# edavalosanaya/FastPoseCNN

Hardware: AMD Instinct MI355X
Metric: img/s end-to-end 640x480 inference; hough-vote kernel HBM GB/s vs roofline (higher is better)
Workload: dtype f32

## Files before the change

fastposecnn_amd/_native.py:

```python
import ctypes
import os

import torch

_HERE = os.path.dirname(os.path.abspath(__file__))
LIB_PATH = os.path.join(_HERE, "libfpc_hip.so")

_lib = None

_vp = ctypes.c_void_p
_i = ctypes.c_int
_i64 = ctypes.c_int64
_u64 = ctypes.c_uint64
_f = ctypes.c_float
_sz = ctypes.c_size_t

_SIGNATURES = {
    "fpc_abi_version": (ctypes.c_int, []),
    "fpc_error_string": (ctypes.c_char_p, [_i]),
    "fpc_last_hip_error": (ctypes.c_char_p, []),
    "fpc_generate_hypothesis": (_i, [_vp, _vp, _vp, _vp, _i, _i, _i, _vp]),
    "fpc_voting_for_hypothesis": (_i, [_vp, _vp, _vp, _vp, _i, _i, _i, _f, _vp]),
    "fpc_ransac_workspace_bytes": (_sz, [_i, _i, _i, _i]),
    "fpc_ransac_voting_v3": (_i, [_vp, _vp, _i64, _i64, _i64, _i64, _i, _vp, _i, _i, _i, _vp, _vp, _u64, _f, _i, _i,
                                  _vp, _vp, _vp, _vp, _vp, _vp, _vp, _vp, _vp, _sz, _vp]),
    "fpc_ransac_voting_v3_bits": (_i, [_vp, _vp, _vp, _i64, _i64, _i64, _i64, _i, _vp, _i, _i, _i, _vp, _vp, _u64, _f, _i, _i, _vp, _vp, _vp, _vp, _vp, _vp, _vp, _vp, _vp, _sz, _vp]),
    "fpc_ransac_voting_v3_pose": (_i, [_vp, _vp, _vp, _i64, _i64, _i64, _i64, _i, _vp, _i, _i, _i, _vp, _vp, _u64, _f, _i, _i, _vp, _vp, _vp, _vp, _vp, _vp, _vp, _vp,
                                       _vp, _vp, _vp, _vp, _vp, _vp, _vp, _sz, _vp]),
    "fpc_vote_set_prune": (_i, [_i, _i, ctypes.POINTER(ctypes.c_int32)]),
    "fpc_vote_prune_info": (_i, [_vp, _sz, _i, _i, _i, _i, _vp, _vp]),
    "fpc_class_compress": (_i, [_vp, _vp, _vp, _vp, _vp, _vp, _i, _i, _i, _vp, _vp, _vp, _vp, _vp, _vp]),
    "fpc_class_compress_bits": (_i, [_vp, _vp, _vp, _vp, _vp, _vp, _i, _i, _i, _vp, _vp, _vp, _vp, _vp, _vp, _vp]),
    "fpc_cc_workspace_bytes": (_sz, [_i, _i, _i]),
    "fpc_cc_bits_supported": (_i, [_i, _i, _i]),
    "fpc_fg_bits": (_i, [_vp, _i, _i, _i, _vp, _vp]),
    "fpc_cc_label_bits": (_i, [_vp, _i, _i, _i, _vp, _vp, _vp, _i, _vp, _sz, _vp]),
    "fpc_cc_label": (_i, [_vp, _i, _i, _i, _vp, _vp, _vp, _i, _vp, _sz, _vp]),
    "fpc_aggregate_workspace_bytes": (_sz, [_i]),
    "fpc_aggregate": (_i, [_vp, _vp, _vp, _vp, _vp, _vp, _i, _i, _i, _i, _vp, _vp, _vp, _vp, _vp, _vp, _vp, _vp, _vp, _vp, _sz,
                           _vp]),
    "fpc_aggregate_bits": (_i, [_vp, _vp, _vp, _vp, _vp, _vp, _i, _i, _i, _i, _vp, _vp, _vp, _vp, _vp, _vp, _vp, _vp, _vp, _vp, _vp, _vp, _sz, _vp]),
    "fpc_mask_bits_words": (_sz, [_i, _i]),
    "fpc_pose_errors": (_i, [_vp, _vp, _vp, _vp, _i, _vp, _vp, _vp, _vp, _vp, _vp, _i, _vp, _vp, _vp, _vp]),
    "fpc_post_network_backward": (_i, [_vp, _vp, _i, _i, _i, _i, _vp, _vp, _f, _i, _u64, _vp, _vp, _vp, _vp, _vp, _vp]),
    "fpc_vote_refine_backward": (_i, [_vp, _vp, _i64, _i64, _i64, _i64, _i, _i, _i, _vp, _f, _i, _u64, _vp, _vp, _vp]),
    "fpc_class_compress_backward": (_i, [_vp, _vp, _vp, _vp, _vp, _vp, _vp, _i, _i, _i, _vp, _vp, _vp, _vp, _vp]),
    "fpc_mask_losses": (_i, [_vp, _vp, _i, _i, _i, _i64, _i64, _f, _f, _vp, _vp, _vp, _vp]),
    "fpc_grad_sumsq": (_i, [_vp, _sz, _vp, _vp]),
    "fpc_lookahead_radam_step": (_i, [_vp, _vp, _vp, _vp, _vp, _sz, _f, _f, _f, _f, _f, _i64, _i, _f, _vp, _vp]),
    "fpc_pose_rt": (_i, [_vp, _vp, _vp, _vp, _i, _vp, _vp, _vp, _vp]),
    "fpc_pack_pose_records": (_i, [_vp] * 9 + [_i, _i, _i, _vp, _vp]),
    "fpc_mask_iou_workspace_bytes": (_sz, [_i, _i, _i64]),
    "fpc_mask_iou": (_i, [_vp, _i, _vp, _i, _i64, _i, _vp, _vp, _vp, _vp, _sz, _vp]),
    "fpc_preprocess_workspace_bytes": (_sz, [_i]),
    "fpc_preprocess_u8": (_i, [_vp, _i, _i, _i, ctypes.POINTER(ctypes.c_double), ctypes.POINTER(ctypes.c_double), _i, _vp, _vp,
                               _sz, _vp]),
    "fpc_png_info": (_i, [_vp, _sz, ctypes.POINTER(ctypes.c_int32)]),
    "fpc_png_decode": (_i, [_vp, _sz, _vp, _sz, _i]),
    "fpc_png_decode_batch": (_i, [ctypes.POINTER(_vp), ctypes.POINTER(_sz), _i, _vp, _i, _i, _i]),
    "fpc_net_create": (_i, [ctypes.c_char_p, _i, _i, _i, _i, ctypes.POINTER(_vp)]),
    "fpc_net_create_encoder": (_i, [_i, ctypes.POINTER(_i), _i, _i, _i, _i, ctypes.POINTER(_vp)]),
    "fpc_net_destroy": (None, [_vp]),
    "fpc_net_set_graph": (_i, [_vp, _i]),
    "fpc_net_set_split_precision": (_i, [_vp, _i]),
    "fpc_net_param_count": (_i, [_vp]),
    "fpc_net_param_name": (ctypes.c_char_p, [_vp, _i]),
    "fpc_net_param_numel": (_i64, [_vp, _i]),
    "fpc_net_workspace_bytes": (_sz, [_vp]),
    "fpc_net_load_params": (_i, [_vp, _vp, _i, _vp, _sz, _vp]),
    "fpc_net_forward": (_i, [_vp, _vp, _vp, _vp, _vp, _vp, _vp, _vp, _vp, _vp, _vp, _vp, _vp]),
    "fpc_net_forward_bits": (_i, [_vp, _vp, _vp, _vp, _vp, _vp, _vp, _vp, _vp, _vp, _vp, _vp, _vp, _vp]),
    "fpc_net_autotune_next": (_i, [_vp, _i]),
    "fpc_net_conv_count": (_i, [_vp]),
    "fpc_net_conv_plan": (_i, [_vp, _i, ctypes.POINTER(_i)]),
    "fpc_net_copy_plans": (_i, [_vp, _vp]),
    "fpc_net_force_winograd": (_i, [_vp, _i]),
    "fpc_net_force_pointwise": (_i, [_vp, _i]),
    "fpc_net_force_fold": (_i, [_vp, _i]),
    "fpc_net_force_direct_h3": (_i, [_vp, _i]),
    "fpc_net_force_stem_pool": (_i, [_vp, _i]),
    "fpc_stem_pool_tasks": (_i, [_i, _i, ctypes.POINTER(_i64)]),
    "fpc_net_graph_recorded": (_i, [_vp]),
    "fpc_net_flops": (_i, [_vp, ctypes.POINTER(ctypes.c_double)]),
    "fpc_net_tensor": (_i, [_vp, ctypes.c_char_p, ctypes.POINTER(_vp), ctypes.POINTER(_i), ctypes.POINTER(_i),
                            ctypes.POINTER(_i)]),
    "fpc_conv2d_workspace_bytes": (_sz, [_i, _i, _i, _i, _i, _i, _i]),
    "fpc_conv2d_workspace_bytes_for": (_sz, [_i, _i, _i, _i, _i, _i, _i, _i, _i, _i]),
    "fpc_conv2d_plan": (_i, [_i, _i, _i, _i, _i, _i, _i, _i, _i, _i, ctypes.POINTER(_i)]),
    "fpc_conv2d": (_i, [_vp, _i64, _i64, _i64, _i64, _vp, _vp, _vp, _vp, _vp, _vp, _vp, _i, _i, _i, _i, _i, _i, _i, _i,
                        _i, _i, _i, _i, _i, _vp, _sz, _vp]),
    "fpc_conv2d_wgrad_workspace_bytes": (_sz, [_i, _i, _i, _i, _i, _i, _i]),
    "fpc_upsample_bilinear_fwd": (_i, [_vp, _i64, _i64, _i64, _i64, _vp, _i, _i, _i, _i, _i, _i, _vp]),
    "fpc_upsample_bilinear_bwd_scratch_floats": (_sz, [_i, _i, _i, _i, _i]),
    "fpc_upsample_bilinear_bwd": (_i, [_vp, _i64, _i64, _i64, _i64, _vp, _vp, _i, _i, _i, _i, _i, _i, _vp]),
    "fpc_groupnorm4_relu_scratch_floats": (_sz, [_i, _i, _i]),
    "fpc_groupnorm4_relu_fwd": (_i, [_vp, _vp, _vp, _vp, _vp, _vp, _i, _i, _i, _i, ctypes.c_float, _vp]),
    "fpc_groupnorm4_relu_bwd": (_i, [_vp, _vp, _vp, _vp, _vp, _vp, _vp, _i, _i, _i, _i, _vp]),
    "fpc_conv2d_wgrad": (_i, [_vp, _i64, _i64, _i64, _vp, _vp, _i, _i, _i, _i, _i, _i, _i, _i, _i, _vp, _sz, _vp]),
    "fpc_conv2d_wgrad_split": (_i, [_vp, _i64, _i64, _i64, _vp, _vp, _i, _i, _i, _i, _i, _i, _i, _i, _i, _vp, _sz, _vp]),
}

EXPORTED = tuple(_SIGNATURES)


def lib():
    global _lib
    if _lib is None:
        if not os.path.exists(LIB_PATH):
            raise RuntimeError(
                f"fastposecnn_amd: {LIB_PATH} is missing — build it with `python -m fastposecnn_amd.build` "
                "(hipcc --offload-arch=gfx950). There is no CPU fallback for the HIP hot path.")
        L = ctypes.CDLL(LIB_PATH)
        for name, (res, args) in _SIGNATURES.items():
            fn = getattr(L, name)
            fn.restype = res
            fn.argtypes = args
        if L.fpc_abi_version() != 11:
            raise RuntimeError("fastposecnn_amd: libfpc_hip.so ABI version mismatch")
        _lib = L
    return _lib


def check(rc, what):
    if rc != 0:
        L = lib()
        msg = L.fpc_error_string(rc).decode()
        hip = L.fpc_last_hip_error().decode() if rc == -3 else ""
        raise RuntimeError(f"fastposecnn_amd: {what} failed: {msg} (code {rc}){' — HIP: ' + hip if hip else ''}")


def ptr(t):
    return None if t is None else t.data_ptr()


_raw_stream = getattr(torch._C, "_cuda_getCurrentRawStream", None)
_cur_device = getattr(torch._C, "_cuda_getDevice", None)


def stream():
    if _raw_stream is not None and _cur_device is not None:
        return _raw_stream(_cur_device())
    return torch.cuda.current_stream().cuda_stream


def require_gpu(*tensors, what="this op"):
    for t in tensors:
        if t is not None and not t.is_cuda:
            raise RuntimeError(f"fastposecnn_amd: {what} runs only on GPU tensors (HIP kernels, no CPU fallback)")


_workspaces = {}


def workspace(tag, device, nbytes):
    key = (tag, device.index, stream())
    ws = _workspaces.get(key)
    if ws is None or ws.numel() < nbytes:
        ws = torch.empty(max(int(nbytes), 256), dtype=torch.uint8, device=device)
        assert ws.data_ptr() % 256 == 0
        _workspaces[key] = ws
    return ws
```

fastposecnn_amd/csrc/net.hip:

```cpp
#include <math.h>
#include <stdio.h>
#include <stdlib.h>
#include <string.h>

#include <initializer_list>
#include <string>
#include <utility>
#include <vector>

#include "net_kernels.hpp"

namespace fpc {

struct PackedConv {
    int Cin = 0, Cinp = 0, Cout = 0, Kh = 1, Kw = 1, stride = 1, pad = 0;
    int Kwp = 1;
    int K = 0, Kpad = 0, Npad = 0;
    int p_w = -1;
    int p_bn = -1;
    int p_bias = -1;
    size_t w_off = 0, scale_off = 0, shift_off = 0;
    size_t wino_off = 0;
    bool wino_ok = false;
    size_t h3_off = 0;
    bool h3_ok = false;
};

struct Act { size_t off = 0; int H = 0, W = 0, C = 0; };

struct ConvPlan {
    int bm = 64, bn = 64, nsplit = 1, mtiles = 1, ntiles = 1, wino = 0, bf3 = 0, fused = 0;
    int lat = 0;
    int stem = 0;
    int pw = 0;
    int fold = 0;
    int h3 = 0;
    int pool = 0;
};

static bool stem_ok(const ConvArgs& a) {
    return a.lanepx == 1 && a.generic == 0 && a.Kh == 7 && a.stride == 2 && a.pad == 3 && a.Cout == 64 && a.Kpad == 224 &&
           a.Wo % 64 == 0 && !a.p[0].res && !a.p[0].up && !a.p[0].gn_part && a.in_sc == 1 && a.in_sw == 4 &&
           a.in_sh == (long long)4 * a.Wi && a.in_sb == (long long)4 * a.Hi * a.Wi;
}

static bool lateral_ok(const ConvArgs& a, int groups) {
    if (a.Kh != 1 || a.Kw != 1 || a.stride != 1 || a.pad != 0 || a.generic != 0 || (a.Cin != 64 && a.Cin != 128) || a.Kpad != a.Cin ||
        a.Cout % 32 != 0 || a.in_sc != 1 || a.in_sw != a.Cin || a.in_sh != (long long)a.Wi * a.Cin ||
        a.in_sb != (long long)a.Hi * a.Wi * a.Cin || a.lanepx)
        return false;
    for (int g = 0; g < groups; ++g)
        if (a.p[g].in != a.p[0].in || a.p[g].scale || a.p[g].res || a.p[g].gn_part || ((a.p[g].up != nullptr) != (a.p[0].up != nullptr)))
            return false;
    return !(a.p[0].up && ((a.Ho | a.Wo) & 1));
}

static bool pw_ok(const ConvArgs& a, int groups) {
    if (a.Kh != 1 || a.Kw != 1 || a.pad != 0 || (a.stride != 1 && a.stride != 2) || a.generic != 0 || a.lanepx || a.Cin % 64 != 0 ||
        a.Kpad != a.Cin || a.Cout % 64 != 0 || a.in_sc != 1)
        return false;
    for (int g = 0; g < groups; ++g)
        if (a.p[g].in != a.p[0].in || a.p[g].gn_part || (a.p[g].scale != nullptr) != (a.p[0].scale != nullptr) ||
            (a.p[g].shift != nullptr) != (a.p[0].shift != nullptr) || (a.p[g].res != nullptr) != (a.p[0].res != nullptr) ||
            (a.p[g].up != nullptr) != (a.p[0].up != nullptr))
            return false;
    return !(a.p[0].up && ((a.Ho | a.Wo) & 1));
}

static bool can_fuse(const ConvPlan& p, int groups, int B) {
    return p.nsplit > 1 && (long long)groups * B * p.mtiles * p.ntiles <= kConvTickets;
}

static ConvPlan plan_conv(int HoWo, int B, int Cout, int ksteps, int groups, int force_bm = 0, int force_bn = 0,
                          int force_split = 0) {
    ConvPlan best;
    double best_t = 1e300;
    const int bms[2] = {64, 128}, bns[2] = {64, 128};
    for (int bi = 0; bi < 2; ++bi)
        for (int bj = 0; bj < 2; ++bj) {
            int bm = bms[bi], bn = bns[bj];
            if (force_bm && bm != force_bm) continue;
            if (force_bn && bn != force_bn) continue;
            if (!force_bn && bn == 128 && Cout <= 64) continue;
            int mt = cdiv(HoWo, bm), nt = cdiv(Cout, bn);
            for (int ns = 1; ns <= 32; ++ns) {
                if (force_split && ns != force_split) continue;
                int per = cdiv(ksteps, ns);
                if ((ns - 1) * per >= ksteps) continue;
                if (ns > 1 && (Cout % 4 != 0)) continue;
                double nblk = (double)groups * B * mt * nt * ns;
                double work = (double)(bm / 64) * (bn / 64) * per * 16.0 * 64.0 + 4000.0;
                double t = ceil(nblk / 256.0) * work + (ns > 1 ? 10000.0 + 200.0 * ns : 0.0);
                if (t < best_t) { best_t = t; best = ConvPlan{bm, bn, ns, mt, nt, 0}; }
            }
        }
    best.fused = can_fuse(best, groups, B) ? 1 : 0;
    return best;
}

static std::vector<ConvPlan> conv_candidates(int HoWo, int B, int Cout, int ksteps, int groups) {
    std::vector<ConvPlan> out;
    const int splits[] = {1, 2, 3, 4, 6, 8, 12, 16, 24};
    for (int bm = 64; bm <= 128; bm += 64)
        for (int bn = 64; bn <= 128; bn += 64) {
            if (bn == 128 && Cout <= 64) continue;
            int mt = cdiv(HoWo, bm), nt = cdiv(Cout, bn);
            long long base = (long long)groups * B * mt * nt;
            for (int ns : splits) {
                int per = cdiv(ksteps, ns);
                if (ns > 1 && (per < 2 || (ns - 1) * per >= ksteps || Cout % 4 != 0)) continue;
                if (ns > 1 && base * ns > 4096) continue;
                out.push_back(ConvPlan{bm, bn, ns, mt, nt, 0});
                if (can_fuse(out.back(), groups, B)) { ConvPlan f = out.back(); f.fused = 1; out.push_back(f); }
            }
        }
    return out;
}

static size_t splitk_floats_for(const ConvPlan& p, int groups, int B, int Npad) {
    return p.nsplit > 1 ? (size_t)groups * p.nsplit * B * p.mtiles * p.bm * Npad : 0;
}

}

using namespace fpc;

struct fpc_net {
    int layers[4];
    int classes, B, H, W;
    int expansion = 1;
    std::vector<std::string> pnames;
    std::vector<int64_t> pnumel;
    std::vector<const float*> pptr;
    std::vector<PackedConv> convs;
    size_t packed_floats = 0;
    size_t total_floats = 0;
    float* ws = nullptr;
    bool loaded = false;
    bool tuning = false;
    bool tuned = false;
    int tune_mode = 0;

    int c_stem = -1;
    struct Block { int conv1, conv2, ds, conv3 = -1; };
    std::vector<Block> blocks[4];
    struct Dec {
        int lat[4];
        int seg[7];
        int p_gn[7];
        int p_head_w, p_head_b;
        int head_ch, head_chp;
    } dec[4];

    Act a_img4, a_stem, a_pool;
    std::vector<Act> a_blk_t[4], a_blk_y[4], a_blk_d[4];
    std::vector<Act> a_blk_t2[4];
    Act a_p[4][4];
    Act a_seg[4][7];
    Act a_up[4][3];
    size_t gn_part_off[4][7], gn_aff_off[4][7];
    int gn_P[7];
    Act a_low[4];
    Act a_lsum[4];
    int merge_split = -1;
    size_t splitk_off = 0, splitk_floats = 0;
    int use_graph = 0;
    int split_precision = 0;
    hipGraphExec_t graph_exec = nullptr;
    size_t zeros_off = 0;
    size_t tickets_off = 0;

    bool h3_packed = false;
    hipStream_t load_stream = nullptr;
    size_t stem_h3_off = 0;
    bool fold_ok = false;
    size_t fold_wc_off[4] = {}, fold_img1_off[4] = {}, fold_img2_off[4] = {}, fold_tab_off[4] = {};

    std::vector<ConvPlan> cplan;
    std::vector<float> tune_score;
    std::vector<int> c_howo, c_groups;

    size_t bump = 0;
    size_t alloc(size_t n) { size_t o = bump; bump += (n + 63) / 64 * 64; return o; }
    Act alloc_act(int h, int w, int c) { Act a; a.H = h; a.W = w; a.C = c; a.off = alloc((size_t)B * h * w * c); return a; }
    int add_param(const std::string& n, int64_t numel) { pnames.push_back(n); pnumel.push_back(numel); return (int)pnames.size() - 1; }

    int add_conv(const std::string& wname, int Cin, int Cout, int k, int stride, int pad, const char* bn_prefix,
                 const char* bias_name, int Cinp = 0, int Kwp = 0) {
        PackedConv c;
        c.Cin = Cin; c.Cinp = Cinp ? Cinp : Cin; c.Cout = Cout; c.Kh = c.Kw = k; c.stride = stride; c.pad = pad;
        c.Kwp = Kwp ? Kwp : k;
        c.K = c.Cinp * k * c.Kwp; c.Kpad = cdiv(c.K, kConvBK) * kConvBK; c.Npad = cdiv(Cout, kConvNAlign) * kConvNAlign;
        c.p_w = add_param(wname, (int64_t)Cout * Cin * k * k);
        if (bn_prefix) {
            std::string p(bn_prefix);
            c.p_bn = add_param(p + ".weight", Cout);
            add_param(p + ".bias", Cout);
            add_param(p + ".running_mean", Cout);
            add_param(p + ".running_var", Cout);
        }
        if (bias_name) c.p_bias = add_param(bias_name, Cout);
        c.w_off = alloc(conv_packed_floats(c.Npad, c.Kpad));
        if (bn_prefix) { c.scale_off = alloc(Cout); c.shift_off = alloc(Cout); }
        c.wino_ok = (k == 3 && stride == 1 && pad == 1 && c.Cinp == Cin && Cin % 8 == 0 && Cout % 64 == 0);
        if (c.wino_ok) c.wino_off = alloc((size_t)(Cout % 128 == 0 ? 96 : 72) * Cout * Cin + 80);
        convs.push_back(c);
        return (int)convs.size() - 1;
    }
};

static const char* kDecNames[4] = {"mask_decoder", "rotation_decoder", "translation_decoder", "scales_decoder"};
static const char* kHeadNames[4] = {"segmentation_head", "rotation_head", "translation_head", "scales_head"};

static int conv_out(int x, int k, int s, int p) { return (x + 2 * p - k) / s + 1; }

static int net_build(fpc_net* n, int classes, int B, int H, int W, fpc_net_t** out);

extern "C" int fpc_net_create(const char* encoder, int classes, int B, int H, int W, fpc_net_t** out) {
    if (!encoder || !out || classes < 2 || classes > 8 || B < 1 || H < 32 || W < 32 || H % 32 || W % 32) return FPC_EINVAL;
    fpc_net* n = new fpc_net();
    if (!strcmp(encoder, "resnet18")) { int l[4] = {2, 2, 2, 2}; memcpy(n->layers, l, sizeof(l)); }
    else if (!strcmp(encoder, "resnet34")) { int l[4] = {3, 4, 6, 3}; memcpy(n->layers, l, sizeof(l)); }
    else { delete n; return FPC_EINVAL; }
    return net_build(n, classes, B, H, W, out);
}

extern "C" int fpc_net_create_encoder(int block, const int* layers4, int classes, int B, int H, int W, fpc_net_t** out) {
    if (!layers4 || !out || (block != 1 && block != 4) || classes < 2 || classes > 8 || B < 1 || H < 32 || W < 32 || H % 32 ||
        W % 32)
        return FPC_EINVAL;
    for (int L = 0; L < 4; ++L)
        if (layers4[L] < 1 || layers4[L] > 64) return FPC_EINVAL;
    fpc_net* n = new fpc_net();
    memcpy(n->layers, layers4, sizeof(n->layers));
    n->expansion = block;
    return net_build(n, classes, B, H, W, out);
}

static int net_build(fpc_net* n, int classes, int B, int H, int W, fpc_net_t** out) {
    n->classes = classes; n->B = B; n->H = H; n->W = W;
    {
        const char* e = getenv("FPC_MERGE_SPLIT");
        n->merge_split = e ? (atoi(e) != 0) : 1;
    }
    char buf[256];

    n->c_stem = n->add_conv("encoder.conv1.weight", 3, 64, 7, 2, 3, "encoder.bn1", nullptr, 4, 8);
    const int planes[4] = {64, 128, 256, 512};
    const int e = n->expansion;
    int inpl = 64;
    for (int L = 0; L < 4; ++L)
        for (int bi = 0; bi < n->layers[L]; ++bi) {
            int stride = (bi == 0 && L > 0) ? 2 : 1;
            fpc_net::Block blk;
            snprintf(buf, sizeof(buf), "encoder.layer%d.%d", L + 1, bi);
            std::string p(buf);
            if (e == 4) {
                const int C = 4 * planes[L];
                blk.conv1 = n->add_conv(p + ".conv1.weight", inpl, planes[L], 1, 1, 0, (p + ".bn1").c_str(), nullptr);
                blk.conv2 = n->add_conv(p + ".conv2.weight", planes[L], planes[L], 3, stride, 1, (p + ".bn2").c_str(), nullptr);
                blk.conv3 = n->add_conv(p + ".conv3.weight", planes[L], C, 1, 1, 0, (p + ".bn3").c_str(), nullptr);
                blk.ds = -1;
                if (stride != 1 || inpl != C)
                    blk.ds = n->add_conv(p + ".downsample.0.weight", inpl, C, 1, stride, 0, (p + ".downsample.1").c_str(), nullptr);
                inpl = C;
                n->blocks[L].push_back(blk);
                continue;
            }
            blk.conv1 = n->add_conv(p + ".conv1.weight", inpl, planes[L], 3, stride, 1, (p + ".bn1").c_str(), nullptr);
            blk.conv2 = n->add_conv(p + ".conv2.weight", planes[L], planes[L], 3, 1, 1, (p + ".bn2").c_str(), nullptr);
            blk.ds = -1;
            if (stride != 1 || inpl != planes[L])
                blk.ds = n->add_conv(p + ".downsample.0.weight", inpl, planes[L], 1, stride, 0, (p + ".downsample.1").c_str(), nullptr);
            inpl = planes[L];
            n->blocks[L].push_back(blk);
        }
    const int G = classes - 1;
    const int head_ch[4] = {classes, 4 * G, 3 * G, 3 * G};
    for (int d = 0; d < 4; ++d) {
        std::string D(kDecNames[d]);
        fpc_net::Dec& dc = n->dec[d];
        dc.lat[0] = n->add_conv(D + ".p5.weight", 512 * e, 256, 1, 1, 0, nullptr, (D + ".p5.bias").c_str());
        const int skipc[3] = {256 * e, 128 * e, 64 * e};
        for (int i = 0; i < 3; ++i) {
            snprintf(buf, sizeof(buf), "%s.p%d.skip_conv", kDecNames[d], 4 - i);
            std::string p(buf);
            dc.lat[1 + i] = n->add_conv(p + ".weight", skipc[i], 256, 1, 1, 0, nullptr, (p + ".bias").c_str());
        }
        const int nconv[4] = {3, 2, 1, 1};
        int si = 0;
        for (int sb = 0; sb < 4; ++sb)
            for (int j = 0; j < nconv[sb]; ++j) {
                snprintf(buf, sizeof(buf), "%s.seg_blocks.%d.block.%d.block", kDecNames[d], sb, j);
                std::string p(buf);
                dc.seg[si] = n->add_conv(p + ".0.weight", j == 0 ? 256 : 128, 128, 3, 1, 1, nullptr, nullptr);
                dc.p_gn[si] = n->add_param(p + ".1.weight", 128);
                n->add_param(p + ".1.bias", 128);
                ++si;
            }
    }
    for (int d = 0; d < 4; ++d) {
        fpc_net::Dec& dc = n->dec[d];
        dc.head_ch = head_ch[d];
        dc.head_chp = (head_ch[d] + 3) / 4 * 4;
        dc.p_head_w = n->add_param(std::string(kHeadNames[d]) + ".0.weight", (int64_t)head_ch[d] * 128);
        dc.p_head_b = n->add_param(std::string(kHeadNames[d]) + ".0.bias", head_ch[d]);
    }
    n->fold_ok = e == 1;
    if (n->fold_ok)
        for (int d = 0; d < 4; ++d) {
            n->fold_wc_off[d] = n->alloc((size_t)128 * 64 * 9);
            n->fold_img1_off[d] = n->alloc((size_t)16 * 128 * 64 + 2);
            n->fold_img2_off[d] = n->alloc((size_t)16 * 128 * 256 + 2);
            n->fold_tab_off[d] = n->alloc((size_t)16 * 128);
        }
    if (e == 1) {
        std::vector<int> sites;
        for (int L = 1; L < 4; ++L) { sites.push_back(n->blocks[L][0].conv1); if (n->blocks[L][0].ds >= 0) sites.push_back(n->blocks[L][0].ds); }
        for (int d = 0; d < 4; ++d)
            for (int i = 0; i < 3; ++i) sites.push_back(n->dec[d].lat[i]);
        for (int ci : sites) {
            PackedConv& c = n->convs[ci];
            if (c.wino_ok || c.Cin % kConvBK != 0 || c.Cinp != c.Cin || c.Kh * c.Kw > 32) continue;
            c.h3_ok = true;
            c.h3_off = n->alloc(h3_packed_floats(c.Npad, c.Kpad));
        }
    }
    n->stem_h3_off = n->alloc(h3_packed_floats(n->convs[n->c_stem].Npad, n->convs[n->c_stem].Kpad));
    n->zeros_off = n->alloc(64);
    n->tickets_off = n->alloc(kConvTickets);
    n->packed_floats = n->bump;

    int h1 = conv_out(H, 7, 2, 3), w1 = conv_out(W, 7, 2, 3);
    n->a_img4 = n->alloc_act(H, W, 4);
    n->a_stem = n->alloc_act(h1, w1, 64);
    int hp = conv_out(h1, 3, 2, 1), wp = conv_out(w1, 3, 2, 1);
    n->a_pool = n->alloc_act(hp, wp, 64);
    int fh[4], fw[4];
    {
        int h = hp, w = wp;
        for (int L = 0; L < 4; ++L) {
            const int hin = h, win = w;
            if (L > 0) { h = conv_out(h, 3, 2, 1); w = conv_out(w, 3, 2, 1); }
            fh[L] = h; fw[L] = w;
            if (e == 4) {
                const int C = 4 * planes[L];
                const Act t1 = n->alloc_act(hin, win, planes[L]), t2 = n->alloc_act(h, w, planes[L]);
                const Act y[2] = {n->alloc_act(h, w, C), n->alloc_act(h, w, C)};
                const Act dd = n->alloc_act(h, w, C);
                for (int bi = 0; bi < n->layers[L]; ++bi) {
                    Act t = t1;
                    if (bi > 0) { t.H = h; t.W = w; }
                    n->a_blk_t[L].push_back(t);
                    n->a_blk_t2[L].push_back(t2);
                    n->a_blk_y[L].push_back(y[bi & 1]);
                    n->a_blk_d[L].push_back(n->blocks[L][bi].ds >= 0 ? dd : Act());
                }
                continue;
            }
            for (int bi = 0; bi < n->layers[L]; ++bi) {
                n->a_blk_t[L].push_back(n->alloc_act(h, w, planes[L]));
                n->a_blk_y[L].push_back(n->alloc_act(h, w, planes[L]));
                n->a_blk_d[L].push_back(n->blocks[L][bi].ds >= 0 ? n->alloc_act(h, w, planes[L]) : Act());
            }
        }
    }
    for (int L = 1; L < 4; ++L)
        if (fh[L - 1] != 2 * fh[L] || fw[L - 1] != 2 * fw[L]) { delete n; return FPC_EINVAL; }
    const int seg_level[7] = {3, 2, 1, 2, 1, 1, 0};
    for (int d = 0; d < 4; ++d) {
        for (int i = 0; i < 4; ++i) n->a_p[d][i] = n->alloc_act(fh[3 - i], fw[3 - i], 256);
        for (int i = 0; i < 7; ++i) n->a_seg[d][i] = n->alloc_act(fh[seg_level[i]], fw[seg_level[i]], 128);
        n->a_up[d][0] = n->alloc_act(fh[2], fw[2], 128);
        n->a_up[d][1] = n->alloc_act(fh[1], fw[1], 128);
        n->a_up[d][2] = n->alloc_act(fh[1], fw[1], 128);
        n->a_low[d] = n->alloc_act(fh[0], fw[0], n->dec[d].head_chp);
        n->a_lsum[d] = n->alloc_act(fh[1], fw[1], n->dec[d].head_chp);
    }

    n->cplan.resize(n->convs.size());
    n->tune_score.assign(n->convs.size(), 0.f);
    n->c_howo.assign(n->convs.size(), 0);
    n->c_groups.assign(n->convs.size(), 0);
    auto plan = [&](int ci, int HoWo, int groups) {
        const PackedConv& c = n->convs[ci];
        n->c_howo[ci] = HoWo; n->c_groups[ci] = groups;
        n->cplan[ci] = plan_conv(HoWo, B, c.Cout, c.Kpad / kConvBK, groups);
        size_t need = splitk_floats_for(n->cplan[ci], groups, B, c.Npad);
        for (const ConvPlan& q : conv_candidates(HoWo, B, c.Cout, c.Kpad / kConvBK, groups)) {
            size_t f = splitk_floats_for(q, groups, B, c.Npad);
            if (f * sizeof(float) <= ((size_t)256 << 20) && f > need) need = f;
        }
        if (need > n->splitk_floats) n->splitk_floats = need;
    };
    plan(n->c_stem, h1 * w1, 1);
    for (int L = 0; L < 4; ++L)
        for (size_t bi = 0; bi < n->blocks[L].size(); ++bi) {
            const fpc_net::Block& blk = n->blocks[L][bi];
            if (e == 4) {
                plan(blk.conv1, n->a_blk_t[L][bi].H * n->a_blk_t[L][bi].W, 1);
                plan(blk.conv2, fh[L] * fw[L], 1);
                plan(blk.conv3, fh[L] * fw[L], 1);
                if (blk.ds >= 0) plan(blk.ds, fh[L] * fw[L], 1);
                continue;
            }
            plan(blk.conv1, fh[L] * fw[L], 1);
            plan(blk.conv2, fh[L] * fw[L], 1);
            if (blk.ds >= 0) plan(blk.ds, fh[L] * fw[L], 1);
        }
    for (int i = 0; i < 4; ++i) plan(n->dec[0].lat[i], fh[3 - i] * fw[3 - i], 4);
    for (int i = 0; i < 7; ++i) {
        int HoWo = fh[seg_level[i]] * fw[seg_level[i]];
        plan(n->dec[0].seg[i], HoWo, 4);
        n->gn_P[i] = cdiv(HoWo, 128) * 4;
        for (int d = 0; d < 4; ++d) {
            n->gn_part_off[d][i] = n->alloc((size_t)B * n->gn_P[i] * 128 * 2);
            n->gn_aff_off[d][i] = n->alloc((size_t)B * 128 * 2);
        }
    }
    n->splitk_off = n->alloc(n->splitk_floats);
    n->total_floats = n->bump;
    n->pptr.assign(n->pnames.size(), nullptr);
    *out = n;
    return FPC_OK;
}

extern "C" void fpc_net_destroy(fpc_net_t* n) {
    if (!n) return;
    if (n->graph_exec) (void)hipGraphExecDestroy(n->graph_exec);
    delete n;
}

static int pack_h3_images(fpc_net* n, hipStream_t s) {
    for (const PackedConv& c : n->convs)
        if (c.h3_ok) {
            int rc = launch_pack_weight_h3(n->pptr[c.p_w], n->ws + c.h3_off, c.Cout, c.Cin, c.Cinp, c.Kh, c.Kw, c.Kwp, c.Npad, c.Kpad, s);
            if (rc) return rc;
        }
    const PackedConv& st = n->convs[n->c_stem];
    int rc = launch_pack_weight_h3(n->pptr[st.p_w], n->ws + n->stem_h3_off, st.Cout, st.Cin, st.Cinp, st.Kh, st.Kw, st.Kwp, st.Npad, st.Kpad, s);
    if (rc) return rc;
    n->h3_packed = true;
    return FPC_OK;
}

extern "C" int fpc_net_set_split_precision(fpc_net_t* n, int on) {
    if (!n) return FPC_EINVAL;
    n->split_precision = on < 0 ? 0 : (on > 3 ? 3 : on);
    if (n->split_precision >= 3 && n->loaded && !n->h3_packed) return pack_h3_images(n, n->load_stream);
    return FPC_OK;
}

extern "C" int fpc_net_graph_recorded(const fpc_net_t* n) { return n && n->use_graph && n->graph_exec ? 1 : 0; }

extern "C" int fpc_net_set_graph(fpc_net_t* n, int on) {
    if (!n) return FPC_EINVAL;
    n->use_graph = on ? 1 : 0;
    if (!on && n->graph_exec) { (void)hipGraphExecDestroy(n->graph_exec); n->graph_exec = nullptr; }
    return FPC_OK;
}
extern "C" int fpc_net_param_count(const fpc_net_t* n) { return n ? (int)n->pnames.size() : 0; }
extern "C" const char* fpc_net_param_name(const fpc_net_t* n, int i) {
    return (n && i >= 0 && i < (int)n->pnames.size()) ? n->pnames[i].c_str() : nullptr;
}
extern "C" int64_t fpc_net_param_numel(const fpc_net_t* n, int i) {
    return (n && i >= 0 && i < (int)n->pnumel.size()) ? n->pnumel[i] : -1;
}
extern "C" size_t fpc_net_workspace_bytes(const fpc_net_t* n) { return n ? n->total_floats * sizeof(float) : 0; }

extern "C" int fpc_net_load_params(fpc_net_t* n, const float* const* params, int count, void* ws, size_t ws_bytes,
                                   fpc_stream_t stream) {
    if (!n || !params || count != (int)n->pnames.size() || !ws) return FPC_EINVAL;
    if (((uintptr_t)ws & 255) != 0 || ws_bytes < n->total_floats * sizeof(float)) return FPC_EWORKSPACE;
    if (n->graph_exec) { (void)hipGraphExecDestroy(n->graph_exec); n->graph_exec = nullptr; }
    for (int i = 0; i < count; ++i)
        if (!params[i] || ((uintptr_t)params[i] & 15)) return FPC_EINVAL;
    hipStream_t s = (hipStream_t)stream;
    n->ws = (float*)ws;
    n->pptr.assign(params, params + count);
    n->load_stream = s;
    n->h3_packed = false;
    if (n->split_precision >= 3) { int rc = pack_h3_images(n, s); if (rc) return rc; }
    if (hipMemsetAsync(n->ws + n->zeros_off, 0, 64 * sizeof(float), s) != hipSuccess) return FPC_ELAUNCH;
    if (hipMemsetAsync(n->ws + n->tickets_off, 0, kConvTickets * sizeof(int), s) != hipSuccess) return FPC_ELAUNCH;
    for (const PackedConv& c : n->convs) {
        int rc = launch_pack_weight(n->pptr[c.p_w], n->ws + c.w_off, c.Cout, c.Cin, c.Cinp, c.Kh, c.Kw, c.Kwp, c.Npad, c.Kpad, s);
        if (rc) return rc;
        rc = launch_pack_weight_bf3(n->pptr[c.p_w], n->ws + c.w_off, c.Cout, c.Cin, c.Cinp, c.Kh, c.Kw, c.Kwp, c.Npad, c.Kpad, s);
        if (rc) return rc;
        if (c.wino_ok) {
            rc = launch_wino_pack(n->pptr[c.p_w], n->ws + c.wino_off, c.Cout, c.Cin, s);
            if (rc) return rc;
            rc = launch_wino_pack_bf3(n->pptr[c.p_w], n->ws + c.wino_off + (size_t)16 * c.Cout * c.Cin, c.Cout, c.Cin, s);
            if (rc) return rc;
            if (c.Cout % 128 == 0) {
                rc = launch_wino_pack_c128(n->pptr[c.p_w], n->ws + c.wino_off + (size_t)40 * c.Cout * c.Cin, c.Cout, c.Cin, s);
                if (rc) return rc;
            }
            rc = launch_wino_pack_h2(n->pptr[c.p_w], n->ws + c.wino_off + (size_t)(c.Cout % 128 == 0 ? 64 : 40) * c.Cout * c.Cin, c.Cout, c.Cin, s);
            if (rc) return rc;
            if (c.Cin % 16 == 0) {
                rc = launch_wino_pack_h3(n->pptr[c.p_w], n->ws + c.wino_off + (size_t)(c.Cout % 128 == 0 ? 80 : 56) * c.Cout * c.Cin + 8, c.Cout, c.Cin, s);
                if (rc) return rc;
            }
        }
        if (c.p_bn >= 0) {
            rc = launch_fold_bn(n->pptr[c.p_bn], n->pptr[c.p_bn + 1], n->pptr[c.p_bn + 2], n->pptr[c.p_bn + 3], 1e-5f,
                                c.Cout, n->ws + c.scale_off, n->ws + c.shift_off, s);
            if (rc) return rc;
        }
    }
    if (n->fold_ok)
        for (int d = 0; d < 4; ++d) {
            const PackedConv &sc = n->convs[n->dec[d].seg[6]], &lc = n->convs[n->dec[d].lat[3]];
            int rc = launch_fold_compose(n->pptr[sc.p_w], n->pptr[lc.p_w], n->pptr[lc.p_bias], n->ws + n->fold_wc_off[d],
                                         n->ws + n->fold_tab_off[d], sc.Cout, sc.Cin, lc.Cin, s);
            if (!rc) rc = launch_wino_pack_h3_pair(n->ws + n->fold_wc_off[d], n->ws + n->fold_img1_off[d], lc.Cin, n->pptr[sc.p_w],
                                                   n->ws + n->fold_img2_off[d], sc.Cin, sc.Cout, s);
            if (rc) return rc;
        }
    n->loaded = true;
    return FPC_OK;
}

namespace {

struct ConvIO {
    const float* in; long long sb, sh, sw, sc; int Hi, Wi;
    float* out; int Ho, Wo;
    const float* res; const float* up; float* gn_part;
};

void fill_conv_args(const fpc_net* n, ConvArgs& a, const PackedConv& c, const ConvPlan& p, int Hi, int Wi, int Ho,
                    int Wo, long long sb, long long sh, long long sw, long long sc, bool relu, int mode) {
    memset(&a, 0, sizeof(a));
    a.B = n->B; a.Hi = Hi; a.Wi = Wi; a.Cin = c.Cin; a.Ho = Ho; a.Wo = Wo; a.Cout = c.Cout; a.Npad = c.Npad;
    a.Kh = c.Kh; a.Kw = c.Kw; a.stride = c.stride; a.pad = c.pad; a.K = c.K; a.Kpad = c.Kpad;
    a.in_sb = sb; a.in_sh = sh; a.in_sw = sw; a.in_sc = sc;
    a.relu = relu ? 1 : 0; a.nsplit = p.nsplit; a.mtiles = p.mtiles; a.ntiles = p.ntiles; a.ksteps = c.Kpad / kConvBK;
    a.bm = p.bm; a.bn = p.bn; a.generic = mode;
    a.splitk_ws = n->ws + n->splitk_off;
    a.zeros = n->ws + n->zeros_off;
    a.tickets = (int*)(n->ws + n->tickets_off);
    a.fused = p.fused;
}

int launch_conv_plan(ConvArgs& a, const ConvPlan& p, int groups, hipStream_t s) {
    if (p.stem) {
        if (groups != 1 || !stem_ok(a)) return FPC_EINVAL;
        StemArgs t;
        memset(&t, 0, sizeof(t));
        t.in = a.p[0].in;
        t.wpl = reinterpret_cast<const unsigned short*>(a.p[0].w + (size_t)a.Npad * a.Kpad);
        t.out = a.p[0].out; t.scale = a.p[0].scale; t.shift = a.p[0].shift;
        t.B = a.B; t.Hi = a.Hi; t.Wi = a.Wi; t.Ho = a.Ho; t.Wo = a.Wo; t.Cout = a.Cout; t.Npad = a.Npad; t.Kpad = a.Kpad; t.relu = a.relu;
        t.grid = p.stem;
        return launch_stem7x7(t, s);
    }
    if (p.pw) {
        if (!pw_ok(a, groups)) return FPC_EINVAL;
        PwArgs w;
        memset(&w, 0, sizeof(w));
        w.in = a.p[0].in;
        for (int g = 0; g < groups; ++g) {
            w.wpl[g] = reinterpret_cast<const unsigned short*>(a.p[g].w + (size_t)a.Npad * a.Kpad);
            w.out[g] = a.p[g].out; w.scale[g] = a.p[g].scale; w.shift[g] = a.p[g].shift; w.res[g] = a.p[g].res; w.up[g] = a.p[g].up;
        }
        w.in_sb = a.in_sb; w.in_sh = a.in_sh; w.in_sw = a.in_sw;
        w.B = a.B; w.Ho = a.Ho; w.Wo = a.Wo; w.Cin = a.Cin; w.Cout = a.Cout; w.Npad = a.Npad; w.Kpad = a.Kpad; w.stride = a.stride;
        w.groups = groups; w.relu = a.relu;
        w.has_scale = a.p[0].scale != nullptr; w.has_shift = a.p[0].shift != nullptr;
        w.has_res = a.p[0].res != nullptr; w.has_up = a.p[0].up != nullptr;
        w.variant = p.pw - 1;
        return launch_conv1x1(w, s);
    }
    if (p.lat) {
        if (!lateral_ok(a, groups)) return FPC_EINVAL;
        LatArgs l;
        memset(&l, 0, sizeof(l));
        l.in = a.p[0].in;
        for (int g = 0; g < groups; ++g) {
            if (p.h3 && !a.h3_w[g]) return FPC_EINVAL;
            l.wpl[g] = reinterpret_cast<const unsigned short*>(p.h3 ? a.h3_w[g] : a.p[g].w + (size_t)a.Npad * a.Kpad);
            l.out[g] = a.p[g].out; l.shift[g] = a.p[g].shift; l.up[g] = a.p[g].up;
        }
        l.B = a.B; l.Ho = a.Ho; l.Wo = a.Wo; l.Cout = a.Cout; l.Npad = a.Npad; l.Kpad = a.Kpad; l.groups = groups; l.relu = a.relu;
        l.parts = p.lat;
        l.h3 = p.h3;
        return launch_lateral1x1(l, s);
    }
    if (p.wino) {
        WinoArgs w;
        memset(&w, 0, sizeof(w));
        for (int g = 0; g < groups; ++g) {
            if (!a.wino_w[g] || a.p[g].up) return FPC_EINVAL;
            w.p[g] = a.p[g];
            w.p[g].w = a.wino_w[g] + ((p.wino == 5 || p.wino == 7) ? (size_t)16 * a.Cout * a.Cin : p.wino == 6 ? (size_t)40 * a.Cout * a.Cin
                                      : p.wino == 8 ? (size_t)(a.Cout % 128 == 0 ? 64 : 40) * a.Cout * a.Cin
                                      : p.wino == 9 ? (size_t)(a.Cout % 128 == 0 ? 80 : 56) * a.Cout * a.Cin + 8 : 0);
        }
        w.variant = p.wino == 3 ? 1 : (p.wino == 4 ? 2 : (p.wino == 5 ? 3 : 0));
        w.zeros = a.zeros;
        w.dbg = (long long*)a.dbg;
        w.groups = groups;
        w.B = a.B; w.H = a.Ho; w.W = a.Wo; w.Cin = a.Cin; w.Cout = a.Cout; w.relu = a.relu;
        w.waves = (p.wino == 2 || p.wino == 4 || p.wino == 5 || p.wino == 7 || p.wino == 8 || p.wino == 9) ? 8 : 4;
        w.tbx = cdiv(cdiv(a.Wo, 2), 8); w.tby = cdiv(cdiv(a.Ho, 2), w.waves);
        if (p.fold) {
            if (p.wino != 9 || !a.fold_in) return FPC_EINVAL;
            for (int g = 0; g < groups; ++g) {
                w.in2[g] = a.fold_up[g]; w.w2[g] = a.fold_w2[g];
                w.btab[g] = a.fold_tab[g];
                w.p[g].in = a.fold_in; w.p[g].w = a.fold_w[g];
            }
            w.fold = 1; w.Cin2 = a.Cin; w.Cin = a.fold_cin;
        }
        if (p.wino == 6) return a.Cout % 128 == 0 ? launch_conv_wino_c128(w, groups, s) : FPC_EINVAL;
        if (p.wino == 7) return launch_conv_wino_w4(w, groups, s);
        if (p.wino == 9) return launch_conv_wino_h3(w, groups, s);
        if (p.wino == 8) return launch_conv_wino_h2(w, groups, s);
        return launch_conv_wino(w, groups, s);
    }
    a.bm = p.bm; a.bn = p.bn; a.nsplit = p.nsplit; a.mtiles = p.mtiles; a.ntiles = p.ntiles; a.groups = groups;
    a.bf3 = (p.bf3 && a.generic == 0) ? 1 : 0;
    a.fused = (p.fused && p.nsplit > 1) ? 1 : 0;
    a.h3 = 0;
    if (p.h3) {
        if (a.generic != 0) return FPC_EINVAL;
        ConvArgs h = a;
        h.bf3 = 0; h.h3 = 1;
        for (int g = 0; g < groups; ++g) {
            if (!a.h3_w[g]) return FPC_EINVAL;
            h.p[g].w = a.h3_w[g];
        }
        int rc = launch_conv(h, groups, s);
        if (!rc && h.nsplit > 1 && !h.fused) rc = launch_conv_splitk_epilogue(h, groups, s);
        return rc;
    }
    int rc = launch_conv(a, groups, s);
    if (rc) return rc;
    if (a.nsplit > 1 && !a.fused) rc = launch_conv_splitk_epilogue(a, groups, s);
    return rc;
}

int plan_gn_rows(const ConvPlan& p, int Ho, int Wo) {
    return p.wino ? cdiv(cdiv(Wo, 2), 8) * cdiv(cdiv(Ho, 2), (p.wino == 2 || p.wino == 4 || p.wino == 5 || p.wino == 7 || p.wino == 8 || p.wino == 9) ? 8 : 4) : p.mtiles * p.bm / 32;
}

int run_conv(fpc_net* n, ConvArgs& a, int groups, int ci, hipStream_t s) {
    if (n && n->tuning) {
        hipEvent_t e0, e1;
        if (hipEventCreate(&e0) != hipSuccess || hipEventCreate(&e1) != hipSuccess) return FPC_ELAUNCH;
        float best_ms = 1e30f;
        ConvPlan best = n->cplan[ci];
        size_t cap = n->splitk_floats;
        std::vector<ConvPlan> cands = conv_candidates(a.Ho * a.Wo, a.B, a.Cout, a.ksteps, groups);
        const size_t nf = cands.size();
        if (n->split_precision && a.generic == 0) {
            for (size_t i = 0; i < nf; ++i) { ConvPlan q = cands[i]; q.bf3 = 1; cands.push_back(q); }
        }
        if (n->split_precision >= 3 && a.generic == 0 && a.h3_w[0]) {
            for (size_t i = 0; i < nf; ++i) { ConvPlan q = cands[i]; q.h3 = 1; cands.push_back(q); }
        }
        if (n->split_precision && groups == 1 && stem_ok(a)) {
            ConvPlan sq; sq.stem = 256; cands.push_back(sq);
        }
        if (n->split_precision && lateral_ok(a, groups)) {
            const int tiles = groups * (a.Cout / 32);
            for (int parts = 1; parts <= tiles; parts *= 2)
                if (tiles % parts == 0) {
                    ConvPlan lq; lq.lat = parts; cands.push_back(lq);
                    if (n->split_precision >= 3 && a.h3_w[0]) { lq.h3 = 1; cands.push_back(lq); }
                }
        }
        if (n->split_precision && n->expansion == 4 && pw_ok(a, groups)) {
            ConvPlan pq;
            pq.pw = 1; cands.push_back(pq);
            pq.pw = 2; cands.push_back(pq);
        }
        if (a.wino_w[0] && !a.p[0].up) {
            ConvPlan wq;
            wq.wino = 1; cands.push_back(wq);
            wq.wino = 2; cands.push_back(wq);
            wq.wino = 3; cands.push_back(wq);
            if (a.zeros) { wq.wino = 4; cands.push_back(wq); }
            if (n->split_precision && a.zeros) { wq.wino = 5; cands.push_back(wq); }
            if (n->split_precision && a.Cout % 128 == 0) { wq.wino = 6; cands.push_back(wq); }
            if (n->split_precision) { wq.wino = 7; cands.push_back(wq); }
            if (n->split_precision >= 3 && a.Cin % 16 == 0) { wq.wino = 9; cands.push_back(wq); }
            else if (n->split_precision >= 2) { wq.wino = 8; cands.push_back(wq); }
        }
        for (const ConvPlan& q : cands) {
            if (splitk_floats_for(q, groups, a.B, a.Npad) > cap) continue;
            int rc = launch_conv_plan(a, q, groups, s);
            if (rc == FPC_EINVAL) continue;
            if (rc) { (void)hipEventDestroy(e0); (void)hipEventDestroy(e1); return rc; }
            float ms = 1e30f;
            for (int rep = 0; rep < 3; ++rep) {
                float t = 0.f;
                bool timed = hipEventRecord(e0, s) == hipSuccess && launch_conv_plan(a, q, groups, s) == FPC_OK &&
                             hipEventRecord(e1, s) == hipSuccess && hipEventSynchronize(e1) == hipSuccess &&
                             hipEventElapsedTime(&t, e0, e1) == hipSuccess;
                if (timed && t < ms) ms = t;
            }
            float score = ms;
            if (n->tune_mode >= 1) {
                double nblk = q.stem ? 512.0
                              : q.lat ? (double)cdiv(a.Ho * a.Wo, 128) * a.B * q.lat
                              : q.pw ? (double)cdiv(a.B * a.Ho * a.Wo, pw_tile_pixels(q.pw - 1)) * (a.Cout / 64) * groups * q.pw
                              : q.wino ? (double)cdiv(cdiv(a.Wo, 2), 8) * cdiv(cdiv(a.Ho, 2), (q.wino == 2 || q.wino == 4 || q.wino == 5 || q.wino == 7 || q.wino == 8 || q.wino == 9) ? 8 : 4) * a.B * (a.Cout / (q.wino == 6 ? 128 : 64)) * groups
                                     : (double)q.mtiles * q.ntiles * q.nsplit * a.B * groups;
                double slots = 256.0 * ((q.wino == 2 || q.wino == 4 || q.wino == 5 || q.wino == 6 || q.wino == 7 || q.wino == 8 || q.wino == 9) ? 1.0 : 2.0);
                double share = nblk / slots;
                if (share > 1.0) share = 1.0;
                if (share < 0.125) share = 0.125;
                score = ms * (float)(n->tune_mode == 2 ? share : sqrt(share));
            }
            if (score < best_ms) { best_ms = score; best = q; }
        }
        n->tune_score[ci] = best_ms;
        if (n->split_precision >= 3 && a.fold_in && a.fold_lat_ms > 0.f) {
            ConvPlan fq;
            fq.wino = 9; fq.fold = 1;
            int rc = launch_conv_plan(a, fq, groups, s);
            if (rc && rc != FPC_EINVAL) { (void)hipEventDestroy(e0); (void)hipEventDestroy(e1); return rc; }
            float ms = 1e30f;
            for (int rep = 0; rep < 3 && !rc; ++rep) {
                float t = 0.f;
                bool timed = hipEventRecord(e0, s) == hipSuccess && launch_conv_plan(a, fq, groups, s) == FPC_OK &&
                             hipEventRecord(e1, s) == hipSuccess && hipEventSynchronize(e1) == hipSuccess &&
                             hipEventElapsedTime(&t, e0, e1) == hipSuccess;
                if (timed && t < ms) ms = t;
            }
            if (ms < best_ms + a.fold_lat_ms) best = fq;
        }
        (void)hipEventDestroy(e0);
        (void)hipEventDestroy(e1);
        n->cplan[ci] = best;
    }
    ConvPlan p = n ? n->cplan[ci] : ConvPlan{a.bm, a.bn, a.nsplit, a.mtiles, a.ntiles, 0, a.bf3, a.fused};
    return launch_conv_plan(a, p, groups, s);
}

}

#define FPC_TRY(x) do { int rc__ = (x); if (rc__) return rc__; } while (0)

static int launch_stem_pool(const ConvArgs& a, const float* h3_image, float* pool, int Hp, int Wp, hipStream_t s) {
    if (!h3_image || !stem_ok(a)) return FPC_EINVAL;
    StemPoolArgs t;
    memset(&t, 0, sizeof(t));
    t.in = a.p[0].in; t.wpl = reinterpret_cast<const unsigned short*>(h3_image); t.out = pool;
    t.scale = a.p[0].scale; t.shift = a.p[0].shift;
    t.B = a.B; t.Hi = a.Hi; t.Wi = a.Wi; t.Ho = a.Ho; t.Wo = a.Wo; t.Hp = Hp; t.Wp = Wp; t.Npad = a.Npad; t.Kpad = a.Kpad; t.relu = a.relu;
    t.band = kStemPoolBand; t.grid = 256;
    return launch_stem_pool_h3(t, s);
}

static int forward_middle(fpc_net* n, hipStream_t s) {
    float* ws = n->ws;
    const int B = n->B, H = n->H, W = n->W;
    ConvArgs a;
    auto nhwc = [&](const Act& t, long long& sb, long long& sh, long long& sw, long long& sc) {
        sc = 1; sw = t.C; sh = (long long)t.W * t.C; sb = (long long)t.H * sh;
    };
    {
        const PackedConv& c = n->convs[n->c_stem];
        fill_conv_args(n, a, c, n->cplan[n->c_stem], H, W, n->a_stem.H, n->a_stem.W, (long long)4 * H * W, (long long)4 * W, 4,
                       1, true, 0);
        a.Cin = 8 * c.Cinp; a.Kw = 1; a.K = c.K; a.lanepx = 1;
        a.p[0] = ConvPtrs{ws + n->a_img4.off, ws + c.w_off, ws + n->a_stem.off, ws + c.scale_off, ws + c.shift_off, nullptr, nullptr, nullptr};
        const float* h3img = n->h3_packed ? ws + n->stem_h3_off : nullptr;
        auto pool_launch = [&]() {
            return launch_maxpool3x3s2(ws + n->a_stem.off, ws + n->a_pool.off, B, n->a_stem.H, n->a_stem.W, 64, n->a_pool.H, n->a_pool.W, s);
        };
        if (n->cplan[n->c_stem].pool && !n->tuning) {
            FPC_TRY(launch_stem_pool(a, h3img, ws + n->a_pool.off, n->a_pool.H, n->a_pool.W, s));
        } else {
            n->cplan[n->c_stem].pool = 0;
            FPC_TRY(run_conv(n, a, 1, n->c_stem, s));
            FPC_TRY(pool_launch());
            if (n->tuning && n->split_precision >= 3 && launch_stem_pool(a, h3img, ws + n->a_pool.off, n->a_pool.H, n->a_pool.W, s) == FPC_OK) {
                hipEvent_t e0, e1;
                if (hipEventCreate(&e0) != hipSuccess || hipEventCreate(&e1) != hipSuccess) return FPC_ELAUNCH;
                const ConvPlan cur = n->cplan[n->c_stem];
                float ms_pair = 1e30f, ms_fused = 1e30f;
                for (int rep = 0; rep < 6; ++rep) {
                    const bool fused = rep & 1;
                    float t = 0.f;
                    bool timed = hipEventRecord(e0, s) == hipSuccess &&
                                 (fused ? launch_stem_pool(a, h3img, ws + n->a_pool.off, n->a_pool.H, n->a_pool.W, s) == FPC_OK
                                        : (launch_conv_plan(a, cur, 1, s) == FPC_OK && pool_launch() == FPC_OK)) &&
                                 hipEventRecord(e1, s) == hipSuccess && hipEventSynchronize(e1) == hipSuccess &&
                                 hipEventElapsedTime(&t, e0, e1) == hipSuccess;
                    if (timed && fused && t < ms_fused) ms_fused = t;
                    if (timed && !fused && t < ms_pair) ms_pair = t;
                }
                (void)hipEventDestroy(e0);
                (void)hipEventDestroy(e1);
                if (ms_fused < ms_pair) { ConvPlan q; q.stem = 256; q.pool = 1; n->cplan[n->c_stem] = q; }
            }
        }
    }
    Act cur = n->a_pool;
    Act feat[4];
    for (int L = 0; L < 4; ++L) {
        for (size_t bi = 0; bi < n->blocks[L].size(); ++bi) {
            const fpc_net::Block& blk = n->blocks[L][bi];
            const Act& T = n->a_blk_t[L][bi];
            const Act& Y = n->a_blk_y[L][bi];
            long long sb, sh, sw, sc;
            if (n->expansion == 4) {
                const Act& T2 = n->a_blk_t2[L][bi];
                nhwc(cur, sb, sh, sw, sc);
                const PackedConv& c1 = n->convs[blk.conv1];
                fill_conv_args(n, a, c1, n->cplan[blk.conv1], cur.H, cur.W, T.H, T.W, sb, sh, sw, sc, true, 0);
                a.p[0] = ConvPtrs{ws + cur.off, ws + c1.w_off, ws + T.off, ws + c1.scale_off, ws + c1.shift_off, nullptr, nullptr, nullptr};
                FPC_TRY(run_conv(n, a, 1, blk.conv1, s));
                long long tb, th, tw, tc;
                nhwc(T, tb, th, tw, tc);
                const PackedConv& c2 = n->convs[blk.conv2];
                fill_conv_args(n, a, c2, n->cplan[blk.conv2], T.H, T.W, T2.H, T2.W, tb, th, tw, tc, true, 0);
                a.p[0] = ConvPtrs{ws + T.off, ws + c2.w_off, ws + T2.off, ws + c2.scale_off, ws + c2.shift_off, nullptr, nullptr, nullptr};
                if (c2.wino_ok) a.wino_w[0] = ws + c2.wino_off;
                FPC_TRY(run_conv(n, a, 1, blk.conv2, s));
                const float* res = ws + cur.off;
                if (blk.ds >= 0) {
                    const PackedConv& cd = n->convs[blk.ds];
                    const Act& D = n->a_blk_d[L][bi];
                    fill_conv_args(n, a, cd, n->cplan[blk.ds], cur.H, cur.W, D.H, D.W, sb, sh, sw, sc, false, 0);
                    a.p[0] = ConvPtrs{ws + cur.off, ws + cd.w_off, ws + D.off, ws + cd.scale_off, ws + cd.shift_off, nullptr, nullptr, nullptr};
                    FPC_TRY(run_conv(n, a, 1, blk.ds, s));
                    res = ws + D.off;
                }
                nhwc(T2, tb, th, tw, tc);
                const PackedConv& c3 = n->convs[blk.conv3];
                fill_conv_args(n, a, c3, n->cplan[blk.conv3], T2.H, T2.W, Y.H, Y.W, tb, th, tw, tc, true, 0);
                a.p[0] = ConvPtrs{ws + T2.off, ws + c3.w_off, ws + Y.off, ws + c3.scale_off, ws + c3.shift_off, res, nullptr, nullptr};
                FPC_TRY(run_conv(n, a, 1, blk.conv3, s));
                cur = Y;
                continue;
            }
            nhwc(cur, sb, sh, sw, sc);
            const PackedConv& c1 = n->convs[blk.conv1];
            fill_conv_args(n, a, c1, n->cplan[blk.conv1], cur.H, cur.W, T.H, T.W, sb, sh, sw, sc, true, 0);
            a.p[0] = ConvPtrs{ws + cur.off, ws + c1.w_off, ws + T.off, ws + c1.scale_off, ws + c1.shift_off, nullptr, nullptr, nullptr};
            if (c1.wino_ok) a.wino_w[0] = ws + c1.wino_off;
            if (c1.h3_ok && n->h3_packed) a.h3_w[0] = ws + c1.h3_off;
            FPC_TRY(run_conv(n, a, 1, blk.conv1, s));
            const float* res = ws + cur.off;
            if (blk.ds >= 0) {
                const PackedConv& cd = n->convs[blk.ds];
                const Act& D = n->a_blk_d[L][bi];
                fill_conv_args(n, a, cd, n->cplan[blk.ds], cur.H, cur.W, D.H, D.W, sb, sh, sw, sc, false, 0);
                a.p[0] = ConvPtrs{ws + cur.off, ws + cd.w_off, ws + D.off, ws + cd.scale_off, ws + cd.shift_off, nullptr, nullptr, nullptr};
                if (cd.h3_ok && n->h3_packed) a.h3_w[0] = ws + cd.h3_off;
                FPC_TRY(run_conv(n, a, 1, blk.ds, s));
                res = ws + D.off;
            }
            nhwc(T, sb, sh, sw, sc);
            const PackedConv& c2 = n->convs[blk.conv2];
            fill_conv_args(n, a, c2, n->cplan[blk.conv2], T.H, T.W, Y.H, Y.W, sb, sh, sw, sc, true, 0);
            a.p[0] = ConvPtrs{ws + T.off, ws + c2.w_off, ws + Y.off, ws + c2.scale_off, ws + c2.shift_off, res, nullptr, nullptr};
            if (c2.wino_ok) a.wino_w[0] = ws + c2.wino_off;
            FPC_TRY(run_conv(n, a, 1, blk.conv2, s));
            cur = Y;
        }
        feat[L] = cur;
    }

    const bool fold = n->cplan[n->dec[0].seg[6]].fold && !n->tuning;
    for (int i = 0; i < 4; ++i) {
        if (i == 3 && fold) continue;
        const Act& src = feat[3 - i];
        long long sb, sh, sw, sc;
        nhwc(src, sb, sh, sw, sc);
        int ci0 = n->dec[0].lat[i];
        fill_conv_args(n, a, n->convs[ci0], n->cplan[ci0], src.H, src.W, src.H, src.W, sb, sh, sw, sc, false, 0);
        for (int d = 0; d < 4; ++d) {
            const PackedConv& c = n->convs[n->dec[d].lat[i]];
            a.p[d] = ConvPtrs{ws + src.off, ws + c.w_off, ws + n->a_p[d][i].off, nullptr, n->pptr[c.p_bias], nullptr,
                              i > 0 ? ws + n->a_p[d][i - 1].off : nullptr, nullptr};
            if (c.h3_ok && n->h3_packed) a.h3_w[d] = ws + c.h3_off;
        }
        FPC_TRY(run_conv(n, a, 4, ci0, s));
    }
    auto seg_conv = [&](int si, int which) -> int {
        int ci0 = n->dec[0].seg[si];
        const Act& in0 = which < 0 ? n->a_p[0][-which - 1] : n->a_up[0][which];
        long long sb, sh, sw, sc;
        nhwc(in0, sb, sh, sw, sc);
        const Act& o0 = n->a_seg[0][si];
        fill_conv_args(n, a, n->convs[ci0], n->cplan[ci0], in0.H, in0.W, o0.H, o0.W, sb, sh, sw, sc, false, 0);
        for (int d = 0; d < 4; ++d) {
            const PackedConv& c = n->convs[n->dec[d].seg[si]];
            const Act& in = which < 0 ? n->a_p[d][-which - 1] : n->a_up[d][which];
            a.p[d] = ConvPtrs{ws + in.off, ws + c.w_off, ws + n->a_seg[d][si].off, nullptr, nullptr, nullptr, nullptr,
                              ws + n->gn_part_off[d][si]};
            if (c.wino_ok) a.wino_w[d] = ws + c.wino_off;
        }
        if (si == 6 && n->fold_ok) {
            a.fold_in = ws + feat[0].off;
            a.fold_cin = feat[0].C;
            for (int d = 0; d < 4; ++d) {
                a.fold_w[d] = ws + n->fold_img1_off[d];
                a.fold_w2[d] = ws + n->fold_img2_off[d];
                a.fold_up[d] = ws + n->a_p[d][2].off;
                a.fold_tab[d] = ws + n->fold_tab_off[d];
            }
            a.fold_lat_ms = n->tune_score[n->dec[0].lat[3]];
        }
        return run_conv(n, a, 4, ci0, s);
    };
    auto gn_finish = [&](std::initializer_list<int> sites) -> int {
        GnFinArgs g;
        memset(&g, 0, sizeof(g));
        int k = 0;
        for (int si : sites) {
            const Act& o0 = n->a_seg[0][si];
            for (int d = 0; d < 4; ++d) {
                g.gn_part[k * kMaxGroup + d] = ws + n->gn_part_off[d][si];
                g.gamma[k * kMaxGroup + d] = n->pptr[n->dec[d].p_gn[si]];
                g.beta[k * kMaxGroup + d] = n->pptr[n->dec[d].p_gn[si] + 1];
                g.affine[k * kMaxGroup + d] = ws + n->gn_aff_off[d][si];
            }
            g.P[k] = plan_gn_rows(n->cplan[n->dec[0].seg[si]], o0.H, o0.W);
            g.count[k] = (long long)o0.H * o0.W * 4;
            ++k;
        }
        g.B = B; g.C = 128; g.groups = 32; g.sites = k; g.eps = 1e-5f;
        return launch_gn_finalize(g, 4, s);
    };
    auto gn_up = [&](std::initializer_list<std::pair<int, int>> jobs) -> int {
        GnUpArgs u;
        memset(&u, 0, sizeof(u));
        int k = 0;
        for (const auto& job : jobs) {
            const int si = job.first, ui = job.second;
            for (int d = 0; d < 4; ++d) {
                u.in[k * kMaxGroup + d] = ws + n->a_seg[d][si].off;
                u.affine[k * kMaxGroup + d] = ws + n->gn_aff_off[d][si];
                u.out[k * kMaxGroup + d] = ws + n->a_up[d][ui].off;
            }
            u.h[k] = n->a_seg[0][si].H; u.w[k] = n->a_seg[0][si].W;
            ++k;
        }
        u.B = B; u.C = 128; u.jobs = k;
        return launch_gn_relu_up2(u, 4, s);
    };
    FPC_TRY(seg_conv(0, -1));
    FPC_TRY(seg_conv(3, -2));
    FPC_TRY(seg_conv(5, -3));
    FPC_TRY(seg_conv(6, -4));
    FPC_TRY(gn_finish({0, 3, 5, 6}));
    FPC_TRY(gn_up({{0, 0}, {3, 2}}));
    FPC_TRY(seg_conv(1, 0));
    FPC_TRY(seg_conv(4, 2));
    FPC_TRY(gn_finish({1, 4}));
    FPC_TRY(gn_up({{1, 1}}));
    FPC_TRY(seg_conv(2, 1));
    FPC_TRY(gn_finish({2}));

    const int lo[3] = {2, 4, 5};
    const int split = n->merge_split;
    if (split) {
        HeadPartArgs hl, hh;
        memset(&hl, 0, sizeof(hl));
        memset(&hh, 0, sizeof(hh));
        for (int d = 0; d < 4; ++d) {
            for (int k = 0; k < 3; ++k) {
                hl.t[d][k] = ws + n->a_seg[d][lo[k]].off;
                hl.aff[d][k] = ws + n->gn_aff_off[d][lo[k]];
            }
            hh.t[d][0] = ws + n->a_seg[d][6].off;
            hh.aff[d][0] = ws + n->gn_aff_off[d][6];
            hl.hw[d] = hh.hw[d] = n->pptr[n->dec[d].p_head_w];
            hl.hb[d] = hh.hb[d] = n->pptr[n->dec[d].p_head_b];
            hl.out[d] = ws + n->a_lsum[d].off;
            hh.lsum[d] = ws + n->a_lsum[d].off;
            hh.out[d] = ws + n->a_low[d].off;
            hl.ch[d] = hh.ch[d] = n->dec[d].head_ch;
            hl.chp[d] = hh.chp[d] = n->dec[d].head_chp;
        }
        hl.B = hh.B = B; hl.C = hh.C = 128;
        hl.H = n->a_seg[0][2].H; hl.W = n->a_seg[0][2].W; hl.hl = hl.H; hl.wl = hl.W;
        hh.H = n->a_seg[0][6].H; hh.W = n->a_seg[0][6].W; hh.hl = hl.H; hh.wl = hl.W;
        FPC_TRY(launch_head_part(hl, false, 4, s));
        FPC_TRY(launch_head_part(hh, true, 4, s));
    } else {
        MergeHeadArgs m;
        memset(&m, 0, sizeof(m));
        for (int d = 0; d < 4; ++d) {
            for (int k = 0; k < 3; ++k) {
                m.t_lo[d][k] = ws + n->a_seg[d][lo[k]].off;
                m.a_lo[d][k] = ws + n->gn_aff_off[d][lo[k]];
            }
            m.t_hi[d] = ws + n->a_seg[d][6].off;
            m.a_hi[d] = ws + n->gn_aff_off[d][6];
            m.hw[d] = n->pptr[n->dec[d].p_head_w];
            m.hb[d] = n->pptr[n->dec[d].p_head_b];
            m.out[d] = ws + n->a_low[d].off;
            m.ch[d] = n->dec[d].head_ch;
            m.chp[d] = n->dec[d].head_chp;
        }
        m.B = B; m.h = n->a_seg[0][2].H; m.w = n->a_seg[0][2].W; m.C = 128;
        FPC_TRY(launch_merge_head(m, 4, s));
    }
    return FPC_OK;
}

extern "C" int fpc_net_forward(fpc_net_t* n, const float* x, float* logits_mask, float* logits_quat,
                               float* logits_scales, float* logits_xy, float* logits_z, int64_t* cat_mask, float* cq,
                               float* cs, float* cxy, float* cz, fpc_stream_t stream) {
    return fpc_net_forward_bits(n, x, logits_mask, logits_quat, logits_scales, logits_xy, logits_z, cat_mask, cq, cs, cxy, cz, nullptr, stream);
}

extern "C" int fpc_net_forward_bits(fpc_net_t* n, const float* x, float* logits_mask, float* logits_quat,
                                    float* logits_scales, float* logits_xy, float* logits_z, int64_t* cat_mask, float* cq,
                                    float* cs, float* cxy, float* cz, uint64_t* fg_bits, fpc_stream_t stream) {
    if (!n || !n->loaded || !x || !cat_mask || !cq || !cs || !cxy || !cz) return FPC_EINVAL;
    if (fg_bits && (n->W % 64 != 0 || ((uintptr_t)fg_bits & 7))) return FPC_EINVAL;
    bool any = logits_mask || logits_quat || logits_scales || logits_xy || logits_z;
    bool all = logits_mask && logits_quat && logits_scales && logits_xy && logits_z;
    if (any && !all) return FPC_EINVAL;
    hipStream_t s = (hipStream_t)stream;
    float* ws = n->ws;
    const int B = n->B, H = n->H, W = n->W;

    FPC_TRY(launch_nchw3_to_nhwc4(x, ws + n->a_img4.off, B, H * W, s));
    if (n->use_graph && !n->tuning && s != nullptr && !n->graph_exec) {
        hipGraph_t g = nullptr;
        if (hipStreamBeginCapture(s, hipStreamCaptureModeThreadLocal) == hipSuccess) {
            int rc = forward_middle(n, s);
            hipError_t e = hipStreamEndCapture(s, &g);
            if (rc) { if (g) (void)hipGraphDestroy(g); return rc; }
            if (e == hipSuccess && g) e = hipGraphInstantiate(&n->graph_exec, g, nullptr, nullptr, 0);
            if (g) (void)hipGraphDestroy(g);
            if (e != hipSuccess) n->graph_exec = nullptr;
        }
        if (!n->graph_exec) { (void)hipGetLastError(); n->use_graph = 0; }
    }
    if (n->use_graph && !n->tuning && s != nullptr && n->graph_exec) {
        if (hipGraphLaunch(n->graph_exec, s) != hipSuccess) return FPC_ELAUNCH;
    } else {
        FPC_TRY(forward_middle(n, s));
    }
    {
        Up4Args u;
        memset(&u, 0, sizeof(u));
        u.lm = ws + n->a_low[0].off; u.lq = ws + n->a_low[1].off; u.lt = ws + n->a_low[2].off; u.ls = ws + n->a_low[3].off;
        u.pm = n->dec[0].head_chp; u.pq = n->dec[1].head_chp; u.pt = n->dec[2].head_chp; u.ps = n->dec[3].head_chp;
        u.o_mask = logits_mask; u.o_quat = logits_quat; u.o_scales = logits_scales; u.o_xy = logits_xy; u.o_z = logits_z;
        u.cat_mask = (long long*)cat_mask; u.cq = cq; u.cs = cs; u.cxy = cxy; u.cz = cz;
        u.B = B; u.hl = n->a_low[0].H; u.wl = n->a_low[0].W; u.H = H; u.W = W; u.C = n->classes;
        u.fg_bits = reinterpret_cast<unsigned long long*>(fg_bits); u.fg_stride = (size_t)((H * W + 4095) / 4096) * 64;
        if (u.hl * 4 != H || u.wl * 4 != W) return FPC_EINVAL;
        FPC_TRY(launch_up4_compress(u, s));
    }
    if (n->tuning) { n->tuning = false; n->tuned = true; }
    return FPC_OK;
}

extern "C" int fpc_net_autotune_next(fpc_net_t* n, int mode) {
    if (!n || !n->loaded || mode < 0 || mode > 2) return FPC_EINVAL;
    n->tuning = true;
    n->tune_mode = mode;
    if (n->graph_exec) { (void)hipGraphExecDestroy(n->graph_exec); n->graph_exec = nullptr; }
    return FPC_OK;
}

extern "C" int fpc_net_conv_count(const fpc_net_t* n) { return n ? (int)n->convs.size() : 0; }
extern "C" int fpc_net_conv_plan(const fpc_net_t* n, int i, int* out5) {
    if (!n || !out5 || i < 0 || i >= (int)n->convs.size()) return FPC_EINVAL;
    out5[0] = n->cplan[i].bm; out5[1] = n->cplan[i].bn; out5[2] = n->cplan[i].wino ? -n->cplan[i].wino : n->cplan[i].nsplit;
    if (n->cplan[i].lat) { out5[0] = 128; out5[1] = 32; out5[2] = 2000 + n->cplan[i].lat; }
    if (n->cplan[i].stem) { out5[0] = 64; out5[1] = 64; out5[2] = n->cplan[i].pool ? 3100 : 3000; }
    if (n->cplan[i].pw) { out5[0] = pw_tile_pixels(n->cplan[i].pw - 1); out5[1] = 64; out5[2] = 4000 + n->cplan[i].pw - 1; }
    if (n->cplan[i].h3) out5[2] = n->cplan[i].lat ? 7000 + n->cplan[i].lat : 6000 + n->cplan[i].nsplit;
    if (n->fold_ok && i == n->dec[0].lat[3] && n->cplan[n->dec[0].seg[6]].fold) out5[2] = 5000;
    out5[3] = n->convs[i].Cout; out5[4] = n->convs[i].K;
    return FPC_OK;
}

extern "C" int fpc_net_force_winograd(fpc_net_t* n, int form) {
    if (!n || form < 1 || form > 9) return FPC_EINVAL;
    int changed = 0;
    for (size_t i = 0; i < n->convs.size(); ++i) {
        const PackedConv& c = n->convs[i];
        if (!c.wino_ok || !n->c_groups[i] || (form == 6 && c.Cout % 128 != 0) || (form == 9 && c.Cin % 16 != 0)) continue;
        ConvPlan q = n->cplan[i];
        q.wino = form; q.lat = 0; q.stem = 0;
        if (form != 9) q.fold = 0;
        n->cplan[i] = q;
        ++changed;
    }
    if (n->graph_exec) { (void)hipGraphExecDestroy(n->graph_exec); n->graph_exec = nullptr; }
    return changed;
}

extern "C" int fpc_net_force_fold(fpc_net_t* n, int on) {
    if (!n || on < 0 || on > 1 || (on && !n->fold_ok)) return FPC_EINVAL;
    ConvPlan& p = n->cplan[n->dec[0].seg[6]];
    if (p.fold == on) return 0;
    ConvPlan q;
    q.wino = 9; q.fold = on;
    p = q;
    if (n->graph_exec) { (void)hipGraphExecDestroy(n->graph_exec); n->graph_exec = nullptr; }
    return 1;
}

extern "C" int fpc_net_force_pointwise(fpc_net_t* n, int on) {
    if (!n || on < 0 || on > 1) return FPC_EINVAL;
    int changed = 0;
    for (size_t i = 0; i < n->convs.size(); ++i) {
        const PackedConv& c = n->convs[i];
        if (!n->c_groups[i] || c.Kh != 1 || c.pad != 0 || c.Cinp != c.Cin || c.Cin % 64 || c.Kpad != c.Cin || c.Cout % 64) continue;
        if (on) {
            if (n->cplan[i].pw) continue;
            ConvPlan q;
            q.pw = 1;
            n->cplan[i] = q;
        } else {
            if (!n->cplan[i].pw) continue;
            n->cplan[i] = plan_conv(n->c_howo[i], n->B, c.Cout, c.Kpad / kConvBK, n->c_groups[i]);
        }
        ++changed;
    }
    if (n->graph_exec) { (void)hipGraphExecDestroy(n->graph_exec); n->graph_exec = nullptr; }
    return changed;
}

extern "C" int fpc_net_force_direct_h3(fpc_net_t* n, int on) {
    if (!n || on < 0 || on > 1 || (on && !n->h3_packed)) return FPC_EINVAL;
    int changed = 0;
    for (size_t i = 0; i < n->convs.size(); ++i) {
        const PackedConv& c = n->convs[i];
        if (!c.h3_ok || !n->c_groups[i] || on == n->cplan[i].h3) continue;
        const ConvPlan& p = n->cplan[i];
        ConvPlan q = plan_conv(n->c_howo[i], n->B, c.Cout, c.Kpad / kConvBK, n->c_groups[i]);
        if (on && !p.wino && !p.stem && !p.pw) q = p;
        q.bf3 = 0;
        q.h3 = on;
        n->cplan[i] = q;
        ++changed;
    }
    if (n->graph_exec) { (void)hipGraphExecDestroy(n->graph_exec); n->graph_exec = nullptr; }
    return changed;
}

extern "C" int fpc_net_force_stem_pool(fpc_net_t* n, int on) {
    if (!n || on < 0 || on > 1 || (on && !n->h3_packed)) return FPC_EINVAL;
    if (on && ((n->a_stem.H & 1) || (n->a_stem.W & 63) || (long long)n->H * n->W * 16 >= (1LL << 31))) return FPC_EINVAL;
    ConvPlan& p = n->cplan[n->c_stem];
    if (p.pool == on) return 0;
    ConvPlan q;
    q.stem = 256; q.pool = on;
    p = q;
    if (n->graph_exec) { (void)hipGraphExecDestroy(n->graph_exec); n->graph_exec = nullptr; }
    return 1;
}

extern "C" int fpc_net_copy_plans(fpc_net_t* dst, const fpc_net_t* src) {
    if (!dst || !src || dst->convs.size() != src->convs.size() || dst->H != src->H || dst->W != src->W) return FPC_EINVAL;
    for (size_t i = 0; i < dst->convs.size(); ++i) {
        const PackedConv &a = dst->convs[i], &b = src->convs[i];
        if (a.Cin != b.Cin || a.Cout != b.Cout || a.Kh != b.Kh || a.Kw != b.Kw || a.stride != b.stride || a.Npad != b.Npad ||
            a.Kpad != b.Kpad || dst->c_groups[i] != src->c_groups[i])
            return FPC_EINVAL;
    }
    for (size_t i = 0; i < dst->convs.size(); ++i) {
        const ConvPlan& q = src->cplan[i];
        if (splitk_floats_for(q, dst->c_groups[i] ? dst->c_groups[i] : 1, dst->B, dst->convs[i].Npad) > dst->splitk_floats) continue;
        if (q.nsplit > 1 && q.fused && !can_fuse(q, dst->c_groups[i] ? dst->c_groups[i] : 1, dst->B)) continue;
        if ((q.h3 || q.pool) && !dst->h3_packed) continue;
        dst->cplan[i] = q;
    }
    dst->tuned = true;
    if (dst->graph_exec) { (void)hipGraphExecDestroy(dst->graph_exec); dst->graph_exec = nullptr; }
    return FPC_OK;
}

extern "C" int fpc_net_flops(const fpc_net_t* n, double* out3) {
    if (!n || !out3) return FPC_EINVAL;
    double direct = 0.0, executed = 0.0, wino = 0.0;
    for (size_t i = 0; i < n->convs.size(); ++i) {
        if (!n->c_groups[i]) continue;
        const PackedConv& c = n->convs[i];
        const double f = 2.0 * n->B * (double)n->c_howo[i] * c.Cout * c.Cin * c.Kh * c.Kw * n->c_groups[i];
        direct += f;
        if (n->cplan[i].wino) { executed += f / 2.25; wino += f; } else executed += f;
    }
    for (int d = 0; d < 4; ++d)
        direct += 2.0 * n->B * (double)n->a_low[d].H * n->a_low[d].W * 128.0 * n->dec[d].head_ch,
        executed += 2.0 * n->B * (double)n->a_low[d].H * n->a_low[d].W * 128.0 * n->dec[d].head_ch;
    out3[0] = direct; out3[1] = executed; out3[2] = direct > 0.0 ? wino / direct : 0.0;
    return FPC_OK;
}

extern "C" int fpc_net_tensor(const fpc_net_t* n, const char* name, const float** ptr, int* H, int* W, int* C) {
    if (!n || !n->ws || !name || !ptr || !H || !W || !C) return FPC_EINVAL;
    Act t;
    bool ok = false;
    if (!strcmp(name, "stem")) {
        if (n->cplan[n->c_stem].pool) return FPC_EINVAL;
        t = n->a_stem; ok = true;
    }
    else if (!strcmp(name, "pool")) { t = n->a_pool; ok = true; }
    else if (name[0] == 'c' && name[1] >= '2' && name[1] <= '5' && !name[2]) { t = n->a_blk_y[name[1] - '2'].back(); ok = true; }
    else if (name[0] == 'd' && name[1] >= '0' && name[1] <= '3' && name[2] == '.') {
        int d = name[1] - '0';
        const char* r = name + 3;
        if (r[0] == 'p' && r[1] >= '2' && r[1] <= '5' && !r[2]) {
            if (r[1] == '2' && n->cplan[n->dec[0].seg[6]].fold) return FPC_EINVAL;
            t = n->a_p[d]['5' - r[1]]; ok = true;
        }
        else if (!strncmp(r, "seg", 3) && r[3] >= '0' && r[3] <= '6' && !r[4]) { t = n->a_seg[d][r[3] - '0']; ok = true; }
        else if (!strcmp(r, "low")) { t = n->a_low[d]; ok = true; }
    }
    if (!ok) return FPC_EINVAL;
    *ptr = n->ws + t.off; *H = t.H; *W = t.W; *C = t.C;
    return FPC_OK;
}

extern "C" int fpc_stem_pool_tasks(int Ho, int Wo, int64_t* out4) {
    if (!out4 || Ho < 2 || (Ho & 1) || Wo < 64 || (Wo & 63)) return FPC_EINVAL;
    long long o[4];
    stem_pool_tasks(Ho, Wo, kStemPoolBand, o);
    for (int i = 0; i < 4; ++i) out4[i] = o[i];
    return FPC_OK;
}

extern "C" size_t fpc_conv2d_workspace_bytes(int B, int Ho, int Wo, int Cin, int Cout, int Kh, int Kw) {
    int K = Cin * Kh * Kw, Kpad = cdiv(K, kConvBK) * kConvBK, Npad = cdiv(Cout, kConvNAlign) * kConvNAlign;
    size_t packed = conv_packed_floats(Npad, Kpad);
    size_t splitk = (size_t)32 * B * (cdiv(Ho * Wo, 128) * 128) * Npad;
    size_t wino = (size_t)96 * Cout * Cin + 128;
    return (packed + splitk + wino + kConvTickets) * sizeof(float);
}

extern "C" int fpc_conv2d_plan(int B, int Ho, int Wo, int Cin, int Cout, int Kh, int Kw, int bm, int bn, int nsplit,
                               int* out4) {
    if (!out4) return FPC_EINVAL;
    int Kpad = cdiv(Cin * Kh * Kw, kConvBK) * kConvBK;
    if (nsplit >= 6000 && nsplit < 6200) nsplit -= 6000;
    if (nsplit >= 2000) nsplit = 1;
    if (nsplit >= 1000) nsplit -= 1000;
    if (nsplit >= 100) nsplit -= 100;
    ConvPlan p = plan_conv(Ho * Wo, B, Cout, Kpad / kConvBK, 1, bm, bn, nsplit);
    if (nsplit <= -1 && nsplit >= -9) { p.wino = -nsplit; p.nsplit = nsplit; }
    out4[0] = p.bm; out4[1] = p.bn; out4[2] = p.nsplit; out4[3] = plan_gn_rows(p, Ho, Wo);
    return FPC_OK;
}

namespace {
struct Conv2dRequest { int nsplit; bool bf3, two_launch, wino; int lat; bool stem; int pw; bool h3; bool pool; };
Conv2dRequest conv2d_request(int nsplit) {
    Conv2dRequest r{nsplit, false, false, false, 0, false, 0, false, false};
    if (r.nsplit >= 7000 && r.nsplit < 8000) { r.lat = r.nsplit - 7000; r.h3 = true; r.nsplit = 1; return r; }
    if (r.nsplit >= 6000 && r.nsplit < 6200) {
        r.h3 = true; r.nsplit -= 6000;
        if (r.nsplit >= 100) { r.two_launch = true; r.nsplit -= 100; }
        return r;
    }
    if (r.nsplit >= 4000) { r.pw = r.nsplit - 4000 + 1; r.bf3 = true; r.nsplit = 1; return r; }
    if (r.nsplit == 3100) { r.stem = true; r.pool = true; r.h3 = true; r.nsplit = 1; return r; }
    if (r.nsplit == 3000) { r.stem = true; r.bf3 = true; r.nsplit = 1; return r; }
    if (r.nsplit >= 2000) { r.lat = r.nsplit - 2000; r.bf3 = true; r.nsplit = 1; return r; }
    if (r.nsplit >= 1000) { r.bf3 = true; r.nsplit -= 1000; }
    if (r.nsplit >= 100) { r.two_launch = true; r.nsplit -= 100; }
    r.wino = r.nsplit <= -1 && r.nsplit >= -9;
    return r;
}
struct Conv2dLayout { size_t packed, splitk, wino, tickets, total; };
Conv2dLayout conv2d_layout(int B, int Cin, int Cout, int Kh, int Kw, const ConvPlan& p, const Conv2dRequest& r) {
    const int K = Cin * Kh * Kw, Kpad = cdiv(K, kConvBK) * kConvBK, Npad = cdiv(Cout, kConvNAlign) * kConvNAlign;
    Conv2dLayout L;
    L.packed = r.wino ? 0 : conv_packed_floats(Npad, Kpad);
    L.splitk = r.wino ? 0 : (splitk_floats_for(p, 1, B, Npad) + 63) / 64 * 64;
    L.wino = r.wino ? (size_t)(r.nsplit == -9 ? (Cout % 128 == 0 ? 96 : 72) : r.nsplit == -8 ? (Cout % 128 == 0 ? 80 : 56) : r.nsplit == -6 ? 64 : (r.nsplit == -5 || r.nsplit == -7) ? 40 : 16) * Cout * Cin + 128 : 0;
    L.tickets = (!r.wino && p.fused && p.nsplit > 1) ? kConvTickets : 0;
    L.total = L.packed + L.splitk + L.wino + L.tickets;
    return L;
}
ConvPlan conv2d_plan_for(int B, int Ho, int Wo, int Cin, int Cout, int Kh, int Kw, int bm, int bn, const Conv2dRequest& r) {
    const int Kpad = cdiv(Cin * Kh * Kw, kConvBK) * kConvBK;
    ConvPlan p = plan_conv(Ho * Wo, B, Cout, Kpad / kConvBK, 1, r.wino ? 0 : bm, bn, r.wino ? 1 : r.nsplit);
    p.bf3 = r.bf3 ? 1 : 0;
    p.h3 = r.h3 ? 1 : 0;
    if (r.two_launch) p.fused = 0;
    p.lat = r.lat;
    p.stem = r.stem ? 256 : 0;
    p.pool = r.pool ? 1 : 0;
    p.pw = r.pw;
    return p;
}
}

extern "C" size_t fpc_conv2d_workspace_bytes_for(int B, int Ho, int Wo, int Cin, int Cout, int Kh, int Kw, int bm, int bn,
                                                 int nsplit) {
    if (B < 1 || Ho < 1 || Wo < 1 || Cin < 1 || Cout < 1 || Kh < 1 || Kw < 1) return 0;
    const Conv2dRequest r = conv2d_request(nsplit);
    const ConvPlan p = conv2d_plan_for(B, Ho, Wo, Cin, Cout, Kh, Kw, bm, bn, r);
    return std::max<size_t>(conv2d_layout(B, Cin, Cout, Kh, Kw, p, r).total * sizeof(float), 256);
}

extern "C" int fpc_conv2d(const float* in, int64_t sb, int64_t sh, int64_t sw, int64_t sc, const float* w_oihw,
                          const float* scale, const float* shift, const float* res, const float* up, float* out,
                          float* gn_part, int B, int Hi, int Wi, int Cin, int Cout, int Kh, int Kw, int stride, int pad,
                          int relu, int bm, int bn, int nsplit, void* ws, size_t ws_bytes, fpc_stream_t stream) {
    if (!in || !w_oihw || !out || !ws || B < 1 || Kh != Kw) return FPC_EINVAL;
    int Ho = conv_out(Hi, Kh, stride, pad), Wo = conv_out(Wi, Kw, stride, pad);
    if (Ho < 1 || Wo < 1) return FPC_EINVAL;
    const Conv2dRequest rq = conv2d_request(nsplit);
    nsplit = rq.nsplit;
    const bool wino = rq.wino;
    ConvPlan p = conv2d_plan_for(B, Ho, Wo, Cin, Cout, Kh, Kw, bm, bn, rq);
    const Conv2dLayout lay = conv2d_layout(B, Cin, Cout, Kh, Kw, p, rq);
    if (ws_bytes < lay.total * sizeof(float) || ((uintptr_t)ws & 255)) return FPC_EWORKSPACE;
    PackedConv c;
    c.Cin = c.Cinp = Cin; c.Cout = Cout; c.Kh = Kh; c.Kw = Kw; c.stride = stride; c.pad = pad;
    c.K = Cin * Kh * Kw; c.Kpad = cdiv(c.K, kConvBK) * kConvBK; c.Npad = cdiv(Cout, kConvNAlign) * kConvNAlign;
    hipStream_t s = (hipStream_t)stream;
    float* packed = (float*)ws;
    if (rq.stem) {
        if (Cin != 4 || Kh != 7 || stride != 2 || pad != 3 || Cout != 64 || sc != 1 || sw != 4 || sh != (int64_t)4 * Wi ||
            sb != (int64_t)4 * Hi * Wi || res || up || gn_part)
            return FPC_EINVAL;
        c.Kwp = 8; c.K = 4 * 7 * 8; c.Kpad = 224;
        if (rq.pool) {
            FPC_TRY(launch_pack_weight_h3(w_oihw, packed, Cout, Cin, Cin, Kh, Kw, c.Kwp, c.Npad, c.Kpad, s));
            fpc_net tmp1;
            tmp1.B = B; tmp1.ws = packed; tmp1.splitk_off = lay.packed;
            ConvArgs a1;
            fill_conv_args(&tmp1, a1, c, p, Hi, Wi, Ho, Wo, sb, sh, sw, sc, relu != 0, 0);
            a1.Cin = 8 * c.Cinp; a1.Kw = 1; a1.K = c.K; a1.lanepx = 1;
            a1.p[0] = ConvPtrs{in, packed, out, scale, shift, nullptr, nullptr, nullptr};
            return launch_stem_pool(a1, packed, out, Ho / 2, Wo / 2, s);
        }
        FPC_TRY(launch_pack_weight_bf3(w_oihw, packed, Cout, Cin, Cin, Kh, Kw, c.Kwp, c.Npad, c.Kpad, s));
        fpc_net tmp0;
        tmp0.B = B; tmp0.ws = packed; tmp0.splitk_off = lay.packed;
        ConvArgs a0;
        fill_conv_args(&tmp0, a0, c, p, Hi, Wi, Ho, Wo, sb, sh, sw, sc, relu != 0, 0);
        a0.Cin = 8 * c.Cinp; a0.Kw = 1; a0.K = c.K; a0.lanepx = 1;
        a0.p[0] = ConvPtrs{in, packed, out, scale, shift, nullptr, nullptr, nullptr};
        return launch_conv_plan(a0, p, 1, s);
    }
    static_assert(FPC_IGEMM_DMA_B, "the split-precision direct form stages its B rows from the bf16 planes by LDS-DMA; a build that loads "
                                   "them from the f32 image must pack that image here as well");
    if (!wino && !p.bf3 && !p.h3) FPC_TRY(launch_pack_weight(w_oihw, packed, Cout, Cin, Cin, Kh, Kw, Kw, c.Npad, c.Kpad, s));
    if (!wino && p.bf3) FPC_TRY(launch_pack_weight_bf3(w_oihw, packed, Cout, Cin, Cin, Kh, Kw, Kw, c.Npad, c.Kpad, s));
    if (!wino && p.h3) FPC_TRY(launch_pack_weight_h3(w_oihw, packed, Cout, Cin, Cin, Kh, Kw, Kw, c.Npad, c.Kpad, s));
    int mode = (sc == 1 && Cin % kConvBK == 0 && Kh * Kw <= 32 && ((int64_t)Hi + 2 * pad) * sh * 4 < ((int64_t)1 << 31)) ? 0
               : (sc == 1 && Cin % 4 == 0 && sw % 4 == 0 && sh % 4 == 0 && sb % 4 == 0 && ((uintptr_t)in & 15) == 0) ? 2 : 1;
    fpc_net tmp;
    tmp.B = B;
    tmp.ws = packed;
    tmp.splitk_off = lay.packed;
    ConvArgs a;
    fill_conv_args(&tmp, a, c, p, Hi, Wi, Ho, Wo, sb, sh, sw, sc, relu != 0, mode);
    a.p[0] = ConvPtrs{in, packed, out, scale, shift, res, up, gn_part};
    a.zeros = nullptr;
    a.tickets = nullptr;
    if (lay.tickets) {
        float* tk = packed + lay.packed + lay.splitk + lay.wino;
        a.tickets = (int*)tk;
        if (hipMemsetAsync(tk, 0, kConvTickets * sizeof(int), s) != hipSuccess) return FPC_ELAUNCH;
    }
    if (wino && relu == 77) { a.dbg = gn_part; a.p[0].gn_part = nullptr; a.relu = 0; }
#ifdef FPC_STAMP_IGEMM
    if (!wino && relu == 77) { a.dbg = gn_part; a.p[0].gn_part = nullptr; a.relu = 0; }
#endif
    if (wino) {
        if (Kh != 3 || stride != 1 || pad != 1 || Cin % 8 || Cout % 64 || sc != 1 || up || sw != Cin ||
            sh != (int64_t)Wi * Cin || sb != (int64_t)Hi * Wi * Cin)
            return FPC_EINVAL;
        float* wp = packed + lay.packed + lay.splitk;
        if (nsplit == -6 && Cout % 128) return FPC_EINVAL;
        if (nsplit > -5) FPC_TRY(launch_wino_pack(w_oihw, wp, Cout, Cin, s));
        if (nsplit == -5 || nsplit == -7) FPC_TRY(launch_wino_pack_bf3(w_oihw, wp + (size_t)16 * Cout * Cin, Cout, Cin, s));
        if (nsplit == -6) FPC_TRY(launch_wino_pack_c128(w_oihw, wp + (size_t)40 * Cout * Cin, Cout, Cin, s));
        if (nsplit == -9) FPC_TRY(launch_wino_pack_h3(w_oihw, wp + (size_t)(Cout % 128 == 0 ? 80 : 56) * Cout * Cin + 8, Cout, Cin, s));
        if (nsplit == -8) FPC_TRY(launch_wino_pack_h2(w_oihw, wp + (size_t)(Cout % 128 == 0 ? 64 : 40) * Cout * Cin, Cout, Cin, s));
        a.wino_w[0] = wp;
        a.zeros = zero_page();
        if (!a.zeros) {
            float* zp = wp + lay.wino - 64;
            if (hipMemsetAsync(zp, 0, 64 * sizeof(float), s) != hipSuccess) return FPC_ELAUNCH;
            a.zeros = zp;
        }
        p.wino = -nsplit;
        return launch_conv_plan(a, p, 1, s);
    }
    if (p.h3) {
        if (mode != 0) return FPC_EINVAL;
        a.h3_w[0] = packed;
        return launch_conv_plan(a, p, 1, s);
    }
    a.bf3 = (p.bf3 && mode == 0) ? 1 : 0;
    if (p.bf3 && mode != 0) return FPC_EINVAL;
    if (p.lat || p.pw) return launch_conv_plan(a, p, 1, s);
    return run_conv(nullptr, a, 1, 0, s);
}
```

fastposecnn_amd/csrc/net_kernels.hpp:

```cpp
#pragma once
#include "common.hpp"

namespace fpc {

#ifndef FPC_IGEMM_DMA_B
#define FPC_IGEMM_DMA_B 1
#endif

constexpr int kMaxGroup = 4;
constexpr int kConvBK = 32;
constexpr int kConvNAlign = 128;
constexpr int kConvTickets = 16384;

struct ConvPtrs {
    const float* in;
    const float* w;
    float* out;
    const float* scale;
    const float* shift;
    const float* res;
    const float* up;
    float* gn_part;
};

struct ConvArgs {
    ConvPtrs p[kMaxGroup];
    float* splitk_ws;
    int* tickets;
    int fused;
    int B, Hi, Wi, Cin, Ho, Wo, Cout, Npad, Kh, Kw, stride, pad, K, Kpad;
    long long in_sb, in_sh, in_sw, in_sc;
    int relu, nsplit, mtiles, ntiles, ksteps, bm, bn, generic, groups;
    int bf3;
    int h3;
    int lanepx;
    const float* wino_w[kMaxGroup];
    const float* h3_w[kMaxGroup];
    const float* zeros;
    const float* fold_in;
    const float* fold_w[kMaxGroup];
    const float* fold_w2[kMaxGroup];
    const float* fold_up[kMaxGroup];
    const float* fold_tab[kMaxGroup];
    int fold_cin;
    float fold_lat_ms;
    void* dbg;
};

struct LatArgs {
    const float* in;
    const unsigned short* wpl[kMaxGroup];
    float* out[kMaxGroup];
    const float* shift[kMaxGroup];
    const float* up[kMaxGroup];
    int B, Ho, Wo, Cout, Npad, Kpad, groups, relu;
    unsigned bias_mask;
    int parts;
    int h3;
};
int launch_lateral1x1(const LatArgs& a, hipStream_t s);

struct PwArgs {
    const float* in;
    const unsigned short* wpl[kMaxGroup];
    float* out[kMaxGroup];
    const float* scale[kMaxGroup];
    const float* shift[kMaxGroup];
    const float* res[kMaxGroup];
    const float* up[kMaxGroup];
    long long in_sb, in_sh, in_sw;
    int B, Ho, Wo, Cin, Cout, Npad, Kpad, stride, groups, relu;
    int has_scale, has_shift, has_res, has_up;
    int variant;
};
int launch_conv1x1(const PwArgs& a, hipStream_t s);
inline int pw_tile_pixels(int variant) { return variant == 0 ? 64 : 128; }

struct StemArgs {
    const float* in;
    const unsigned short* wpl;
    float* out;
    const float* scale;
    const float* shift;
    int B, Hi, Wi, Ho, Wo, Cout, Npad, Kpad, relu;
    int grid;
};
int launch_stem7x7(const StemArgs& a, hipStream_t s);

struct StemPoolArgs {
    const float* in;
    const unsigned short* wpl;
    float* out;
    const float* scale;
    const float* shift;
    int B, Hi, Wi, Ho, Wo, Hp, Wp, Npad, Kpad, relu;
    int band;
    int grid;
};
constexpr int kStemPoolBand = 10;
int launch_stem_pool_h3(const StemPoolArgs& a, hipStream_t s);
void stem_pool_tasks(int Ho, int Wo, int band, long long out4[4]);

constexpr int kMaxGnSites = 4;
struct GnFinArgs {
    const float* gn_part[kMaxGnSites * kMaxGroup];
    const float* gamma[kMaxGnSites * kMaxGroup];
    const float* beta[kMaxGnSites * kMaxGroup];
    float* affine[kMaxGnSites * kMaxGroup];
    int P[kMaxGnSites];
    long long count[kMaxGnSites];
    int B, C, groups, sites;
    float eps;
};

constexpr int kMaxUpJobs = 2;
struct GnUpArgs {
    const float* in[kMaxUpJobs * kMaxGroup];
    const float* affine[kMaxUpJobs * kMaxGroup];
    float* out[kMaxUpJobs * kMaxGroup];
    int h[kMaxUpJobs], w[kMaxUpJobs];
    int B, C, jobs;
};

struct MergeHeadArgs {
    const float* t_lo[kMaxGroup][3];
    const float* a_lo[kMaxGroup][3];
    const float* t_hi[kMaxGroup];
    const float* a_hi[kMaxGroup];
    const float* hw[kMaxGroup];
    const float* hb[kMaxGroup];
    float* out[kMaxGroup];
    int ch[kMaxGroup];
    int chp[kMaxGroup];
    int B, h, w, C;
};

struct HeadPartArgs {
    const float* t[kMaxGroup][3];
    const float* aff[kMaxGroup][3];
    const float* hw[kMaxGroup];
    const float* hb[kMaxGroup];
    const float* lsum[kMaxGroup];
    float* out[kMaxGroup];
    int ch[kMaxGroup], chp[kMaxGroup];
    int B, H, W, C, hl, wl;
};
int launch_head_part(const HeadPartArgs& a, bool hi, int groups, hipStream_t s);

struct Up4Args {
    const float* lm; const float* lq; const float* lt; const float* ls;
    int pm, pq, pt, ps;
    float* o_mask; float* o_quat; float* o_scales; float* o_xy; float* o_z;
    long long* cat_mask; float* cq; float* cs; float* cxy; float* cz;
    int B, hl, wl, H, W, C;
    unsigned long long* fg_bits; size_t fg_stride;
};

struct WinoArgs {
    ConvPtrs p[kMaxGroup];
    long long* dbg;
    const float* zeros;
    int variant;
    int groups;
    int waves;
    int B, H, W, Cin, Cout, relu, tbx, tby;
    const float* in2[kMaxGroup];
    const float* w2[kMaxGroup];
    const float* btab[kMaxGroup];
    int fold, Cin2;
};
int launch_conv_wino(const WinoArgs& a, int groups, hipStream_t s);
const float* zero_page();
int launch_wino_pack(const float* w_oihw, float* packed, int Cout, int Cin, hipStream_t s);
int launch_wino_pack_bf3(const float* w_oihw, float* packed, int Cout, int Cin, hipStream_t s);
int launch_conv_wino_c128(const WinoArgs& a, int groups, hipStream_t s);
int launch_wino_pack_c128(const float* w_oihw, float* packed, int Cout, int Cin, hipStream_t s);
int launch_conv_wino_w4(const WinoArgs& a, int groups, hipStream_t s);
int launch_conv_wino_h2(const WinoArgs& a, int groups, hipStream_t s);
int launch_wino_pack_h2(const float* w_oihw, float* packed, int Cout, int Cin, hipStream_t s);
int launch_absmax_bits(const float* w, long long n, unsigned* out_bits, hipStream_t s);
int launch_conv_wino_h3(const WinoArgs& a, int groups, hipStream_t s);
int launch_wino_pack_h3(const float* w_oihw, float* packed, int Cout, int Cin, hipStream_t s);
int launch_wino_pack_h3_pair(const float* w1, float* packed1, int Cin1, const float* w2, float* packed2, int Cin2, int Cout, hipStream_t s);
int launch_fold_compose(const float* W, const float* L, const float* bias, float* wc, float* btab, int Cout, int Cmid, int Cin,
                        hipStream_t s);
int launch_conv(const ConvArgs& a, int groups, hipStream_t s);
int launch_conv_splitk_epilogue(const ConvArgs& a, int groups, hipStream_t s);
int launch_maxpool3x3s2(const float* in, float* out, int B, int Hi, int Wi, int C, int Ho, int Wo, hipStream_t s);
int launch_gn_finalize(const GnFinArgs& a, int groups, hipStream_t s);
int launch_gn_relu_up2(const GnUpArgs& a, int groups, hipStream_t s);
int launch_merge_head(const MergeHeadArgs& a, int groups, hipStream_t s);
int launch_up4_compress(const Up4Args& a, hipStream_t s);
void launch_up4_compress7x4(const Up4Args& a, hipStream_t s);

struct Lerp { int i0, i1; float l0, l1; };
__device__ __forceinline__ Lerp lerp_coord(int dst, int in, int out) {
    float scale = out > 1 ? (float)(in - 1) / (float)(out - 1) : 0.f;
    float src = scale * (float)dst;
    Lerp L;
    L.i0 = (int)src;
    L.i1 = L.i0 + (L.i0 < in - 1 ? 1 : 0);
    L.l1 = src - (float)L.i0;
    L.l0 = 1.f - L.l1;
    return L;
}

__device__ __forceinline__ Lerp lerp_scaled(int dst, int in, float scale) {
    float src = scale * (float)dst;
    Lerp L;
    L.i0 = (int)src;
    L.i1 = L.i0 + (L.i0 < in - 1 ? 1 : 0);
    L.l1 = src - (float)L.i0;
    L.l0 = 1.f - L.l1;
    return L;
}

int launch_pack_weight(const float* w_oihw, float* packed, int Cout, int Cin, int Cinp, int Kh, int Kw, int Kwp, int Npad,
                       int Kpad, hipStream_t s);
int launch_pack_weight_bf3(const float* w_oihw, float* packed, int Cout, int Cin, int Cinp, int Kh, int Kw, int Kwp, int Npad,
                           int Kpad, hipStream_t s);
inline size_t conv_packed_floats(int Npad, int Kpad) { return ((size_t)Npad * Kpad * 5 / 2 + 63) / 64 * 64; }
int launch_pack_weight_h3(const float* w_oihw, float* packed, int Cout, int Cin, int Cinp, int Kh, int Kw, int Kwp, int Npad,
                          int Kpad, hipStream_t s);
inline size_t h3_packed_floats(int Npad, int Kpad) { return ((size_t)Npad * Kpad + 2 + 63) / 64 * 64; }
int launch_nchw3_to_nhwc4(const float* x, float* out, int B, int HW, hipStream_t s);
int launch_fold_bn(const float* gamma, const float* beta, const float* mean, const float* var, float eps, int C,
                   float* scale, float* shift, hipStream_t s);

}
```

fastposecnn_amd/csrc/wino_h3.hip:

```cpp
#include <algorithm>
#include <cstdlib>
#include <type_traits>
#include "net_kernels.hpp"

namespace fpc {

typedef float f32x16 __attribute__((ext_vector_type(16)));
typedef unsigned u32x4 __attribute__((ext_vector_type(4)));
typedef _Float16 f16x8 __attribute__((ext_vector_type(8)));
typedef __fp16 fp16x2 __attribute__((ext_vector_type(2)));

namespace {

constexpr int kTX = 8, kTY = 8;
constexpr int kRW = 2 * kTX + 2, kRH = 2 * kTY + 2;
constexpr int kBN = 64;
constexpr int kNT = kTX * kTY;
constexpr int kInPieces = 18;
constexpr int kInFloats = kInPieces * 256;
constexpr int kRing = 4;
constexpr int kPairBytes = 16 * 2 * 2 * 64 * 16;
constexpr int kLdsFloats = 4 * 2 * kNT * kBN;
static_assert(kLdsFloats >= kRing * kInFloats, "the K loop's input ring lives in the output image's space");

__device__ __forceinline__ __amdgpu_buffer_rsrc_t make_rsrc(const void* base) {
    return __builtin_amdgcn_make_buffer_rsrc(const_cast<void*>(base), 0, 0x7FFFFFFF, 0x00020000);
}
__device__ __forceinline__ f32x4 fma_s4(float s, f32x4 b, f32x4 a) {
    return f32x4{__builtin_fmaf(s, b[0], a[0]), __builtin_fmaf(s, b[1], a[1]), __builtin_fmaf(s, b[2], a[2]), __builtin_fmaf(s, b[3], a[3])};
}
__device__ __forceinline__ const float* sgpr_ptr(const float* p) {
    const unsigned long long v = reinterpret_cast<unsigned long long>(p);
    const unsigned lo = __builtin_amdgcn_readfirstlane((unsigned)v), hi = __builtin_amdgcn_readfirstlane((unsigned)(v >> 32));
    return reinterpret_cast<const float*>(((unsigned long long)hi << 32) | lo);
}
__device__ __forceinline__ f32x4 sub_s4(f32x4 a, f32x4 b) { return f32x4{a[0] - b[0], a[1] - b[1], a[2] - b[2], a[3] - b[3]}; }
__device__ __forceinline__ f32x4 add_s4(f32x4 a, f32x4 b) { return f32x4{a[0] + b[0], a[1] + b[1], a[2] + b[2], a[3] + b[3]}; }

}

template <int VAR, bool FOLD>
__global__ __launch_bounds__(256, 1) void k_conv_wino_h3(const WinoArgs a) {
    __shared__ __attribute__((aligned(16))) float lds[kLdsFloats];
    const long long t_entry = a.dbg ? clock64() : 0;
    const int t = threadIdx.x, lane = t & 63;
    const int wi = __builtin_amdgcn_readfirstlane(t >> 6);
    const int li = lane & 31, lh = lane >> 5;
    const int H = a.H, W = a.W, Cout = a.Cout, HW = H * W;
    int bid = blockIdx.x;
    const int nnb = Cout / kBN;
    const int nb = bid % nnb; bid /= nnb;
    const int grp = bid % a.groups; bid /= a.groups;
    const int bx = bid % a.tbx; bid /= a.tbx;
    const int by = bid % a.tby;
    const int b = bid / a.tby;
    ConvPtrs P = a.p[0];
    if (grp == 1) P = a.p[1];
    if (grp == 2) P = a.p[2];
    if (grp == 3) P = a.p[3];
    const int ty0 = by * kTY, tx0 = bx * kTX;
    const int y_in0 = 2 * ty0 - 1, x_in0 = 2 * tx0 - 1;

    f32x16 acc[4][2][2];
    float inv_s = 1.f;
    long long t_issued = 0, t_landed = 0, t_synced = 0, c_begin = 0, r_begin = 0;
    const bool stamp = a.dbg != nullptr;

    auto kloop = [&](auto ph, const float* src, const float* wimg, const int Cs, const int up) __attribute__((always_inline)) {
    constexpr int PH = decltype(ph)::value;
    constexpr bool SKIPC = PH == 1;
    const int nkb = Cs >> 3;
    const int npair = nkb >> 1;
    const __amdgpu_buffer_rsrc_t rs_w = make_rsrc(reinterpret_cast<const char*>(wimg) + (size_t)nb * npair * kPairBytes);
    inv_s = wimg[(size_t)nnb * npair * (kPairBytes / 4)];
    const int vo_u = lane * 16;
    int so_u = wi * 4 * 4096;
    u32x4 U1[4][2], U2[4][2];
#define FPC_H3_XI_LIVE(J) (!(SKIPC && (J) == 2))
#define FPC_H3_LOAD_U1_AT(SO, J, NT) do { if (FPC_H3_XI_LIVE(J)) U1[J][NT] = __builtin_bit_cast(u32x4, __builtin_amdgcn_raw_buffer_load_b128(rs_w, vo_u, (SO) + (J) * 4096 + (NT) * 2048, 0)); } while (0)
#define FPC_H3_LOAD_U2_AT(SO, J, NT) do { if (FPC_H3_XI_LIVE(J)) U2[J][NT] = __builtin_bit_cast(u32x4, __builtin_amdgcn_raw_buffer_load_b128(rs_w, vo_u, (SO) + (J) * 4096 + (NT) * 2048 + 1024, 0)); } while (0)
#define FPC_H3_LOAD_U1(J, NT) FPC_H3_LOAD_U1_AT(so_u, J, NT)
#define FPC_H3_LOAD_U2(J, NT) FPC_H3_LOAD_U2_AT(so_u, J, NT)
#pragma unroll
    for (int j = 0; j < 4; ++j)
#pragma unroll
        for (int nt = 0; nt < 2; ++nt) { FPC_H3_LOAD_U1(j, nt); FPC_H3_LOAD_U2(j, nt); }
    if (npair > 1) so_u += kPairBytes;

    const int Hs = H >> up, Ws = W >> up;
    const float* isb = sgpr_ptr(src + (size_t)b * Hs * Ws * Cs);
    unsigned ivo[5];
    bool iok[5];
#pragma unroll
    for (int i = 0; i < 5; ++i) {
        const int slot = (wi + 4 * i) * 64 + lane;
        const int blk = slot >> 4, res = slot & 15, cell = blk >> 3;
        const int ah = (cell / 3) * 4 + (res & 3), qh = (cell % 3) * 4 + (res >> 2);
        const int hf = blk & 1;
        const int ry = 2 * ah + ((blk >> 2) & 1), rx = 2 * qh + ((blk >> 1) & 1);
        const int y = y_in0 + ry, x = x_in0 + rx;
        iok[i] = wi + 4 * i < kInPieces && ah <= kTY && qh <= kTX && y >= 0 && y < H && x >= 0 && x < W;
        ivo[i] = iok[i] ? (unsigned)((((size_t)(y >> up) * Ws + (x >> up)) * Cs + 4 * hf) * sizeof(float)) : 0u;
    }
#pragma clang diagnostic push
#pragma clang diagnostic ignored "-Winline-asm"
#define FPC_LDS_ADDR(PTR) ((unsigned)(size_t)(__attribute__((address_space(3))) void*)(PTR))
    unsigned long long imask[5];
#pragma unroll
    for (int i = 0; i < 5; ++i) imask[i] = __ballot(iok[i]);
#define FPC_H3_ISSUE_IN(BUF, PTR)                                                                             \
    do {                                                                                                      \
        unsigned long long sv_;                                                                               \
        const unsigned l0_ = FPC_LDS_ADDR(lds + (BUF) * kInFloats + wi * 256);                                \
        asm volatile("s_mov_b64 %0, exec\n"                                                                   \
                     "s_mov_b64 exec, %1\n s_mov_b32 m0, %6\n s_nop 0\n global_load_lds_dwordx4 %11, %16\n"   \
                     "s_mov_b64 exec, %2\n s_mov_b32 m0, %7\n s_nop 0\n global_load_lds_dwordx4 %12, %16\n"   \
                     "s_mov_b64 exec, %3\n s_mov_b32 m0, %8\n s_nop 0\n global_load_lds_dwordx4 %13, %16\n"   \
                     "s_mov_b64 exec, %4\n s_mov_b32 m0, %9\n s_nop 0\n global_load_lds_dwordx4 %14, %16\n"   \
                     "s_mov_b64 exec, %5\n s_mov_b32 m0, %10\n s_nop 0\n global_load_lds_dwordx4 %15, %16\n"  \
                     "s_mov_b64 exec, %0\n"                                                                   \
                     : "=&s"(sv_)                                                                             \
                     : "s"(imask[0]), "s"(imask[1]), "s"(imask[2]), "s"(imask[3]), "s"(imask[4]),             \
                       "s"(l0_), "s"(l0_ + 4096), "s"(l0_ + 8192), "s"(l0_ + 12288), "s"(l0_ + 16384),        \
                       "v"(ivo[0]), "v"(ivo[1]), "v"(ivo[2]), "v"(ivo[3]), "v"(ivo[4]), "s"(PTR)              \
                     : "memory", "m0");                                                                       \
    } while (0)

    const int tyl = li >> 3, txl = li & 7;
    const int ra = (wi == 0) ? 0 : (wi == 2 ? 2 : 1);
    const int rb = (wi == 0) ? 2 : (wi == 1 ? 2 : (wi == 2 ? 1 : 3));
    const float sgn = (wi == 1) ? 1.f : -1.f;
    auto unit = [&](int r, int ch) {
        const int ah = tyl + (r >> 1), qh = txl + ch;
        return ((((ah >> 2) * 3 + (qh >> 2)) * 8 + (r & 1) * 4 + lh) * 16 + 4 * (qh & 3) + (ah & 3)) * 4;
    };
    constexpr int in_cs = 2 * 16 * 4;
    constexpr int in_ms = 3 * 8 * 16 * 4;
    const int in_a[2] = {unit(ra, 0), unit(ra, 1)}, in_b[2] = {unit(rb, 0), unit(rb, 1)};

    if (y_in0 < 0 || x_in0 < 0 || y_in0 + kRH > H || x_in0 + kRW > W) {
        for (int i = t; i < kRing * kInFloats / 4; i += 256) reinterpret_cast<f32x4*>(lds)[i] = f32x4{0.f, 0.f, 0.f, 0.f};
        asm volatile("s_waitcnt lgkmcnt(0)" ::: "memory");
        __syncthreads();
    }
    FPC_H3_ISSUE_IN(0, isb);
    isb += 8;
    FPC_H3_ISSUE_IN(1, isb);
    isb += 8;
    FPC_H3_ISSUE_IN(2, nkb > 2 ? isb : isb - 8);
    isb += 8;
    int sn = 3;
#pragma unroll
    for (int j = 0; j < 4; ++j)
#pragma unroll
        for (int mt = 0; mt < 2; ++mt)
#pragma unroll
            for (int nt = 0; nt < 2; ++nt)
#pragma unroll
                for (int r = 0; r < 16; ++r)
                    if (PH == 0) acc[j][mt][nt][r] = 0.f;

    t_issued = stamp ? clock64() : 0;
    asm volatile("s_waitcnt vmcnt(10)" ::: "memory");
    t_landed = stamp ? clock64() : 0;
    __syncthreads();
    t_synced = stamp ? clock64() : 0;

    u32x4 TA1[4][2], TA2[4][2];
    f32x4 vn[2][4];
    float m1;
    asm volatile("s_mov_b32 %0, 0xbf800000" : "=s"(m1));
#define FPC_H3_SPLIT_PAIR(J, MT, PAIR, HALF) FPC_H3_SPLIT_PAIR_V(vn, J, MT, PAIR, HALF)
#define FPC_H3_SPLIT_PAIR_V(V, J, MT, PAIR, HALF)                                                             \
    if (FPC_H3_XI_LIVE(J)) do {                                                                               \
        const float x0_ = V[MT][J][2 * (PAIR)], x1_ = V[MT][J][2 * (PAIR) + 1];                               \
        const fp16x2 h_ = __builtin_amdgcn_cvt_pkrtz(x0_, x1_);                                               \
                                                          \
        const float r0_ = VAR == 1 ? x0_ - (float)h_[0] : __builtin_fmaf((float)h_[0], m1, x0_);              \
        const float r1_ = VAR == 1 ? x1_ - (float)h_[1] : __builtin_fmaf((float)h_[1], m1, x1_);              \
        const unsigned k1_ = __builtin_bit_cast(unsigned, h_);                                                \
        const unsigned k2_ = __builtin_bit_cast(unsigned, __builtin_amdgcn_cvt_pkrtz(r0_, r1_));              \
        asm volatile("" :: "v"(k1_), "v"(k2_));                                                               \
        TA1[J][MT][2 * (HALF) + (PAIR)] = k1_; TA2[J][MT][2 * (HALF) + (PAIR)] = k2_;                         \
    } while (0)
#pragma unroll
    for (int j = 0; j < 4; ++j)
#pragma unroll
        for (int mt = 0; mt < 2; ++mt) { TA1[j][mt] = u32x4{0u, 0u, 0u, 0u}; TA2[j][mt] = u32x4{0u, 0u, 0u, 0u}; }
    {
#pragma unroll
        for (int mt = 0; mt < 2; ++mt) {
            f32x4 e[4];
#pragma unroll
            for (int c = 0; c < 4; ++c)
                e[c] = fma_s4(sgn, *reinterpret_cast<const f32x4*>(lds + in_b[c >> 1] + (c & 1) * in_cs + mt * in_ms),
                              *reinterpret_cast<const f32x4*>(lds + in_a[c >> 1] + (c & 1) * in_cs + mt * in_ms));
            vn[mt][0] = sub_s4(e[0], e[2]); vn[mt][1] = add_s4(e[1], e[2]); vn[mt][2] = sub_s4(e[2], e[1]); vn[mt][3] = sub_s4(e[1], e[3]);
#pragma unroll
            for (int j = 0; j < 3; ++j) { FPC_H3_SPLIT_PAIR(j, mt, 0, 0); FPC_H3_SPLIT_PAIR(j, mt, 1, 0); }
        }
    }
    asm volatile("s_waitcnt vmcnt(0)" ::: "memory");
    __syncthreads();

#define FPC_H3_MFMA(J, MT, NT, A, B) do { if (FPC_H3_XI_LIVE(J)) acc[J][MT][NT] = __builtin_amdgcn_mfma_f32_32x32x16_f16(__builtin_bit_cast(f16x8, A), __builtin_bit_cast(f16x8, B), acc[J][MT][NT], 0, 0, 0); } while (0)
#define FPC_H3_PIN4(V) asm volatile("" :: "v"(V))
#define FPC_H3_SPLIT_Q(J, Q, HALF) do { if ((Q) == 0) FPC_H3_SPLIT_PAIR(J, 0, 0, HALF); if ((Q) == 1) FPC_H3_SPLIT_PAIR(J, 0, 1, HALF); if ((Q) == 2) FPC_H3_SPLIT_PAIR(J, 1, 0, HALF); if ((Q) == 3) FPC_H3_SPLIT_PAIR(J, 1, 1, HALF); } while (0)
    c_begin = stamp ? clock64() : 0; r_begin = stamp ? wall_clock64() : 0;
#pragma unroll 1
    for (int p = 0; p < npair; ++p) {
        {
            const float* InE = lds + ((2 * p + 1) & 3) * kInFloats;
            f32x4 ea[2][4], eb[2][4];
#pragma unroll
            for (int mt = 0; mt < 2; ++mt)
#pragma unroll
                for (int c = 0; c < 4; ++c) {
                    ea[mt][c] = *reinterpret_cast<const f32x4*>(InE + in_a[c >> 1] + (c & 1) * in_cs + mt * in_ms);
                    eb[mt][c] = *reinterpret_cast<const f32x4*>(InE + in_b[c >> 1] + (c & 1) * in_cs + mt * in_ms);
                }
            __builtin_amdgcn_sched_barrier(0);
            if (sn < nkb) { FPC_H3_ISSUE_IN((sn & 3), isb); isb += 8; }
            if (sn + 1 < nkb) { FPC_H3_ISSUE_IN(((sn + 1) & 3), isb); isb += 8; }
            sn += 2;
#pragma unroll
            for (int q = 0; q < 4; ++q) FPC_H3_SPLIT_Q(3, q, 0);
            __builtin_amdgcn_sched_barrier(0);
#pragma unroll
            for (int mt = 0; mt < 2; ++mt) {
                f32x4 e[4];
#pragma unroll
                for (int c = 0; c < 4; ++c) e[c] = fma_s4(sgn, eb[mt][c], ea[mt][c]);
                vn[mt][0] = sub_s4(e[0], e[2]); vn[mt][1] = add_s4(e[1], e[2]); vn[mt][2] = sub_s4(e[2], e[1]); vn[mt][3] = sub_s4(e[1], e[3]);
                FPC_H3_SPLIT_PAIR(0, mt, 0, 1); FPC_H3_SPLIT_PAIR(0, mt, 1, 1);
            }
        }
        __builtin_amdgcn_sched_barrier(0);
        const float* In = lds + ((2 * p + 2) & 3) * kInFloats;
        f32x4 da[2][4], db[2][4], e[2][4];
        __builtin_amdgcn_s_setprio(1);
#pragma unroll
        for (int j = 0; j < 4; ++j)
#pragma unroll
            for (int g = 0; g < 3; ++g)
#pragma unroll
                for (int mt = 0; mt < 2; ++mt)
#pragma unroll
                    for (int nt = 0; nt < 2; ++nt) {
                        const int sl = 12 * j + 4 * g + 2 * mt + nt;
                        if (g == 0) FPC_H3_MFMA(j, mt, nt, TA1[j][mt], U1[j][nt]);
                        if (g == 1) {
                            FPC_H3_MFMA(j, mt, nt, TA2[j][mt], U1[j][nt]);
                            if (mt == 1) FPC_H3_LOAD_U1(j, nt);
                        }
                        if (g == 2) {
                            FPC_H3_MFMA(j, mt, nt, TA1[j][mt], U2[j][nt]);
                            if (mt == 1) FPC_H3_LOAD_U2(j, nt);
                        }
                        if (sl < 4) {
#pragma unroll
                            for (int c = 2 * (sl & 1); c < 2 * (sl & 1) + 2; ++c) {
                                da[sl >> 1][c] = *reinterpret_cast<const f32x4*>(In + in_a[c >> 1] + (c & 1) * in_cs + (sl >> 1) * in_ms);
                                db[sl >> 1][c] = *reinterpret_cast<const f32x4*>(In + in_b[c >> 1] + (c & 1) * in_cs + (sl >> 1) * in_ms);
                            }
                        }
                        if (sl >= 4 && sl < 12) {
                            const int m_ = (sl - 4) >> 2, c = (sl - 4) & 3;
                            e[m_][c] = fma_s4(sgn, db[m_][c], da[m_][c]);
                            FPC_H3_PIN4(e[m_][c]);
                        }
                        if (sl < 4) FPC_H3_SPLIT_Q(1, sl, 1);
                        if (sl >= 4 && sl < 8) FPC_H3_SPLIT_Q(2, sl - 4, 1);
                        if (sl >= 8 && sl < 12) FPC_H3_SPLIT_Q(3, sl - 8, 1);
                        if (sl >= 12 && sl < 20 && !(SKIPC && ((sl - 12) & 3) == 2)) {
                            const int m_ = (sl - 12) >> 2, jx = (sl - 12) & 3;
                            if (jx == 0) vn[m_][0] = sub_s4(e[m_][0], e[m_][2]);
                            if (jx == 1) vn[m_][1] = add_s4(e[m_][1], e[m_][2]);
                            if (jx == 2) vn[m_][2] = sub_s4(e[m_][2], e[m_][1]);
                            if (jx == 3) vn[m_][3] = sub_s4(e[m_][1], e[m_][3]);
                            FPC_H3_PIN4(vn[m_][jx]);
                        }
                        if (sl >= 20 && sl < 24) FPC_H3_SPLIT_Q(0, sl - 20, 0);
                        if (sl >= 24 && sl < 28) FPC_H3_SPLIT_Q(1, sl - 24, 0);
                        if (sl >= 36 && sl < 40) FPC_H3_SPLIT_Q(2, sl - 36, 0);
                        __builtin_amdgcn_sched_barrier(0);
                    }
        __builtin_amdgcn_s_setprio(0);
        so_u += p + 2 < npair ? kPairBytes : 0;
        if (PH == 0) asm volatile("s_waitcnt vmcnt(16)" ::: "memory");
        if (PH == 1) asm volatile("s_waitcnt vmcnt(12)" ::: "memory");
        __syncthreads();
    }
#undef FPC_H3_MFMA
#undef FPC_H3_SPLIT_PAIR
#undef FPC_H3_SPLIT_PAIR_V
#undef FPC_H3_SPLIT_Q
#undef FPC_H3_PIN4
#undef FPC_H3_ISSUE_IN
#undef FPC_H3_LOAD_U1
#undef FPC_H3_LOAD_U2
#undef FPC_H3_LOAD_U1_AT
#undef FPC_H3_LOAD_U2_AT
#undef FPC_H3_XI_LIVE
#undef FPC_LDS_ADDR
#pragma clang diagnostic pop
    };

    if (!FOLD) {
        kloop(std::integral_constant<int, 0>(), P.in, P.w, a.Cin, 0);
    } else {
        kloop(std::integral_constant<int, 0>(), P.in, P.w, a.Cin, 0);
        const float* w2 = a.w2[0];
        const float* in2 = a.in2[0];
        if (grp == 1) { w2 = a.w2[1]; in2 = a.in2[1]; }
        if (grp == 2) { w2 = a.w2[2]; in2 = a.in2[2]; }
        if (grp == 3) { w2 = a.w2[3]; in2 = a.in2[3]; }
        kloop(std::integral_constant<int, 1>(), in2, w2, a.Cin2, 1);
    }
    const long long t_kend = a.dbg ? clock64() : 0;
    if (a.dbg && lane == 0) {
        long long* o = a.dbg + ((size_t)blockIdx.x * 4 + wi) * 8;
        o[0] = t_issued - t_entry; o[1] = t_landed - t_issued; o[2] = t_synced - t_landed;
        o[3] = t_kend - c_begin; o[4] = wall_clock64() - r_begin; o[5] = a.Cin >> 3; o[6] = c_begin - t_entry;
    }

    const int oq = t & 15, otl = t >> 4;
    const int n = nb * kBN + oq * 4;
    const f32x4 e_sc = P.scale ? *reinterpret_cast<const f32x4*>(P.scale + n) : f32x4{1.f, 1.f, 1.f, 1.f};
    const f32x4 e_sh = P.shift ? *reinterpret_cast<const f32x4*>(P.shift + n) : f32x4{0.f, 0.f, 0.f, 0.f};
    const float* btab = a.btab[0];
    if (grp == 1) btab = a.btab[1];
    if (grp == 2) btab = a.btab[2];
    if (grp == 3) btab = a.btab[3];
    f32x4 e_res[4][4];
#pragma unroll
    for (int tp = 0; tp < 4; ++tp)
#pragma unroll
        for (int q = 0; q < 4; ++q) {
            const int ot = otl + 16 * tp;
            const int y = 2 * (ty0 + (ot >> 3)) + (q >> 1), x = 2 * (tx0 + (ot & 7)) + (q & 1);
            e_res[tp][q] = (P.res && y < H && x < W) ? *reinterpret_cast<const f32x4*>(P.res + ((size_t)b * HW + (size_t)y * W + x) * Cout + n)
                                                     : f32x4{0.f, 0.f, 0.f, 0.f};
        }
    __syncthreads();
    float* const zb = lds + ((wi * 2) * kNT + 4 * lh) * kBN + li;
#pragma unroll
    for (int mt = 0; mt < 2; ++mt)
#pragma unroll
        for (int nt = 0; nt < 2; ++nt)
#pragma unroll
            for (int r = 0; r < 16; ++r) {
                const int mc = mt * 32 + (r & 3) + 8 * (r >> 2);
                const float m0 = acc[0][mt][nt][r], m1 = acc[1][mt][nt][r], m2 = acc[2][mt][nt][r], m3 = acc[3][mt][nt][r];
                zb[(0 * kNT + mc) * kBN + nt * 32] = m0 + m1 + m2;
                zb[(1 * kNT + mc) * kBN + nt * 32] = m1 - m2 - m3;
            }
    __syncthreads();
    f32x4 s1 = {0.f, 0.f, 0.f, 0.f}, s2 = {0.f, 0.f, 0.f, 0.f};
#pragma unroll
    for (int tp = 0; tp < 4; ++tp) {
        const int ot = otl + 16 * tp;
        const int oty = ty0 + (ot >> 3), otx = tx0 + (ot & 7);
        f32x4 z[4][2];
#pragma unroll
        for (int i = 0; i < 4; ++i)
#pragma unroll
            for (int cc = 0; cc < 2; ++cc) z[i][cc] = *reinterpret_cast<const f32x4*>(lds + ((i * 2 + cc) * kNT + ot) * kBN + oq * 4);
#pragma unroll
        for (int rr = 0; rr < 2; ++rr)
#pragma unroll
            for (int cc = 0; cc < 2; ++cc) {
                const int y = 2 * oty + rr, x = 2 * otx + cc;
                if (y >= H || x >= W) continue;
                f32x4 val = (rr == 0 ? z[0][cc] + z[1][cc] + z[2][cc] : z[1][cc] - z[2][cc] - z[3][cc]) * inv_s;
                if (FOLD) {
                    const int cls = (((y == 0) | ((y == H - 1) << 1)) << 2) | (x == 0) | ((x == W - 1) << 1);
                    val += *reinterpret_cast<const f32x4*>(btab + (size_t)cls * Cout + n);
                }
                if (P.scale) val = val * e_sc;
                val = val + e_sh;
                const size_t o = ((size_t)b * HW + (size_t)y * W + x) * Cout + n;
                if (P.res) val += e_res[tp][2 * rr + cc];
                if (a.relu) { val[0] = fmaxf(val[0], 0.f); val[1] = fmaxf(val[1], 0.f); val[2] = fmaxf(val[2], 0.f); val[3] = fmaxf(val[3], 0.f); }
                *reinterpret_cast<f32x4*>(P.out + o) = val;
                s1 += val;
                s2 += val * val;
            }
    }
    if (P.gn_part) {
#pragma unroll
        for (int o = 16; o < 64; o <<= 1)
#pragma unroll
            for (int k = 0; k < 4; ++k) { s1[k] += __shfl_xor(s1[k], o, 64); s2[k] += __shfl_xor(s2[k], o, 64); }
        __syncthreads();
        float* red = lds;
        if (lane < 16) {
#pragma unroll
            for (int k = 0; k < 4; ++k) { red[(wi * kBN + oq * 4 + k) * 2] = s1[k]; red[(wi * kBN + oq * 4 + k) * 2 + 1] = s2[k]; }
        }
        __syncthreads();
        if (t < kBN) {
            float u1 = 0.f, u2 = 0.f;
#pragma unroll
            for (int w = 0; w < 4; ++w) { u1 += red[(w * kBN + t) * 2]; u2 += red[(w * kBN + t) * 2 + 1]; }
            const int Pn = a.tbx * a.tby;
            float* g = P.gn_part + (((size_t)b * Pn + by * a.tbx + bx) * Cout + nb * kBN + t) * 2;
            g[0] = u1; g[1] = u2;
        }
    }
    if (a.dbg && lane == 0) {
        asm volatile("s_waitcnt vmcnt(0)" ::: "memory");
        a.dbg[((size_t)blockIdx.x * 4 + wi) * 8 + 7] = clock64() - t_kend;
    }
}

__global__ __launch_bounds__(256) void k_wino_pack_h3(const float* __restrict__ w, unsigned short* __restrict__ out, float* __restrict__ tail,
                                                      int Cout, int Cin) {
    const float wmax = __builtin_bit_cast(float, reinterpret_cast<const unsigned*>(tail)[1]);
    int ex = 0;
    if (wmax > 0.f && wmax < 3.0e38f) { (void)frexpf(2.25f * wmax, &ex); ex = 13 - ex; }
    ex = max(-100, min(100, ex));
    const float sc = ldexpf(1.0f, ex);
    if (blockIdx.x == 0 && threadIdx.x == 0) tail[0] = ldexpf(1.0f, -ex);
    const long long total = (long long)Cout * Cin;
    for (long long g = (long long)blockIdx.x * blockDim.x + threadIdx.x; g < total; g += (long long)gridDim.x * blockDim.x) {
        const int ci = (int)(g % Cin), co = (int)(g / Cin);
        const float* k = w + ((size_t)co * Cin + ci) * 9;
        float gg[4][3];
#pragma unroll
        for (int c = 0; c < 3; ++c) {
            const float g0 = k[c] * sc, g1 = k[3 + c] * sc, g2 = k[6 + c] * sc;
            gg[0][c] = g0;
            gg[1][c] = 0.5f * (g0 + g1 + g2);
            gg[2][c] = 0.5f * (g0 - g1 + g2);
            gg[3][c] = g2;
        }
        const int nb = co >> 6, col = co & 63, nt = col >> 5, kb = ci >> 3, cil = ci & 7, e = cil & 3;
        const int ln = (cil >> 2) * 32 + (col & 31);
        unsigned short* img = out + ((size_t)nb * (Cin >> 4) + (kb >> 1)) * (kPairBytes / 2);
#pragma unroll
        for (int i = 0; i < 4; ++i) {
            const float r0 = gg[i][0], r1 = gg[i][1], r2 = gg[i][2];
            const float u[4] = {r0, 0.5f * (r0 + r1 + r2), 0.5f * (r0 - r1 + r2), r2};
#pragma unroll
            for (int jx = 0; jx < 4; ++jx) {
                const float x = u[jx];
                const fp16x2 h = __builtin_amdgcn_cvt_pkrtz(x, 0.f);
                const float r = x - (float)h[0];
                const fp16x2 h2 = __builtin_amdgcn_cvt_pkrtz(r, 0.f);
                unsigned short* frag = img + ((4 * i + jx) * 4096 + nt * 2048 + ln * 16) / 2;
                frag[(kb & 1) * 4 + e] = (unsigned short)(__builtin_bit_cast(unsigned, h) & 0xFFFFu);
                frag[512 + (kb & 1) * 4 + e] = (unsigned short)(__builtin_bit_cast(unsigned, h2) & 0xFFFFu);
            }
        }
    }
}

int launch_conv_wino_h3(const WinoArgs& a, int groups, hipStream_t s) {
    if (groups < 1 || groups > kMaxGroup || a.Cin % 16 != 0 || a.Cout % kBN != 0) return FPC_EINVAL;
    if ((long long)a.H * a.W * a.Cin * (long long)sizeof(float) >= (1LL << 32)) return FPC_EINVAL;
    if ((long long)(a.Cin >> 4) * kPairBytes >= (1LL << 31)) return FPC_EINVAL;
    if (a.tbx != cdiv(cdiv(a.W, 2), kTX) || a.tby != cdiv(cdiv(a.H, 2), kTY)) return FPC_EINVAL;
    const long long nblk = (long long)a.tbx * a.tby * a.B * (a.Cout / kBN) * groups;
    if (nblk < 1 || nblk >= (1LL << 31)) return FPC_EINVAL;
    if (a.fold) {
        if (a.Cin2 % 16 != 0 || (a.H | a.W) & 1 || (long long)(a.H / 2) * (a.W / 2) * a.Cin2 * (long long)sizeof(float) >= (1LL << 32) ||
            (long long)(a.Cin2 >> 4) * kPairBytes >= (1LL << 31) || a.relu || a.dbg)
            return FPC_EINVAL;
        for (int g = 0; g < groups; ++g)
            if (!a.in2[g] || !a.w2[g] || !a.btab[g] || a.p[g].scale || a.p[g].shift || a.p[g].res || a.p[g].up) return FPC_EINVAL;
        hipLaunchKernelGGL((k_conv_wino_h3<0, true>), dim3((unsigned)nblk), dim3(256), 0, s, a);
        return check_launch();
    }
    static const int var = getenv("FPC_H3_VAR") ? atoi(getenv("FPC_H3_VAR")) : 0;
    if (var == 1) hipLaunchKernelGGL((k_conv_wino_h3<1, false>), dim3((unsigned)nblk), dim3(256), 0, s, a);
    else hipLaunchKernelGGL((k_conv_wino_h3<0, false>), dim3((unsigned)nblk), dim3(256), 0, s, a);
    return check_launch();
}

__global__ __launch_bounds__(256) void k_fold_compose(const float* __restrict__ w, const float* __restrict__ l, const float* __restrict__ bias,
                                                      float* __restrict__ wc, float* __restrict__ btab, int Cout, int Cmid, int Cin) {
    const int g = blockIdx.x * blockDim.x + threadIdx.x;
    const int nw = Cout * Cin * 9;
    if (g < nw) {
        const int tap = g % 9, k = (g / 9) % Cin, o = g / (9 * Cin);
        double acc = 0.0;
        for (int c = 0; c < Cmid; ++c) acc += (double)w[((size_t)o * Cmid + c) * 9 + tap] * (double)l[(size_t)c * Cin + k];
        wc[g] = (float)acc;
    } else if (g < nw + 16 * Cout) {
        const int o = (g - nw) % Cout, cls = (g - nw) / Cout, rc = cls >> 2, cc = cls & 3;
        double acc = 0.0;
        for (int ky = (rc & 1); ky < 3 - ((rc >> 1) & 1); ++ky)
            for (int kx = (cc & 1); kx < 3 - ((cc >> 1) & 1); ++kx)
                for (int c = 0; c < Cmid; ++c) acc += (double)w[((size_t)o * Cmid + c) * 9 + ky * 3 + kx] * (double)bias[c];
        btab[(size_t)cls * Cout + o] = (float)acc;
    }
}

int launch_fold_compose(const float* W, const float* L, const float* bias, float* wc, float* btab, int Cout, int Cmid, int Cin,
                        hipStream_t s) {
    if (!W || !L || !bias || !wc || !btab || Cout < 1 || Cmid < 1 || Cin < 1) return FPC_EINVAL;
    const long long work = (long long)Cout * Cin * 9 + 16LL * Cout;
    hipLaunchKernelGGL(k_fold_compose, dim3((unsigned)((work + 255) / 256)), dim3(256), 0, s, W, L, bias, wc, btab, Cout, Cmid, Cin);
    return check_launch();
}

int launch_wino_pack_h3_pair(const float* w1, float* packed1, int Cin1, const float* w2, float* packed2, int Cin2, int Cout, hipStream_t s) {
    if (Cin1 % 16 != 0 || Cin2 % 16 != 0 || Cout % kBN != 0 || ((uintptr_t)w1 & 15) || ((uintptr_t)w2 & 15)) return FPC_EINVAL;
    float* tail1 = packed1 + (size_t)16 * Cout * Cin1;
    float* tail2 = packed2 + (size_t)16 * Cout * Cin2;
    if (hipMemsetAsync(tail1, 0, 2 * sizeof(float), s) != hipSuccess || hipMemsetAsync(tail2, 0, 2 * sizeof(float), s) != hipSuccess)
        return FPC_ELAUNCH;
    for (float* tail : {tail1, tail2}) {
        int rc = launch_absmax_bits(w1, (long long)Cout * Cin1 * 9, reinterpret_cast<unsigned*>(tail) + 1, s);
        if (!rc) rc = launch_absmax_bits(w2, (long long)Cout * Cin2 * 9, reinterpret_cast<unsigned*>(tail) + 1, s);
        if (rc) return rc;
    }
    hipLaunchKernelGGL(k_wino_pack_h3, dim3((unsigned)std::min<long long>(((long long)Cout * Cin1 + 255) / 256, 4096)), dim3(256), 0, s, w1,
                       reinterpret_cast<unsigned short*>(packed1), tail1, Cout, Cin1);
    int rc = check_launch();
    if (rc) return rc;
    hipLaunchKernelGGL(k_wino_pack_h3, dim3((unsigned)std::min<long long>(((long long)Cout * Cin2 + 255) / 256, 4096)), dim3(256), 0, s, w2,
                       reinterpret_cast<unsigned short*>(packed2), tail2, Cout, Cin2);
    return check_launch();
}

int launch_wino_pack_h3(const float* w_oihw, float* packed, int Cout, int Cin, hipStream_t s) {
    if (Cin % 16 != 0 || Cout % kBN != 0) return FPC_EINVAL;
    float* tail = packed + (size_t)16 * Cout * Cin;
    if (hipMemsetAsync(tail, 0, 2 * sizeof(float), s) != hipSuccess) return FPC_ELAUNCH;
    if ((uintptr_t)w_oihw & 15) return FPC_EINVAL;
    const int rc = launch_absmax_bits(w_oihw, (long long)Cout * Cin * 9, reinterpret_cast<unsigned*>(tail) + 1, s);
    if (rc) return rc;
    const long long work = (long long)Cout * Cin;
    hipLaunchKernelGGL(k_wino_pack_h3, dim3((unsigned)std::min<long long>((work + 255) / 256, 4096)), dim3(256), 0, s, w_oihw,
                       reinterpret_cast<unsigned short*>(packed), tail, Cout, Cin);
    return check_launch();
}

}
```

fastposecnn_amd/engine.py:

```python
import ctypes
import operator

import torch

from fastposecnn_amd import _native as nat


_DATA_PTR = torch.Tensor.data_ptr
_VERSION = operator.attrgetter('_version')

class NetEngine:

    def __init__(self, model, B, H, W, device, autotune=True, tune_mode=0, graph=False, split_precision=False):
        L = nat.lib()
        self._lib = L
        self.B, self.H, self.W, self.device = B, H, W, device
        self.classes = model.classes
        h = ctypes.c_void_p()
        from fastposecnn_amd.lib import backbone
        block, layers = backbone.encoder_layout(model.encoder.name)
        if block == 1:
            nat.check(L.fpc_net_create(model.encoder.name.encode(), self.classes, B, H, W, ctypes.byref(h)), "fpc_net_create")
        else:
            nat.check(L.fpc_net_create_encoder(block, (ctypes.c_int * 4)(*layers), self.classes, B, H, W, ctypes.byref(h)),
                      "fpc_net_create_encoder")
        self._h = h
        self._names = [L.fpc_net_param_name(h, i).decode() for i in range(L.fpc_net_param_count(h))]
        nbytes = L.fpc_net_workspace_bytes(h)
        with torch.cuda.device(device):
            self._ws = torch.empty(nbytes, dtype=torch.uint8, device=device)
            assert self._ws.data_ptr() % 256 == 0
        self.reloads = 0
        self.generation = 0
        self.bind(model)
        if split_precision:
            nat.check(L.fpc_net_set_split_precision(h, int(split_precision)), "fpc_net_set_split_precision")
        if autotune:
            nat.check(L.fpc_net_autotune_next(h, int(tune_mode)), "fpc_net_autotune_next")
            self.forward(torch.zeros((B, 3, H, W), dtype=torch.float32, device=device), want_logits=False)
        if graph:
            nat.check(L.fpc_net_set_graph(h, 1), "fpc_net_set_graph")

    def bind(self, model):
        L, h, device = self._lib, self._h, self.device
        tensors = dict(model.named_parameters())
        tensors.update(dict(model.named_buffers()))
        params = []
        for i, name in enumerate(self._names):
            if name not in tensors:
                raise RuntimeError(f"fastposecnn_amd: the model has no parameter {name!r} (smp naming expected)")
            t = tensors[name]
            if t.device != device or t.dtype != torch.float32 or not t.is_contiguous():
                raise RuntimeError(f"fastposecnn_amd: parameter {name!r} must be a contiguous f32 tensor on {device}")
            if t.numel() != L.fpc_net_param_numel(h, i):
                raise RuntimeError(f"fastposecnn_amd: parameter {name!r} has {t.numel()} elements, expected "
                                   f"{L.fpc_net_param_numel(h, i)}")
            params.append(t)
        self._params = params
        n = len(params)
        ptrs = (ctypes.c_void_p * n)(*[t.data_ptr() for t in params])
        with torch.cuda.device(device):
            nat.check(L.fpc_net_load_params(h, ptrs, n, self._ws.data_ptr(), self._ws.numel(), nat.stream()),
                      "fpc_net_load_params")
        self._stamp = self._fingerprint()
        self.reloads += 1

    def _fingerprint(self):
        return (tuple(map(_DATA_PTR, self._params)), tuple(map(_VERSION, self._params)))

    def stale(self):
        return self._fingerprint() != self._stamp

    def conv_plans(self):
        out = []
        buf = (ctypes.c_int * 5)()
        for i in range(self._lib.fpc_net_conv_count(self._h)):
            self._lib.fpc_net_conv_plan(self._h, i, buf)
            out.append(tuple(buf))
        return out

    def copy_plans_from(self, other):
        nat.check(self._lib.fpc_net_copy_plans(self._h, other._h), "fpc_net_copy_plans")

    def force_winograd(self, form):
        rc = self._lib.fpc_net_force_winograd(self._h, int(form))
        if rc < 0:
            nat.check(rc, "fpc_net_force_winograd")
        return rc

    def force_fold(self, on):
        rc = self._lib.fpc_net_force_fold(self._h, int(on))
        if rc < 0:
            nat.check(rc, "fpc_net_force_fold")
        return rc

    def force_direct_h3(self, on):
        rc = self._lib.fpc_net_force_direct_h3(self._h, int(on))
        if rc < 0:
            nat.check(rc, "fpc_net_force_direct_h3")
        return rc

    def force_stem_pool(self, on):
        rc = self._lib.fpc_net_force_stem_pool(self._h, int(on))
        if rc < 0:
            nat.check(rc, "fpc_net_force_stem_pool")
        return rc

    def force_pointwise(self, on):
        rc = self._lib.fpc_net_force_pointwise(self._h, int(on))
        if rc < 0:
            nat.check(rc, "fpc_net_force_pointwise")
        return rc

    def flops(self):
        buf = (ctypes.c_double * 3)()
        nat.check(self._lib.fpc_net_flops(self._h, buf), "fpc_net_flops")
        return tuple(buf)

    def __del__(self):
        h = getattr(self, "_h", None)
        if h:
            self._lib.fpc_net_destroy(h)
            self._h = None

    def forward(self, x, want_logits=True):
        B, H, W, C, dev = self.B, self.H, self.W, self.classes, self.device
        G = C - 1
        if tuple(x.shape) != (B, 3, H, W) or x.device != dev:
            raise RuntimeError("NetEngine.forward: input shape / device does not match the plan")
        if x.dtype != torch.float32 or not x.is_contiguous():
            x = x.float().contiguous()
        f32 = dict(dtype=torch.float32, device=dev)
        logits = None
        lp = [None] * 5
        if want_logits:
            logits = {'mask': torch.empty((B, C, H, W), **f32), 'quaternion': torch.empty((B, 4 * G, H, W), **f32),
                      'scales': torch.empty((B, 3 * G, H, W), **f32), 'xy': torch.empty((B, 2 * G, H, W), **f32),
                      'z': torch.empty((B, G, H, W), **f32)}
            lp = [logits[k].data_ptr() for k in ('mask', 'quaternion', 'scales', 'xy', 'z')]
        cat = {'mask': torch.empty((B, H, W), dtype=torch.int64, device=dev),
               'quaternion': torch.empty((B, 4, H, W), **f32), 'scales': torch.empty((B, 3, H, W), **f32),
               'xy': torch.empty((B, 2, H, W), **f32), 'z': torch.empty((B, H, W), **f32)}
        bits = None
        if W % 64 == 0 and self._lib.fpc_cc_bits_supported(B, H, W):
            bits = torch.empty((B, self._lib.fpc_mask_bits_words(H, W)), dtype=torch.int64, device=dev)
        with torch.cuda.device(dev):
            nat.check(self._lib.fpc_net_forward_bits(self._h, x.data_ptr(), *lp, cat['mask'].data_ptr(),
                                                     cat['quaternion'].data_ptr(), cat['scales'].data_ptr(),
                                                     cat['xy'].data_ptr(), cat['z'].data_ptr(), nat.ptr(bits), nat.stream()),
                      "fpc_net_forward_bits")
        if bits is not None:
            cat['mask']._fpc_fg_bits = (bits, cat['mask']._version)
        return logits, cat

    def tensor(self, name):
        p = ctypes.c_void_p()
        H, W, C = ctypes.c_int(), ctypes.c_int(), ctypes.c_int()
        nat.check(self._lib.fpc_net_tensor(self._h, name.encode(), ctypes.byref(p), ctypes.byref(H), ctypes.byref(W),
                                           ctypes.byref(C)), "fpc_net_tensor")
        off = p.value - self._ws.data_ptr()
        n = self.B * H.value * W.value * C.value
        return self._ws[off:off + 4 * n].view(torch.float32).view(self.B, H.value, W.value, C.value)
```

include/fpc.h:

```cpp
#ifndef FPC_H_
#define FPC_H_

#include <stddef.h>
#include <stdint.h>

#ifdef __cplusplus
extern "C" {
#endif

#define FPC_ABI_VERSION 11

#define FPC_OK 0
#define FPC_EINVAL (-1)
#define FPC_EWORKSPACE (-2)
#define FPC_ELAUNCH (-3)
#define FPC_EDEVICE (-4)
#define FPC_EFORMAT (-5)

typedef void* fpc_stream_t;

int fpc_abi_version(void);
const char* fpc_error_string(int code);
const char* fpc_last_hip_error(void);

int fpc_generate_hypothesis(const float* direct, const float* coords, const int32_t* idxs,
                            float* hyp, int tn, int vn, int hn, fpc_stream_t stream);

int fpc_voting_for_hypothesis(const float* direct, const float* coords, const float* hyp,
                              uint8_t* inliers, int tn, int vn, int hn, float inlier_thresh,
                              fpc_stream_t stream);

size_t fpc_ransac_workspace_bytes(int n, int H, int W, int hn);
int fpc_ransac_voting_v3(const float* mask, const float* vertex,
                         int64_t vs_n, int64_t vs_h, int64_t vs_w, int64_t vs_c,
                         int n, const int32_t* n_dev, int H, int W, int hn,
                         const int32_t* idxs, const uint8_t* keep, uint64_t seed,
                         float inlier_thresh, int min_num, int max_num,
                         float* out_xy, int32_t* out_tn, int32_t* out_win_idx,
                         int32_t* out_win_count, int32_t* out_inl_count,
                         float* out_hyp, int32_t* out_counts, double* out_refine,
                         void* ws, size_t ws_bytes, fpc_stream_t stream);
int fpc_ransac_voting_v3_bits(const float* mask, const uint64_t* mask_bits, const float* vertex,
                              int64_t vs_n, int64_t vs_h, int64_t vs_w, int64_t vs_c,
                              int n, const int32_t* n_dev, int H, int W, int hn,
                              const int32_t* idxs, const uint8_t* keep, uint64_t seed,
                              float inlier_thresh, int min_num, int max_num,
                              float* out_xy, int32_t* out_tn, int32_t* out_win_idx,
                              int32_t* out_win_count, int32_t* out_inl_count,
                              float* out_hyp, int32_t* out_counts, double* out_refine,
                              void* ws, size_t ws_bytes, fpc_stream_t stream);

int fpc_ransac_voting_v3_pose(const float* mask, const uint64_t* mask_bits, const float* vertex,
                              int64_t vs_n, int64_t vs_h, int64_t vs_w, int64_t vs_c,
                              int n, const int32_t* n_dev, int H, int W, int hn,
                              const int32_t* idxs, const uint8_t* keep, uint64_t seed,
                              float inlier_thresh, int min_num, int max_num,
                              float* out_xy, int32_t* out_tn, int32_t* out_win_idx,
                              int32_t* out_win_count, int32_t* out_inl_count,
                              float* out_hyp, int32_t* out_counts, double* out_refine,
                              const float* pose_q, const float* pose_z, const float* pose_kinv,
                              float* pose_R, float* pose_T, float* pose_RT,
                              void* ws, size_t ws_bytes, fpc_stream_t stream);

int fpc_vote_set_prune(int mode, int npass, const int32_t* cum16);
int fpc_vote_prune_info(const void* ws, size_t ws_bytes, int n, int H, int W, int hn, int32_t* out, fpc_stream_t stream);

int fpc_class_compress(const float* mask_logits, const float* quat, const float* scales,
                       const float* xy, const float* z, const int64_t* cat_mask_in,
                       int B, int C, int HW,
                       int64_t* cat_mask, float* oq, float* os, float* oxy, float* oz,
                       fpc_stream_t stream);
int fpc_class_compress_bits(const float* mask_logits, const float* quat, const float* scales,
                            const float* xy, const float* z, const int64_t* cat_mask_in,
                            int B, int C, int HW,
                            int64_t* cat_mask, float* oq, float* os, float* oxy, float* oz,
                            uint64_t* fg_bits, fpc_stream_t stream);


size_t fpc_cc_workspace_bytes(int B, int H, int W);
int fpc_cc_label(const int64_t* cat_mask, int B, int H, int W,
                 int32_t* labels, int32_t* n_out, int32_t* root_pix, int cap,
                 void* ws, size_t ws_bytes, fpc_stream_t stream);
int fpc_cc_bits_supported(int B, int H, int W);
int fpc_fg_bits(const int64_t* cat_mask, int B, int H, int W, uint64_t* fg_bits, fpc_stream_t stream);
int fpc_cc_label_bits(const uint64_t* fg_bits, int B, int H, int W, int32_t* labels, int32_t* n_out,
                      int32_t* root_pix, int cap, void* ws, size_t ws_bytes, fpc_stream_t stream);


size_t fpc_aggregate_workspace_bytes(int N);
int fpc_aggregate(const int32_t* labels, const int64_t* cat_mask,
                  const float* quat, const float* scales, const float* xy, const float* z,
                  int B, int H, int W, int N, const int32_t* n_dev,
                  int64_t* class_ids, int64_t* sample_ids, float* inst_masks,
                  float* oq, float* os, float* oz, float* oxy, float* out_stats,
                  void* ws, size_t ws_bytes, fpc_stream_t stream);
size_t fpc_mask_bits_words(int H, int W);
int fpc_aggregate_bits(const int32_t* labels, const int64_t* cat_mask,
                       const float* quat, const float* scales, const float* xy, const float* z,
                       int B, int H, int W, int N, const int32_t* n_dev,
                       int64_t* class_ids, int64_t* sample_ids, float* inst_masks,
                       float* oq, float* os, float* oz, float* oxy, float* out_stats, uint64_t* inst_bits,
                       const int32_t* root_pix, void* ws, size_t ws_bytes, fpc_stream_t stream);

int fpc_pose_rt(const float* q, const float* xy, const float* z, const float* kinv, int n,
                float* R, float* T, float* RT, fpc_stream_t stream);

int fpc_pack_pose_records(const int64_t* sample_ids, const int64_t* class_ids, const float* q, const float* scales,
                          const float* xy, const float* z, const float* R, const float* T, const float* RT, int n,
                          int sample_offset, int capacity, float* out, fpc_stream_t stream);

size_t fpc_mask_iou_workspace_bytes(int n1, int n2, int64_t hw);
int fpc_mask_iou(const void* masks1, int n1, const void* masks2, int n2, int64_t hw, int elem_size,
                 float* iou, int32_t* inter, int32_t* uni, void* ws, size_t ws_bytes, fpc_stream_t stream);

size_t fpc_preprocess_workspace_bytes(int B);
int fpc_preprocess_u8(const uint8_t* img_hwc, int B, int H, int W, const double* mean3, const double* std3,
                      int input_range_01, float* out_nchw, void* ws, size_t ws_bytes, fpc_stream_t stream);

int fpc_png_info(const uint8_t* data, size_t nbytes, int32_t* out5);
int fpc_png_decode(const uint8_t* data, size_t nbytes, void* out, size_t out_bytes, int mode);
int fpc_png_decode_batch(const uint8_t* const* datas, const size_t* sizes, int n, uint8_t* out, int H, int W, int threads);

int fpc_pose_errors(const float* q0, const float* q1, const int64_t* symmetric_ids, const float* rot, int nrot,
                    const float* RT1, const float* RT2, const float* scales1, const float* scales2,
                    const float* T1, const float* T2, int n, double* out_degree, float* out_iou3d, float* out_offset,
                    fpc_stream_t stream);

int fpc_post_network_backward(const int32_t* labels, const float* cat_xy, int B, int H, int W, int N,
                              const int32_t* n_dev, const double* table, float inlier_thresh, int max_num,
                              uint64_t seed, const uint8_t* keep, float* g_q, float* g_s, float* g_xy, float* g_z,
                              fpc_stream_t stream);
int fpc_vote_refine_backward(const float* mask, const float* vertex, int64_t vs_n, int64_t vs_h, int64_t vs_w,
                             int64_t vs_c, int n, int H, int W, const double* table, float inlier_thresh, int max_num,
                             uint64_t seed, const uint8_t* keep, float* g_vertex, fpc_stream_t stream);
int fpc_class_compress_backward(const int64_t* cat_mask, const float* quat, const float* xy, const float* go_q,
                                const float* go_s, const float* go_xy, const float* go_z, int B, int C, int HW,
                                float* g_q, float* g_s, float* g_xy, float* g_z, fpc_stream_t stream);
int fpc_mask_losses(const float* logits, const int64_t* target, int B, int C, int HW, int64_t ignore_ce,
                    int64_t ignore_cce, float alpha, float gamma, double* sums6, const float* w3, float* grad,
                    fpc_stream_t stream);
int fpc_grad_sumsq(const float* g, size_t n, double* out2, fpc_stream_t stream);
int fpc_lookahead_radam_step(float* p, const float* g, float* m, float* v, float* slow, size_t n, float lr, float beta1,
                             float beta2, float eps, float weight_decay, int64_t step, int la_k, float la_alpha,
                             const float* ctl, fpc_stream_t stream);

typedef struct fpc_net fpc_net_t;
int fpc_net_create(const char* encoder, int classes, int B, int H, int W, fpc_net_t** out);
int fpc_net_create_encoder(int block, const int* layers4, int classes, int B, int H, int W, fpc_net_t** out);
void fpc_net_destroy(fpc_net_t* net);
int fpc_net_param_count(const fpc_net_t* net);
const char* fpc_net_param_name(const fpc_net_t* net, int i);
int64_t fpc_net_param_numel(const fpc_net_t* net, int i);
size_t fpc_net_workspace_bytes(const fpc_net_t* net);
int fpc_net_load_params(fpc_net_t* net, const float* const* params, int count, void* ws, size_t ws_bytes,
                        fpc_stream_t stream);
int fpc_net_forward(fpc_net_t* net, const float* x, float* logits_mask, float* logits_quat,
                    float* logits_scales, float* logits_xy, float* logits_z, int64_t* cat_mask,
                    float* cq, float* cs, float* cxy, float* cz, fpc_stream_t stream);
int fpc_net_forward_bits(fpc_net_t* net, const float* x, float* logits_mask, float* logits_quat,
                         float* logits_scales, float* logits_xy, float* logits_z, int64_t* cat_mask,
                         float* cq, float* cs, float* cxy, float* cz, uint64_t* fg_bits, fpc_stream_t stream);

int fpc_net_autotune_next(fpc_net_t* net, int mode );
int fpc_net_set_split_precision(fpc_net_t* net, int on);
int fpc_net_set_graph(fpc_net_t* net, int on);
int fpc_net_graph_recorded(const fpc_net_t* net);
int fpc_net_conv_count(const fpc_net_t* net);
int fpc_net_conv_plan(const fpc_net_t* net, int i, int* out5);
int fpc_net_copy_plans(fpc_net_t* dst, const fpc_net_t* src);
int fpc_net_force_winograd(fpc_net_t* net, int form);
int fpc_net_force_pointwise(fpc_net_t* net, int on);
int fpc_net_force_fold(fpc_net_t* net, int on);
int fpc_net_force_direct_h3(fpc_net_t* net, int on);
int fpc_net_force_stem_pool(fpc_net_t* net, int on);
int fpc_stem_pool_tasks(int Ho, int Wo, int64_t* out4);
int fpc_net_flops(const fpc_net_t* net, double* out3);
int fpc_net_tensor(const fpc_net_t* net, const char* name, const float** ptr, int* H, int* W, int* C);

size_t fpc_conv2d_workspace_bytes(int B, int Ho, int Wo, int Cin, int Cout, int Kh, int Kw);
size_t fpc_conv2d_workspace_bytes_for(int B, int Ho, int Wo, int Cin, int Cout, int Kh, int Kw, int bm, int bn, int nsplit);
int fpc_conv2d_plan(int B, int Ho, int Wo, int Cin, int Cout, int Kh, int Kw, int bm, int bn, int nsplit,
                    int* out4 );
int fpc_conv2d(const float* in, int64_t sb, int64_t sh, int64_t sw, int64_t sc, const float* w_oihw,
               const float* scale, const float* shift, const float* res, const float* up, float* out,
               float* gn_part, int B, int Hi, int Wi, int Cin, int Cout, int Kh, int Kw, int stride, int pad,
               int relu, int bm, int bn, int nsplit, void* ws, size_t ws_bytes, fpc_stream_t stream);

size_t fpc_conv2d_wgrad_workspace_bytes(int B, int Ho, int Wo, int Cin, int Cout, int Kh, int Kw);
int fpc_conv2d_wgrad(const float* x, int64_t sb, int64_t sh, int64_t sw, const float* dy, float* dw, int B, int Hi,
                     int Wi, int Cin, int Cout, int Kh, int Kw, int stride, int pad, void* ws, size_t ws_bytes,
                     fpc_stream_t stream);
int fpc_conv2d_wgrad_split(const float* x, int64_t sb, int64_t sh, int64_t sw, const float* dy, float* dw, int B, int Hi,
                           int Wi, int Cin, int Cout, int Kh, int Kw, int stride, int pad, void* ws, size_t ws_bytes,
                           fpc_stream_t stream);

int fpc_upsample_bilinear_fwd(const float* in, int64_t sb, int64_t sc, int64_t sh, int64_t sw, float* out, int B, int C, int h,
                              int w, int scale, int out_nhwc, fpc_stream_t stream);
size_t fpc_upsample_bilinear_bwd_scratch_floats(int B, int C, int h, int w, int scale);
int fpc_upsample_bilinear_bwd(const float* dout, int64_t sb, int64_t sc, int64_t sh, int64_t sw, float* din, float* scratch,
                              int B, int C, int h, int w, int scale, int din_nhwc, fpc_stream_t stream);

size_t fpc_groupnorm4_relu_scratch_floats(int B, int HW, int C);
int fpc_groupnorm4_relu_fwd(const float* x, const float* gamma, const float* beta, float* y, float* stats, float* part, int B,
                            int HW, int C, int groups, float eps, fpc_stream_t stream);
int fpc_groupnorm4_relu_bwd(const float* x, const float* dy, const float* gamma, const float* beta, const float* stats, float* dx,
                            float* part, int B, int HW, int C, int groups, fpc_stream_t stream);

#ifdef __cplusplus
}
#endif
#endif
```

Baseline: 2593.

## Pack multiple batch images into shared Winograd h3 column tiles

Adds a packed mode to the Winograd h3 conv kernel that lays several batch images side by side along the tile-column axis. A block whose tile straddles an image boundary takes its halo and outputs from the next image. This removes partially empty edge tiles when the tile-column count is not a multiple of the tile width, cutting launched blocks and wasted work. It adds boundary handling, a different GroupNorm partial-sum layout with extra zeroed slots, and on-by-default behaviour, so correctness and register pressure are risks.

```diff
diff --git a/fastposecnn_amd/_native.py b/fastposecnn_amd/_native.py
--- a/fastposecnn_amd/_native.py
+++ b/fastposecnn_amd/_native.py
@@ -80,6 +80,9 @@
     "fpc_net_force_direct_h3": (_i, [_vp, _i]),
     "fpc_net_force_stem_pool": (_i, [_vp, _i]),
     "fpc_stem_pool_tasks": (_i, [_i, _i, ctypes.POINTER(_i64)]),
+    "fpc_wino_pack_geometry": (_i, [_i, _i, _i, _i, _i, ctypes.POINTER(_i64)]),
+    "fpc_net_set_wino_pack": (_i, [_vp, _i]),
+    "fpc_net_wino_blocks": (_i64, [_vp]),
     "fpc_net_graph_recorded": (_i, [_vp]),
     "fpc_net_flops": (_i, [_vp, ctypes.POINTER(ctypes.c_double)]),
     "fpc_net_tensor": (_i, [_vp, ctypes.c_char_p, ctypes.POINTER(_vp), ctypes.POINTER(_i), ctypes.POINTER(_i),
diff --git a/fastposecnn_amd/csrc/net.hip b/fastposecnn_amd/csrc/net.hip
--- a/fastposecnn_amd/csrc/net.hip
+++ b/fastposecnn_amd/csrc/net.hip
@@ -165,6 +165,8 @@
     int merge_split = -1;
     size_t splitk_off = 0, splitk_floats = 0;
     int use_graph = 0;
+    long long wino_blocks = 0;
+    int wino_pack = 1;
     int split_precision = 0;
     hipGraphExec_t graph_exec = nullptr;
     size_t zeros_off = 0;
@@ -413,6 +415,7 @@
         int HoWo = fh[seg_level[i]] * fw[seg_level[i]];
         plan(n->dec[0].seg[i], HoWo, 4);
         n->gn_P[i] = cdiv(HoWo, 128) * 4;
+        n->gn_P[i] = std::max(n->gn_P[i], wino_pack_geometry(fh[seg_level[i]], fw[seg_level[i]], B, n->convs[n->dec[0].seg[i]].Cin, true).gn_rows);
         for (int d = 0; d < 4; ++d) {
             n->gn_part_off[d][i] = n->alloc((size_t)B * n->gn_P[i] * 128 * 2);
             n->gn_aff_off[d][i] = n->alloc((size_t)B * 128 * 2);
@@ -452,6 +455,15 @@
 }
 
 extern "C" int fpc_net_graph_recorded(const fpc_net_t* n) { return n && n->use_graph && n->graph_exec ? 1 : 0; }
+
+extern "C" int fpc_net_set_wino_pack(fpc_net_t* n, int on) {
+    if (!n || on < 0 || on > 1) return FPC_EINVAL;
+    if (n->wino_pack != on && n->graph_exec) { (void)hipGraphExecDestroy(n->graph_exec); n->graph_exec = nullptr; }
+    n->wino_pack = on;
+    return FPC_OK;
+}
+
+extern "C" int64_t fpc_net_wino_blocks(const fpc_net_t* n) { return n ? (int64_t)n->wino_blocks : -1; }
 
 extern "C" int fpc_net_set_graph(fpc_net_t* n, int on) {
     if (!n) return FPC_EINVAL;
@@ -543,6 +555,7 @@
     a.zeros = n->ws + n->zeros_off;
     a.tickets = (int*)(n->ws + n->tickets_off);
     a.fused = p.fused;
+    a.wino_pack = n->wino_pack;
 }
 
 int launch_conv_plan(ConvArgs& a, const ConvPlan& p, int groups, hipStream_t s) {
@@ -606,6 +619,11 @@
         w.B = a.B; w.H = a.Ho; w.W = a.Wo; w.Cin = a.Cin; w.Cout = a.Cout; w.relu = a.relu;
         w.waves = (p.wino == 2 || p.wino == 4 || p.wino == 5 || p.wino == 7 || p.wino == 8 || p.wino == 9) ? 8 : 4;
         w.tbx = cdiv(cdiv(a.Wo, 2), 8); w.tby = cdiv(cdiv(a.Ho, 2), w.waves);
+        if (p.wino == 9) {
+            const WinoPackGeom q = wino_pack_geometry(a.Ho, a.Wo, a.B, a.Cin, a.wino_pack && !p.fold);
+            if (q.G > 1) { w.pack = q.G; w.tbx = q.tbx; w.pack_rx = q.rx; }
+            a.wino_blocks = q.patches * (a.Cout / 64) * groups;
+        }
         if (p.fold) {
             if (p.wino != 9 || !a.fold_in) return FPC_EINVAL;
             for (int g = 0; g < groups; ++g) {
@@ -643,7 +661,8 @@
     return rc;
 }
 
-int plan_gn_rows(const ConvPlan& p, int Ho, int Wo) {
+int plan_gn_rows(const ConvPlan& p, int Ho, int Wo, int B, int Cin, int pack) {
+    if (p.wino == 9) return wino_pack_geometry(Ho, Wo, B, Cin, pack && !p.fold).gn_rows;
     return p.wino ? cdiv(cdiv(Wo, 2), 8) * cdiv(cdiv(Ho, 2), (p.wino == 2 || p.wino == 4 || p.wino == 5 || p.wino == 7 || p.wino == 8 || p.wino == 9) ? 8 : 4) : p.mtiles * p.bm / 32;
 }
 
@@ -708,6 +727,7 @@
                 double nblk = q.stem ? 512.0
                               : q.lat ? (double)cdiv(a.Ho * a.Wo, 128) * a.B * q.lat
                               : q.pw ? (double)cdiv(a.B * a.Ho * a.Wo, pw_tile_pixels(q.pw - 1)) * (a.Cout / 64) * groups * q.pw
+                              : q.wino == 9 ? (double)wino_pack_geometry(a.Ho, a.Wo, a.B, a.Cin, a.wino_pack && !q.fold).patches * (a.Cout / 64) * groups
                               : q.wino ? (double)cdiv(cdiv(a.Wo, 2), 8) * cdiv(cdiv(a.Ho, 2), (q.wino == 2 || q.wino == 4 || q.wino == 5 || q.wino == 7 || q.wino == 8 || q.wino == 9) ? 8 : 4) * a.B * (a.Cout / (q.wino == 6 ? 128 : 64)) * groups
                                      : (double)q.mtiles * q.ntiles * q.nsplit * a.B * groups;
                 double slots = 256.0 * ((q.wino == 2 || q.wino == 4 || q.wino == 5 || q.wino == 6 || q.wino == 7 || q.wino == 8 || q.wino == 9) ? 1.0 : 2.0);
@@ -739,7 +759,9 @@
         n->cplan[ci] = best;
     }
     ConvPlan p = n ? n->cplan[ci] : ConvPlan{a.bm, a.bn, a.nsplit, a.mtiles, a.ntiles, 0, a.bf3, a.fused};
-    return launch_conv_plan(a, p, groups, s);
+    const int rc = launch_conv_plan(a, p, groups, s);
+    if (n && !rc && p.wino == 9) n->wino_blocks += a.wino_blocks;
+    return rc;
 }
 
 }
@@ -759,6 +781,7 @@
 
 static int forward_middle(fpc_net* n, hipStream_t s) {
     float* ws = n->ws;
+    n->wino_blocks = 0;
     const int B = n->B, H = n->H, W = n->W;
     ConvArgs a;
     auto nhwc = [&](const Act& t, long long& sb, long long& sh, long long& sw, long long& sc) {
@@ -924,7 +947,7 @@
                 g.beta[k * kMaxGroup + d] = n->pptr[n->dec[d].p_gn[si] + 1];
                 g.affine[k * kMaxGroup + d] = ws + n->gn_aff_off[d][si];
             }
-            g.P[k] = plan_gn_rows(n->cplan[n->dec[0].seg[si]], o0.H, o0.W);
+            g.P[k] = plan_gn_rows(n->cplan[n->dec[0].seg[si]], o0.H, o0.W, B, n->convs[n->dec[0].seg[si]].Cin, n->wino_pack);
             g.count[k] = (long long)o0.H * o0.W * 4;
             ++k;
         }
@@ -1230,6 +1253,14 @@
     return FPC_OK;
 }
 
+extern "C" int fpc_wino_pack_geometry(int H, int W, int B, int Cin, int fold, int64_t* out8) {
+    if (!out8 || H < 1 || W < 1 || B < 1 || Cin < 1) return FPC_EINVAL;
+    const WinoPackGeom q = wino_pack_geometry(H, W, B, Cin, !fold);
+    out8[0] = q.G; out8[1] = q.tbx; out8[2] = q.tby; out8[3] = q.patches; out8[4] = q.slots; out8[5] = q.tiles; out8[6] = q.gn_rows;
+    out8[7] = q.rx;
+    return FPC_OK;
+}
+
 extern "C" size_t fpc_conv2d_workspace_bytes(int B, int Ho, int Wo, int Cin, int Cout, int Kh, int Kw) {
     int K = Cin * Kh * Kw, Kpad = cdiv(K, kConvBK) * kConvBK, Npad = cdiv(Cout, kConvNAlign) * kConvNAlign;
     size_t packed = conv_packed_floats(Npad, Kpad);
@@ -1246,16 +1277,19 @@
     if (nsplit >= 2000) nsplit = 1;
     if (nsplit >= 1000) nsplit -= 1000;
     if (nsplit >= 100) nsplit -= 100;
+    const int pack = nsplit == -10;
+    if (pack) nsplit = -9;
     ConvPlan p = plan_conv(Ho * Wo, B, Cout, Kpad / kConvBK, 1, bm, bn, nsplit);
-    if (nsplit <= -1 && nsplit >= -9) { p.wino = -nsplit; p.nsplit = nsplit; }
-    out4[0] = p.bm; out4[1] = p.bn; out4[2] = p.nsplit; out4[3] = plan_gn_rows(p, Ho, Wo);
+    if (nsplit <= -1 && nsplit >= -9) { p.wino = -nsplit; p.nsplit = pack ? -10 : nsplit; }
+    out4[0] = p.bm; out4[1] = p.bn; out4[2] = p.nsplit; out4[3] = plan_gn_rows(p, Ho, Wo, B, Cin, pack);
     return FPC_OK;
 }
 
 namespace {
-struct Conv2dRequest { int nsplit; bool bf3, two_launch, wino; int lat; bool stem; int pw; bool h3; bool pool; };
+struct Conv2dRequest { int nsplit; bool bf3, two_launch, wino; int lat; bool stem; int pw; bool h3; bool pool; bool pack; };
 Conv2dRequest conv2d_request(int nsplit) {
-    Conv2dRequest r{nsplit, false, false, false, 0, false, 0, false, false};
+    Conv2dRequest r{nsplit, false, false, false, 0, false, 0, false, false, false};
+    if (r.nsplit == -10) { r.pack = true; r.nsplit = -9; }
     if (r.nsplit >= 7000 && r.nsplit < 8000) { r.lat = r.nsplit - 7000; r.h3 = true; r.nsplit = 1; return r; }
     if (r.nsplit >= 6000 && r.nsplit < 6200) {
         r.h3 = true; r.nsplit -= 6000;
@@ -1355,6 +1389,7 @@
                : (sc == 1 && Cin % 4 == 0 && sw % 4 == 0 && sh % 4 == 0 && sb % 4 == 0 && ((uintptr_t)in & 15) == 0) ? 2 : 1;
     fpc_net tmp;
     tmp.B = B;
+    tmp.wino_pack = rq.pack ? 1 : 0;
     tmp.ws = packed;
     tmp.splitk_off = lay.packed;
     ConvArgs a;
diff --git a/fastposecnn_amd/csrc/net_kernels.hpp b/fastposecnn_amd/csrc/net_kernels.hpp
--- a/fastposecnn_amd/csrc/net_kernels.hpp
+++ b/fastposecnn_amd/csrc/net_kernels.hpp
@@ -45,6 +45,8 @@
     int fold_cin;
     float fold_lat_ms;
     void* dbg;
+    long long wino_blocks;
+    int wino_pack;
 };
 
 struct LatArgs {
@@ -168,6 +170,7 @@
     const float* w2[kMaxGroup];
     const float* btab[kMaxGroup];
     int fold, Cin2;
+    int pack, pack_rx;
 };
 int launch_conv_wino(const WinoArgs& a, int groups, hipStream_t s);
 const float* zero_page();
@@ -180,6 +183,8 @@
 int launch_wino_pack_h2(const float* w_oihw, float* packed, int Cout, int Cin, hipStream_t s);
 int launch_absmax_bits(const float* w, long long n, unsigned* out_bits, hipStream_t s);
 int launch_conv_wino_h3(const WinoArgs& a, int groups, hipStream_t s);
+struct WinoPackGeom { int G, tbx, tby, rx; long long patches, slots, tiles; int gn_rows; };
+WinoPackGeom wino_pack_geometry(int H, int W, int B, int Cin, bool allow);
 int launch_wino_pack_h3(const float* w_oihw, float* packed, int Cout, int Cin, hipStream_t s);
 int launch_wino_pack_h3_pair(const float* w1, float* packed1, int Cin1, const float* w2, float* packed2, int Cin2, int Cout, hipStream_t s);
 int launch_fold_compose(const float* W, const float* L, const float* bias, float* wc, float* btab, int Cout, int Cmid, int Cin,
diff --git a/fastposecnn_amd/csrc/wino_h3.hip b/fastposecnn_amd/csrc/wino_h3.hip
--- a/fastposecnn_amd/csrc/wino_h3.hip
+++ b/fastposecnn_amd/csrc/wino_h3.hip
@@ -39,7 +39,7 @@
 
 }
 
-template <int VAR, bool FOLD>
+template <int VAR, bool FOLD, bool PACK>
 __global__ __launch_bounds__(256, 1) void k_conv_wino_h3(const WinoArgs a) {
     __shared__ __attribute__((aligned(16))) float lds[kLdsFloats];
     const long long t_entry = a.dbg ? clock64() : 0;
@@ -51,14 +51,33 @@
     const int nnb = Cout / kBN;
     const int nb = bid % nnb; bid /= nnb;
     const int grp = bid % a.groups; bid /= a.groups;
-    const int bx = bid % a.tbx; bid /= a.tbx;
-    const int by = bid % a.tby;
-    const int b = bid / a.tby;
+    int bx, by, b, tx0;
+    int pk_ks = 99, pk_raw = 99, pk_slot = 0;
+    bool pk_two = false;
+    if constexpr (!PACK) {
+        bx = bid % a.tbx; bid /= a.tbx;
+        by = bid % a.tby;
+        b = bid / a.tby;
+        tx0 = bx * kTX;
+    } else {
+        const int G = a.pack, tcw = (a.W + 1) >> 1, per = a.tbx * a.tby;
+        const int g = bid / per, rem = bid - g * per;
+        const int nf = min(G, a.B - g * G);
+        const int tbxg = min(a.tbx, (nf * tcw + kTX - 1) / kTX);
+        bx = rem % tbxg; by = rem / tbxg;
+        const int f = (kTX * bx) / tcw;
+        tx0 = kTX * bx - f * tcw;
+        b = g * G + f;
+        pk_raw = tcw - tx0;
+        pk_ks = pk_raw < kTX ? pk_raw : 99;
+        pk_two = pk_ks < kTX && f + 1 < nf;
+        pk_slot = bx - (f * tcw) / kTX;
+    }
     ConvPtrs P = a.p[0];
     if (grp == 1) P = a.p[1];
     if (grp == 2) P = a.p[2];
     if (grp == 3) P = a.p[3];
-    const int ty0 = by * kTY, tx0 = bx * kTX;
+    const int ty0 = by * kTY;
     const int y_in0 = 2 * ty0 - 1, x_in0 = 2 * tx0 - 1;
 
     f32x16 acc[4][2][2];
@@ -98,9 +117,13 @@
         const int ah = (cell / 3) * 4 + (res & 3), qh = (cell % 3) * 4 + (res >> 2);
         const int hf = blk & 1;
         const int ry = 2 * ah + ((blk >> 2) & 1), rx = 2 * qh + ((blk >> 1) & 1);
-        const int y = y_in0 + ry, x = x_in0 + rx;
-        iok[i] = wi + 4 * i < kInPieces && ah <= kTY && qh <= kTX && y >= 0 && y < H && x >= 0 && x < W;
-        ivo[i] = iok[i] ? (unsigned)((((size_t)(y >> up) * Ws + (x >> up)) * Cs + 4 * hf) * sizeof(float)) : 0u;
+        const bool far = PACK && qh > pk_ks;
+        const int y = y_in0 + ry, x = far ? rx - 2 * pk_ks - 3 : x_in0 + rx;
+        const int qmax = (PACK && pk_ks < kTX) ? kTX + 1 : kTX;
+        iok[i] = wi + 4 * i < kInPieces && ah <= kTY && qh <= qmax && y >= 0 && y < H && x >= 0 && x < W && (!far || pk_two);
+        ivo[i] = iok[i] ? (unsigned)((((size_t)(y >> up) * Ws + (x >> up)) * Cs + 4 * hf) * sizeof(float)) +
+                              (far ? (unsigned)((size_t)Hs * Ws * Cs * sizeof(float)) : 0u)
+                        : 0u;
     }
 #pragma clang diagnostic push
 #pragma clang diagnostic ignored "-Winline-asm"
@@ -126,7 +149,7 @@
                      : "memory", "m0");                                                                       \
     } while (0)
 
-    const int tyl = li >> 3, txl = li & 7;
+    const int tyl = li >> 3, txl = (li & 7) + ((PACK && (li & 7) >= pk_ks) ? 1 : 0);
     const int ra = (wi == 0) ? 0 : (wi == 2 ? 2 : 1);
     const int rb = (wi == 0) ? 2 : (wi == 1 ? 2 : (wi == 2 ? 1 : 3));
     const float sgn = (wi == 1) ? 1.f : -1.f;
@@ -138,7 +161,7 @@
     constexpr int in_ms = 3 * 8 * 16 * 4;
     const int in_a[2] = {unit(ra, 0), unit(ra, 1)}, in_b[2] = {unit(rb, 0), unit(rb, 1)};
 
-    if (y_in0 < 0 || x_in0 < 0 || y_in0 + kRH > H || x_in0 + kRW > W) {
+    if (y_in0 < 0 || x_in0 < 0 || y_in0 + kRH > H || x_in0 + kRW > W || (PACK && pk_ks < kTX)) {
         for (int i = t; i < kRing * kInFloats / 4; i += 256) reinterpret_cast<f32x4*>(lds)[i] = f32x4{0.f, 0.f, 0.f, 0.f};
         asm volatile("s_waitcnt lgkmcnt(0)" ::: "memory");
         __syncthreads();
@@ -324,7 +347,12 @@
         o[3] = t_kend - c_begin; o[4] = wall_clock64() - r_begin; o[5] = a.Cin >> 3; o[6] = c_begin - t_entry;
     }
 
-    const int oq = t & 15, otl = t >> 4;
+    const int lane_e = PACK ? (int)__builtin_amdgcn_mbcnt_hi(~0u, __builtin_amdgcn_mbcnt_lo(~0u, 0u)) : lane;
+    const int t_e = PACK ? wi * 64 + lane_e : t;
+    const int oq = t_e & 15, otl = t_e >> 4;
+    const bool o_far = PACK && (otl & 7) >= pk_ks;
+    const int ob = o_far ? b + 1 : b, otx = o_far ? (otl & 7) - pk_ks : tx0 + (otl & 7);
+    const bool o_ok = !o_far || pk_two;
     const int n = nb * kBN + oq * 4;
     const f32x4 e_sc = P.scale ? *reinterpret_cast<const f32x4*>(P.scale + n) : f32x4{1.f, 1.f, 1.f, 1.f};
     const f32x4 e_sh = P.shift ? *reinterpret_cast<const f32x4*>(P.shift + n) : f32x4{0.f, 0.f, 0.f, 0.f};
@@ -338,12 +366,12 @@
 #pragma unroll
         for (int q = 0; q < 4; ++q) {
             const int ot = otl + 16 * tp;
-            const int y = 2 * (ty0 + (ot >> 3)) + (q >> 1), x = 2 * (tx0 + (ot & 7)) + (q & 1);
-            e_res[tp][q] = (P.res && y < H && x < W) ? *reinterpret_cast<const f32x4*>(P.res + ((size_t)b * HW + (size_t)y * W + x) * Cout + n)
+            const int y = 2 * (ty0 + (ot >> 3)) + (q >> 1), x = 2 * otx + (q & 1);
+            e_res[tp][q] = (P.res && o_ok && y < H && x < W) ? *reinterpret_cast<const f32x4*>(P.res + ((size_t)ob * HW + (size_t)y * W + x) * Cout + n)
                                                      : f32x4{0.f, 0.f, 0.f, 0.f};
         }
     __syncthreads();
-    float* const zb = lds + ((wi * 2) * kNT + 4 * lh) * kBN + li;
+    float* const zb = lds + ((wi * 2) * kNT + 4 * (PACK ? lane_e >> 5 : lh)) * kBN + (PACK ? lane_e & 31 : li);
 #pragma unroll
     for (int mt = 0; mt < 2; ++mt)
 #pragma unroll
@@ -360,7 +388,7 @@
 #pragma unroll
     for (int tp = 0; tp < 4; ++tp) {
         const int ot = otl + 16 * tp;
-        const int oty = ty0 + (ot >> 3), otx = tx0 + (ot & 7);
+        const int oty = ty0 + (ot >> 3);
         f32x4 z[4][2];
 #pragma unroll
         for (int i = 0; i < 4; ++i)
@@ -371,7 +399,7 @@
 #pragma unroll
             for (int cc = 0; cc < 2; ++cc) {
                 const int y = 2 * oty + rr, x = 2 * otx + cc;
-                if (y >= H || x >= W) continue;
+                if (y >= H || x >= W || !o_ok) continue;
                 f32x4 val = (rr == 0 ? z[0][cc] + z[1][cc] + z[2][cc] : z[1][cc] - z[2][cc] - z[3][cc]) * inv_s;
                 if (FOLD) {
                     const int cls = (((y == 0) | ((y == H - 1) << 1)) << 2) | (x == 0) | ((x == W - 1) << 1);
@@ -379,7 +407,7 @@
                 }
                 if (P.scale) val = val * e_sc;
                 val = val + e_sh;
-                const size_t o = ((size_t)b * HW + (size_t)y * W + x) * Cout + n;
+                const size_t o = ((size_t)ob * HW + (size_t)y * W + x) * Cout + n;
                 if (P.res) val += e_res[tp][2 * rr + cc];
                 if (a.relu) { val[0] = fmaxf(val[0], 0.f); val[1] = fmaxf(val[1], 0.f); val[2] = fmaxf(val[2], 0.f); val[3] = fmaxf(val[3], 0.f); }
                 *reinterpret_cast<f32x4*>(P.out + o) = val;
@@ -387,7 +415,39 @@
                 s2 += val * val;
             }
     }
-    if (P.gn_part) {
+    if (PACK && P.gn_part) {
+        f32x4 q1[2] = {o_far ? f32x4{0.f, 0.f, 0.f, 0.f} : s1, o_far ? s1 : f32x4{0.f, 0.f, 0.f, 0.f}};
+        f32x4 q2[2] = {o_far ? f32x4{0.f, 0.f, 0.f, 0.f} : s2, o_far ? s2 : f32x4{0.f, 0.f, 0.f, 0.f}};
+#pragma unroll
+        for (int sd = 0; sd < 2; ++sd)
+#pragma unroll
+            for (int o = 16; o < 64; o <<= 1)
+#pragma unroll
+                for (int k = 0; k < 4; ++k) { q1[sd][k] += __shfl_xor(q1[sd][k], o, 64); q2[sd][k] += __shfl_xor(q2[sd][k], o, 64); }
+        __syncthreads();
+        float* red = lds;
+        if (lane_e < 16) {
+#pragma unroll
+            for (int sd = 0; sd < 2; ++sd)
+#pragma unroll
+                for (int k = 0; k < 4; ++k) {
+                    red[((sd * 4 + wi) * kBN + oq * 4 + k) * 2] = q1[sd][k];
+                    red[((sd * 4 + wi) * kBN + oq * 4 + k) * 2 + 1] = q2[sd][k];
+                }
+        }
+        __syncthreads();
+        if (t_e < 2 * kBN && (t_e < kBN || pk_two)) {
+            const int sd = t_e >> 6, ch = t_e & (kBN - 1);
+            float u1 = 0.f, u2 = 0.f;
+#pragma unroll
+            for (int w = 0; w < 4; ++w) { u1 += red[((sd * 4 + w) * kBN + ch) * 2]; u2 += red[((sd * 4 + w) * kBN + ch) * 2 + 1]; }
+            const int rx = a.pack_rx, Pn = a.tby * rx, slot = sd ? 0 : pk_slot;
+            float* g = P.gn_part + (((size_t)(b + sd) * Pn + by * rx + slot) * Cout + nb * kBN + ch) * 2;
+            g[0] = u1; g[1] = u2;
+            if (sd == 0 && pk_raw <= kTX)
+                for (int z = slot + 1; z < rx; ++z) { g += (size_t)Cout * 2; g[0] = 0.f; g[1] = 0.f; }
+        }
+    } else if (P.gn_part) {
 #pragma unroll
         for (int o = 16; o < 64; o <<= 1)
 #pragma unroll
@@ -456,10 +516,38 @@
     }
 }
 
+WinoPackGeom wino_pack_geometry(int H, int W, int B, int Cin, bool allow) {
+    WinoPackGeom q;
+    const int tcw = cdiv(W, 2), tch = cdiv(H, 2);
+    q.G = 1;
+    q.tby = cdiv(tch, kTY);
+    if (allow && tcw >= kTX && 2LL * H * W * Cin * (long long)sizeof(float) < (1LL << 32)) {
+        int best = cdiv(tcw, kTX);
+        for (int g = 2; g <= std::min(B, 8); ++g)
+            if ((long long)cdiv(g * tcw, kTX) * q.G < (long long)best * g) { best = cdiv(g * tcw, kTX); q.G = g; }
+    }
+    q.tbx = cdiv(q.G * tcw, kTX);
+    q.rx = 1;
+    for (int f = 0; f < q.G; ++f) q.rx = std::max(q.rx, (f * tcw + tcw - 1) / kTX - (f * tcw) / kTX + 1);
+    q.patches = (long long)q.tby * ((long long)(B / q.G) * q.tbx + cdiv((B % q.G) * tcw, kTX));
+    q.slots = q.patches * kNT;
+    q.tiles = (long long)B * tch * tcw;
+    q.gn_rows = q.tby * q.rx;
+    return q;
+}
+
 int launch_conv_wino_h3(const WinoArgs& a, int groups, hipStream_t s) {
     if (groups < 1 || groups > kMaxGroup || a.Cin % 16 != 0 || a.Cout % kBN != 0) return FPC_EINVAL;
     if ((long long)a.H * a.W * a.Cin * (long long)sizeof(float) >= (1LL << 32)) return FPC_EINVAL;
     if ((long long)(a.Cin >> 4) * kPairBytes >= (1LL << 31)) return FPC_EINVAL;
+    if (a.pack > 1) {
+        const WinoPackGeom q = wino_pack_geometry(a.H, a.W, a.B, a.Cin, !a.fold);
+        if (q.G != a.pack || q.tbx != a.tbx || q.tby != a.tby || q.rx != a.pack_rx) return FPC_EINVAL;
+        const long long nblk = q.patches * (a.Cout / kBN) * groups;
+        if (nblk < 1 || nblk >= (1LL << 31)) return FPC_EINVAL;
+        hipLaunchKernelGGL((k_conv_wino_h3<0, false, true>), dim3((unsigned)nblk), dim3(256), 0, s, a);
+        return check_launch();
+    }
     if (a.tbx != cdiv(cdiv(a.W, 2), kTX) || a.tby != cdiv(cdiv(a.H, 2), kTY)) return FPC_EINVAL;
     const long long nblk = (long long)a.tbx * a.tby * a.B * (a.Cout / kBN) * groups;
     if (nblk < 1 || nblk >= (1LL << 31)) return FPC_EINVAL;
@@ -469,12 +557,12 @@
             return FPC_EINVAL;
         for (int g = 0; g < groups; ++g)
             if (!a.in2[g] || !a.w2[g] || !a.btab[g] || a.p[g].scale || a.p[g].shift || a.p[g].res || a.p[g].up) return FPC_EINVAL;
-        hipLaunchKernelGGL((k_conv_wino_h3<0, true>), dim3((unsigned)nblk), dim3(256), 0, s, a);
+        hipLaunchKernelGGL((k_conv_wino_h3<0, true, false>), dim3((unsigned)nblk), dim3(256), 0, s, a);
         return check_launch();
     }
     static const int var = getenv("FPC_H3_VAR") ? atoi(getenv("FPC_H3_VAR")) : 0;
-    if (var == 1) hipLaunchKernelGGL((k_conv_wino_h3<1, false>), dim3((unsigned)nblk), dim3(256), 0, s, a);
-    else hipLaunchKernelGGL((k_conv_wino_h3<0, false>), dim3((unsigned)nblk), dim3(256), 0, s, a);
+    if (var == 1) hipLaunchKernelGGL((k_conv_wino_h3<1, false, false>), dim3((unsigned)nblk), dim3(256), 0, s, a);
+    else hipLaunchKernelGGL((k_conv_wino_h3<0, false, false>), dim3((unsigned)nblk), dim3(256), 0, s, a);
     return check_launch();
 }
 
diff --git a/fastposecnn_amd/engine.py b/fastposecnn_amd/engine.py
--- a/fastposecnn_amd/engine.py
+++ b/fastposecnn_amd/engine.py
@@ -106,6 +106,12 @@
             nat.check(rc, "fpc_net_force_stem_pool")
         return rc
 
+    def set_wino_pack(self, on):
+        nat.check(self._lib.fpc_net_set_wino_pack(self._h, int(on)), "fpc_net_set_wino_pack")
+
+    def wino_blocks(self):
+        return int(self._lib.fpc_net_wino_blocks(self._h))
+
     def force_pointwise(self, on):
         rc = self._lib.fpc_net_force_pointwise(self._h, int(on))
         if rc < 0:
diff --git a/include/fpc.h b/include/fpc.h
--- a/include/fpc.h
+++ b/include/fpc.h
@@ -174,6 +174,9 @@
 int fpc_net_force_direct_h3(fpc_net_t* net, int on);
 int fpc_net_force_stem_pool(fpc_net_t* net, int on);
 int fpc_stem_pool_tasks(int Ho, int Wo, int64_t* out4);
+int fpc_wino_pack_geometry(int H, int W, int B, int Cin, int fold, int64_t* out8);
+int fpc_net_set_wino_pack(fpc_net_t* net, int on);
+int64_t fpc_net_wino_blocks(const fpc_net_t* net);
 int fpc_net_flops(const fpc_net_t* net, double* out3);
 int fpc_net_tensor(const fpc_net_t* net, const char* name, const float** ptr, int* H, int* W, int* C);
 
diff --git a/tools_dev/frame_window_stats.py b/tools_dev/frame_window_stats.py
--- /dev/null
+++ b/tools_dev/frame_window_stats.py
@@ -0,0 +1,39 @@
+import collections
+import csv
+import sys
+
+rows = list(csv.DictReader(open(sys.argv[1])))
+rows.sort(key=lambda r: int(r["Start_Timestamp"]))
+marks = [i for i, r in enumerate(rows) if "nchw3_to_nhwc4" in r["Kernel_Name"]]
+if "--frame" in sys.argv:
+    s = marks[-5]
+    key = "Stream_Id" if "Stream_Id" in rows[s] else "Queue_Id"
+    q = rows[s][key]
+    mine = [r for r in rows[s:] if r[key] == q]
+    end = next(i for i, r in enumerate(mine[1:], 1) if "nchw3_to_nhwc4" in r["Kernel_Name"])
+    t0, tot = int(mine[0]["Start_Timestamp"]), 0.0
+    for r in mine[:end]:
+        d = (int(r["End_Timestamp"]) - int(r["Start_Timestamp"])) / 1e3
+        tot += d
+        print("%9.1f %8.2f grid=(%d,%s,%s) %s" % ((int(r["Start_Timestamp"]) - t0) / 1e3, d, int(r["Grid_Size_X"]) // int(r["Workgroup_Size_X"]),
+                                                 r["Grid_Size_Y"], r["Grid_Size_Z"], r["Kernel_Name"][:80]))
+    print("sum of kernels %.1f us, span %.1f us, %d dispatches on stream / queue %s" % (tot, (int(mine[end]["Start_Timestamp"]) - t0) / 1e3, end, q))
+    sys.exit(0)
+N = int(sys.argv[2]) if len(sys.argv) > 2 else 200
+assert len(marks) > N, "fewer frames in the trace than asked for"
+s, e = marks[-N - 1], marks[-1]
+span = (int(rows[e]["Start_Timestamp"]) - int(rows[s]["Start_Timestamp"])) / 1e3
+tot = collections.OrderedDict()
+for r in rows[s:e]:
+    nm = r["Kernel_Name"].split("(")[0].replace("void ", "").replace("fpc::", "")
+    if "k_conv_wino_h3" in nm:
+        nm += " grid=%d" % (int(r["Grid_Size_X"]) // int(r["Workgroup_Size_X"]))
+    d = (int(r["End_Timestamp"]) - int(r["Start_Timestamp"])) / 1e3
+    c = tot.setdefault(nm[:80], [0, 0.0])
+    c[0] += 1; c[1] += d
+allk = sum(v[1] for v in tot.values())
+wino = sum(v[1] for k, v in tot.items() if "k_conv_wino_h3" in k)
+print("%d frames, span %.1f us per frame, kernels %.1f us per frame, k_conv_wino_h3 %.1f us per frame (%.1f %%)"
+      % (N, span / N, allk / N, wino / N, 100.0 * wino / allk))
+for k, v in sorted(tot.items(), key=lambda kv: -kv[1][1]):
+    print("%10.1f us/frame  %7.2f calls/frame  %9.1f us mean  %s" % (v[1] / N, v[0] / N, v[1] / v[0], k))
```

Result: faster. 2661 (median of 6 runs) (+2.6%).
